# 1879615351/Go-RIO

Measured on AMD Instinct MI355X. Metric: APD-GICP GN iters/sec on 16k-pt scans + GP-preint windows/sec, higher is better.
Workload: dtype f32 search / f64 accumulate; 1 GPU; C4: 64 scan pairs 16384x16384 + 64 GP windows 1 s @ 200 Hz per GPU, k-NN covariances + 20 fixed GN iterations per pair; pairs_per_gpu=64, target_points=16384, optimizer=GN (convergence test disabled), search=pruned, parallelism=batch shard x1 (no collective)

## Files before the change

### go-rio_amd/csrc/apd_kernels.hip

```cpp
#include <hip/hip_runtime.h>
#include <math.h>
#include <stdint.h>

#include "apd_device.h"

namespace gorio {


typedef const float __attribute__((address_space(4)))* scalar_fp;
__device__ __forceinline__ scalar_fp as_scalar(const float* p) { return (scalar_fp)p; }

__device__ __forceinline__ float sqdist3(float qx, float qy, float qz, float tx, float ty, float tz) {
  float dx = qx - tx, dy = qy - ty, dz = qz - tz;
  float r = dx * dx;
  r = r + dy * dy;
  r = r + dz * dz;
  return r;
}

__device__ __forceinline__ void transform_f(const float* __restrict__ Tf, float x, float y, float z, float& qx, float& qy, float& qz) {
  float a = Tf[0] * x;
  a = a + Tf[1] * y;
  a = a + Tf[2] * z;
  qx = a + Tf[3];
// ... 111 lines not shown
      if (d[u] < bd[K - 1]) topk_insert<K>(bd, bi, d[u], j + u);
    }
  }
  if (i < n) {
    const size_t base = (size_t)split * K * n + i;
#pragma unroll
    for (int t = 0; t < K; ++t) {
      job.part_d[base + (size_t)t * n] = bd[t];
      job.part_i[base + (size_t)t * n] = bi[t];
    }
  }
}

__device__ __forceinline__ void jacobi_rot(double& app, double& aqq, double& apq, double& apr, double& aqr, double& v0p, double& v1p, double& v2p, double& v0q, double& v1q, double& v2q) {
  if (apq == 0.0) return;
  const double g = 100.0 * fabs(apq);
  if (fabs(app) + g == fabs(app) && fabs(aqq) + g == fabs(aqq)) {
    apq = 0.0;
    return;
  }
  const double theta = (aqq - app) / (2.0 * apq);
  double t = 1.0 / (fabs(theta) + sqrt(theta * theta + 1.0));
  if (theta < 0.0) t = -t;
  const double c = 1.0 / sqrt(t * t + 1.0);
  const double s = t * c;
  app = app - t * apq;
  aqq = aqq + t * apq;
  apq = 0.0;
  const double npr = c * apr - s * aqr;
  const double nqr = s * apr + c * aqr;
  apr = npr;
  aqr = nqr;
  double a, b;
  a = v0p; b = v0q; v0p = c * a - s * b; v0q = s * a + c * b;
  a = v1p; b = v1q; v1p = c * a - s * b; v1q = s * a + c * b;
  a = v2p; b = v2q; v2p = c * a - s * b; v2q = s * a + c * b;
}

struct Eig3 {
  double w0, w1, w2;
  double v00, v10, v20;
  double v01, v11, v21;
  double v02, v12, v22;
};

__device__ __forceinline__ void swap_cols(double& wa, double& wb, double& a0, double& a1, double& a2, double& b0, double& b1, double& b2) {
  double t;
  t = wa; wa = wb; wb = t;
  t = a0; a0 = b0; b0 = t;
  t = a1; a1 = b1; b1 = t;
  t = a2; a2 = b2; b2 = t;
}

__device__ __forceinline__ Eig3 sym3_eigen(double a00, double a01, double a02, double a11, double a12, double a22) {
  Eig3 e;
  e.v00 = 1; e.v10 = 0; e.v20 = 0;
  e.v01 = 0; e.v11 = 1; e.v21 = 0;
  e.v02 = 0; e.v12 = 0; e.v22 = 1;
#pragma unroll 1
  for (int sweep = 0; sweep < 12; ++sweep) {
    if (a01 == 0.0 && a02 == 0.0 && a12 == 0.0) break;
    jacobi_rot(a00, a11, a01, a02, a12, e.v00, e.v10, e.v20, e.v01, e.v11, e.v21);
    jacobi_rot(a00, a22, a02, a01, a12, e.v00, e.v10, e.v20, e.v02, e.v12, e.v22);
    jacobi_rot(a11, a22, a12, a01, a02, e.v01, e.v11, e.v21, e.v02, e.v12, e.v22);
  }
  e.w0 = a00; e.w1 = a11; e.w2 = a22;
  if (e.w0 < e.w1) swap_cols(e.w0, e.w1, e.v00, e.v10, e.v20, e.v01, e.v11, e.v21);
  if (e.w1 < e.w2) swap_cols(e.w1, e.w2, e.v01, e.v11, e.v21, e.v02, e.v12, e.v22);
  if (e.w0 < e.w1) swap_cols(e.w0, e.w1, e.v00, e.v10, e.v20, e.v01, e.v11, e.v21);
  return e;
}

__device__ __forceinline__ double geo_weight(double c00, double c01, double c02, double c11, double c12, double c22) {
  Eig3 e = sym3_eigen(c00, c01, c02, c11, c12, c22);
  const double s0 = fabs(e.w0), s1 = fabs(e.w1), s2 = fabs(e.w2);
  const double smax = fmax(s0, fmax(s1, s2)), smin = fmin(s0, fmin(s1, s2));
  return smin / smax;
}

__device__ __forceinline__ void inv_sym3(double a00, double a01, double a02, double a11, double a12, double a22, double& i00, double& i01, double& i02, double& i11, double& i12, double& i22) {
  const double c00 = a11 * a22 - a12 * a12;
  const double c01 = a02 * a12 - a01 * a22;
  const double c02 = a01 * a12 - a02 * a11;
  const double det = a00 * c00 + a01 * c01 + a02 * c02;
  const double r = 1.0 / det;
  i00 = c00 * r;
  i01 = c01 * r;
  i02 = c02 * r;
  i11 = (a00 * a22 - a02 * a02) * r;
  i12 = (a01 * a02 - a00 * a12) * r;
  i22 = (a00 * a11 - a01 * a01) * r;
}

template <int K>
__device__ __forceinline__ void covariance_from_list(const KnnJob& job, int i, const float (&bd)[K], const int (&bi)[K]) {
  const int k = job.k;
  (void)bd;
  if (job.knn_out) {
#pragma unroll
    for (int t = 0; t < K; ++t)
      if (t < k) job.knn_out[(size_t)i * k + t] = bi[t];
  }
  const float4* __restrict__ pts = job.cloud.p4;
  float px[K], py[K], pz[K];
#pragma unroll
  for (int t = 0; t < K; ++t) {
    const float4 v = pts[t < k ? bi[t] : bi[0]];
    px[t] = v.x; py[t] = v.y; pz[t] = v.z;
  }
  double mx = 0.0, my = 0.0, mz = 0.0;
#pragma unroll
  for (int t = 0; t < K; ++t)
    if (t < k) {
      mx += (double)px[t];
      my += (double)py[t];
      mz += (double)pz[t];
    }
  const double kd = (double)k;
  mx /= kd;
  my /= kd;
  mz /= kd;
  double c00 = 0, c01 = 0, c02 = 0, c11 = 0, c12 = 0, c22 = 0;
#pragma unroll
  for (int t = 0; t < K; ++t)
    if (t < k) {
      const double dx = (double)px[t] - mx, dy = (double)py[t] - my, dz = (double)pz[t] - mz;
      c00 += dx * dx;
      c01 += dx * dy;
      c02 += dx * dz;
      c11 += dy * dy;
      c12 += dy * dz;
      c22 += dz * dz;
    }
  c00 /= kd; c01 /= kd; c02 /= kd; c11 /= kd; c12 /= kd; c22 /= kd;

  double r00, r01, r02, r11, r12, r22;
  double geo = 0.0;
  bool have_geo = false;
  if (job.regularization == 0) {
    r00 = c00; r01 = c01; r02 = c02; r11 = c11; r12 = c12; r22 = c22;
  } else if (job.regularization == 4) {
    double i00, i01, i02, i11, i12, i22;
    inv_sym3(c00 + 1e-3, c01, c02, c11 + 1e-3, c12, c22 + 1e-3, i00, i01, i02, i11, i12, i22);
    const double fro = sqrt(i00 * i00 + i11 * i11 + i22 * i22 + 2.0 * (i01 * i01 + i02 * i02 + i12 * i12));
    inv_sym3(i00 / fro, i01 / fro, i02 / fro, i11 / fro, i12 / fro, i22 / fro, r00, r01, r02, r11, r12, r22);
  } else {
    Eig3 e = sym3_eigen(c00, c01, c02, c11, c12, c22);
    double s0 = fabs(e.w0), s1 = fabs(e.w1), s2 = fabs(e.w2);
    double l0, l1, l2;
    if (job.regularization == 3) {
      l0 = 1.0; l1 = 1.0; l2 = 1e-3;
    } else if (job.regularization == 1) {
      l0 = fmax(s0, 1e-3); l1 = fmax(s1, 1e-3); l2 = fmax(s2, 1e-3);
    } else {
      const double smax = fmax(s0, fmax(s1, s2));
      l0 = fmax(s0 / smax, 1e-3); l1 = fmax(s1 / smax, 1e-3); l2 = fmax(s2 / smax, 1e-3);
    }
    r00 = e.v00 * l0 * e.v00 + e.v01 * l1 * e.v01 + e.v02 * l2 * e.v02;
    r01 = e.v00 * l0 * e.v10 + e.v01 * l1 * e.v11 + e.v02 * l2 * e.v12;
    r02 = e.v00 * l0 * e.v20 + e.v01 * l1 * e.v21 + e.v02 * l2 * e.v22;
    r11 = e.v10 * l0 * e.v10 + e.v11 * l1 * e.v11 + e.v12 * l2 * e.v12;
    r12 = e.v10 * l0 * e.v20 + e.v11 * l1 * e.v21 + e.v12 * l2 * e.v22;
    r22 = e.v20 * l0 * e.v20 + e.v21 * l1 * e.v21 + e.v22 * l2 * e.v22;
    geo = fmin(l0, fmin(l1, l2)) / fmax(l0, fmax(l1, l2));
    have_geo = true;
  }
  double* o = job.cloud.cov6 + (size_t)i * 6;
  o[0] = r00; o[1] = r01; o[2] = r02; o[3] = r11; o[4] = r12; o[5] = r22;
  job.cloud.geo_w[i] = have_geo ? geo : geo_weight(r00, r01, r02, r11, r12, r22);
}

template <int K>
__global__ __launch_bounds__(256) void cov_finalize_kernel(const KnnJob* __restrict__ jobs) {
  const KnnJob job = jobs[blockIdx.z];
  const int n = job.cloud.n;
  const int i = blockIdx.x * 256 + threadIdx.x;
  if (i >= n) return;
  float bd[K];
  int bi[K];
#pragma unroll
  for (int t = 0; t < K; ++t) {
    bd[t] = INFINITY;
    bi[t] = 0x7fffffff;
  }
  for (int s = 0; s < job.splits; ++s) {
    const size_t base = (size_t)s * K * n + i;
    for (int t = 0; t < K; ++t) {
      const float d = job.part_d[base + (size_t)t * n];
      if (!(d < bd[K - 1])) break;
      topk_insert<K>(bd, bi, d, job.part_i[base + (size_t)t * n]);
    }
  }
  covariance_from_list<K>(job, i, bd, bi);
}

__global__ __launch_bounds__(256) void geo_weight_kernel(const double* __restrict__ cov6, double* __restrict__ geo_w, int n) {
  const int i = blockIdx.x * 256 + threadIdx.x;
  if (i >= n) return;
  const double* c = cov6 + (size_t)i * 6;
  geo_w[i] = geo_weight(c[0], c[1], c[2], c[3], c[4], c[5]);
}


__global__ __launch_bounds__(256) void nn_search_kernel(const PairDesc* __restrict__ descs) {
  const PairDesc& pd = descs[blockIdx.z];
  const PairState* __restrict__ st = pd.state;
  if (st->done) return;
  const int n = pd.src.n;
  if (blockIdx.x * 256 >= n) return;
  if ((int)(blockIdx.x * 256) < pd.shard_lo || (int)(blockIdx.x * 256) >= pd.shard_hi) return;
  const int split = blockIdx.y;
  if (split >= pd.nn_splits) return;
  const int j0 = split * pd.nn_chunk;
  int j1 = j0 + pd.nn_chunk;
  if (j1 > pd.tgt.n_pad) j1 = pd.tgt.n_pad;
  const int i = blockIdx.x * 256 + threadIdx.x;
  const int iq = i < n ? i : n - 1;
  float qx, qy, qz;
  transform_f(st->Tf, pd.src.x[iq], pd.src.y[iq], pd.src.z[iq], qx, qy, qz);
  const scalar_fp tx = as_scalar(pd.tgt.x);
  const scalar_fp ty = as_scalar(pd.tgt.y);
  const scalar_fp tz = as_scalar(pd.tgt.z);
  float best = INFINITY;
  int bc = 0x7fffffff;
  for (int j = j0; j < j1; j += 16) {
    float d[16];
#pragma unroll
    for (int u = 0; u < 16; ++u) d[u] = sqdist3(qx, qy, qz, tx[j + u], ty[j + u], tz[j + u]);
    const float m0 = fminf(fminf(d[0], d[1]), d[2]), m1 = fminf(fminf(d[3], d[4]), d[5]), m2 = fminf(fminf(d[6], d[7]), d[8]);
    const float m3 = fminf(fminf(d[9], d[10]), d[11]), m4 = fminf(fminf(d[12], d[13]), d[14]);
    const float m = fminf(fminf(fminf(m0, m1), m2), fminf(fminf(m3, m4), d[15]));
    const bool lt = m < best;
    best = lt ? m : best;
    bc = lt ? j : bc;
  }
  int bj = 0x7fffffff;
  if (bc != 0x7fffffff) {
#pragma unroll
    for (int u = 15; u >= 0; --u) {
      const float d = sqdist3(qx, qy, qz, pd.tgt.x[bc + u], pd.tgt.y[bc + u], pd.tgt.z[bc + u]);
      bj = d == best ? bc + u : bj;
    }
  }
  if (i < n && bj != 0x7fffffff) {
    const unsigned long long key = ((unsigned long long)__float_as_uint(best) << 32) | (unsigned int)bj;
    atomicMin(pd.best_key + i, key);
  }
}


struct PointTerms {
  double e0, e1, e2;
  double a0, a1, a2;
  double o00, o01, o02, o11, o12, o22;
};

__device__ __forceinline__ double residual_terms(const double* __restrict__ T, float ax, float ay, float az, float bx, float by, float bz, PointTerms& p) {
#pragma clang fp contract(fast)
  const double x = (double)ax, y = (double)ay, z = (double)az;
  p.a0 = T[0] * x + T[1] * y + T[2] * z + T[3];
  p.a1 = T[4] * x + T[5] * y + T[6] * z + T[7];
  p.a2 = T[8] * x + T[9] * y + T[10] * z + T[11];
  p.e0 = (double)bx - p.a0;
  p.e1 = (double)by - p.a1;
  p.e2 = (double)bz - p.a2;
  const double m0 = p.o00 * p.e0 + p.o01 * p.e1 + p.o02 * p.e2;
  const double m1 = p.o01 * p.e0 + p.o11 * p.e1 + p.o12 * p.e2;
  const double m2 = p.o02 * p.e0 + p.o12 * p.e1 + p.o22 * p.e2;
  return p.e0 * m0 + p.e1 * m1 + p.e2 * m2;
}

__device__ void gn_step_tail(const PairDesc& pd, const ApdConsts& cst);
__device__ double vgicp_error_part(const PairDesc& pd, const VoxPair& vp, const double* __restrict__ T);
template <bool VGICP>
__device__ double ndtc_error_part(const PairDesc& pd, const NdtcPair& np, const double* __restrict__ T);

__device__ __forceinline__ float sumsq2_f(float a, float b) {
  float r = a * a;
  r = r + b * b;
  return r;
}

template <int METHOD>
__global__ __launch_bounds__(256) __attribute__((amdgpu_waves_per_eu(6, 6))) void linearize_kernel(const PairDesc* __restrict__ descs, ApdConsts cst, int fuse) {
  const GridPos gp = xcd_grid_pos();
  const PairDesc& pd = descs[gp.z];
  PairState* __restrict__ st = pd.state;
  const __attribute__((address_space(4))) PairState* sst = (const __attribute__((address_space(4))) PairState*)pd.state;
  if (sst->done) return;
  const int n = pd.src.n;
  if (gp.x * 256 >= (unsigned int)n) return;
  const int i = gp.x * 256 + threadIdx.x;

  double acc[28];
#pragma unroll
  for (int t = 0; t < 28; ++t) acc[t] = 0.0;

  if (i < n) {
    typedef const __attribute__((address_space(1))) unsigned long long* g_u64p;
    typedef const __attribute__((address_space(1))) double* g_f64p;
    typedef const __attribute__((address_space(1))) float* g_f32p;
    const unsigned long long key = ((g_u64p)pd.best_key)[i];
    const float ax = ((g_f32p)pd.src.x)[i], ay = ((g_f32p)pd.src.y)[i], az = ((g_f32p)pd.src.z)[i];
    const float src_label = ((g_f32p)pd.src.label)[i];
    const double src_geo_w = ((g_f64p)pd.src.geo_w)[i];
    double cA[6];
#pragma unroll
    for (int t = 0; t < 6; ++t) cA[t] = ((g_f64p)pd.src.cov6)[(size_t)i * 6 + t];
    pd.best_key[i] = ~0ull;
    const float d = __uint_as_float((unsigned int)(key >> 32));
    int j = (int)(unsigned int)(key & 0xffffffffu);
    const bool found = key != ~0ull;
    pd.sqd[i] = found ? d : INFINITY;
    if (!found || !((double)d < cst.thr2)) j = -1;
    pd.corr[i] = j;
    const int jj = j >= 0 ? j : 0;
    double cB[6];
#pragma unroll
    for (int t = 0; t < 6; ++t) cB[t] = ((g_f64p)pd.tgt.cov6)[(size_t)jj * 6 + t];
    float4 tb;
    {
      typedef float v4f_lin __attribute__((ext_vector_type(4)));
      const v4f_lin t4 = ((const __attribute__((address_space(1))) v4f_lin*)pd.tgt.p4)[jj];
      tb = make_float4(t4.x, t4.y, t4.z, t4.w);
    }
    double* om = pd.omega6 + (size_t)i * 6;
    if (j >= 0) {
#pragma clang fp contract(fast)
      double T[12];
      float Tf[12];
#pragma unroll
      for (int t = 0; t < 12; ++t) {
        T[t] = sst->x0[t];
        Tf[t] = sst->Tf[t];
      }
      double r00 = 0.0, r01 = 0.0, r02 = 0.0, r11 = 0.0, r12 = 0.0, r22 = 0.0;
      if constexpr (METHOD == kMethodApd) {
      float qx, qy, qz;
      transform_f(Tf, ax, ay, az, qx, qy, qz);
      const double px = (double)qx, py = (double)qy, pz = (double)qz;
      const double pxy2 = px * px + py * py;
      const double dist = sqrt(pxy2 + pz * pz);
      const double s_x = dist * cst.dist_var / 400;
      const double s_y = dist * cst.sin_az;
      const double s_z = dist * cst.sin_el;
      const float rxy = (float)sqrt((double)sumsq2_f(qx, qy));
      double ce, se, ca, sa;
      {
        const double rd = (double)rxy;
        const double el = atan2(rd, pz), az = atan2(py, px);
        const double del = (double)(float)el - el, daz = (double)(float)az - az;
        const double h2 = rd * rd + pz * pz;
        const double ih = h2 > 0.0 ? rsqrt_newton(h2) : 0.0, ir = pxy2 > 0.0 ? rsqrt_newton(pxy2) : 0.0;
        const double se0 = rd * ih, ce0 = h2 > 0.0 ? pz * ih : 1.0;
        const double sa0 = py * ir, ca0 = pxy2 > 0.0 ? px * ir : 1.0;
        const double sde = del - del * del * del * (1.0 / 6.0), cde = 1.0 - 0.5 * del * del;
        const double sda = daz - daz * daz * daz * (1.0 / 6.0), cda = 1.0 - 0.5 * daz * daz;
        se = se0 * cde + ce0 * sde;
        ce = ce0 * cde - se0 * sde;
        sa = sa0 * cda + ca0 * sda;
        ca = ca0 * cda - sa0 * sda;
      }
      const double A00 = ca * ce * s_x, A01 = -sa * s_y, A02 = ca * se * s_z;
      const double A10 = sa * ce * s_x, A11 = ca * s_y, A12 = sa * se * s_z;
      const double A20 = -se * s_x, A22 = ce * s_z;
      r00 = A00 * A00 + A01 * A01 + A02 * A02;
      r01 = A00 * A10 + A01 * A11 + A02 * A12;
      r02 = A00 * A20 + A02 * A22;
      r11 = A10 * A10 + A11 * A11 + A12 * A12;
      r12 = A10 * A20 + A12 * A22;
      r22 = A20 * A20 + A22 * A22;
      }
      double a00 = cA[0], a01 = cA[1], a02 = cA[2], a11 = cA[3], a12 = cA[4], a22 = cA[5];
      if constexpr (METHOD == kMethodApd) {
        a00 = cA[0] + r00; a01 = cA[1] + r01; a02 = cA[2] + r02; a11 = cA[3] + r11; a12 = cA[4] + r12; a22 = cA[5] + r22;
      }
      const double R00 = T[0], R01 = T[1], R02 = T[2], R10 = T[4], R11 = T[5], R12 = T[6], R20 = T[8], R21 = T[9], R22 = T[10];
      const double M00 = R00 * a00 + R01 * a01 + R02 * a02, M01 = R00 * a01 + R01 * a11 + R02 * a12, M02 = R00 * a02 + R01 * a12 + R02 * a22;
      const double M10 = R10 * a00 + R11 * a01 + R12 * a02, M11 = R10 * a01 + R11 * a11 + R12 * a12, M12 = R10 * a02 + R11 * a12 + R12 * a22;
      const double M20 = R20 * a00 + R21 * a01 + R22 * a02, M21 = R20 * a01 + R21 * a11 + R22 * a12, M22 = R20 * a02 + R21 * a12 + R22 * a22;
      if constexpr (METHOD == kMethodApd) {
        cB[0] += r00; cB[1] += r01; cB[2] += r02; cB[3] += r11; cB[4] += r12; cB[5] += r22;
      }
      const double q00 = cB[0] + (M00 * R00 + M01 * R01 + M02 * R02);
      const double q01 = cB[1] + (M00 * R10 + M01 * R11 + M02 * R12);
      const double q02 = cB[2] + (M00 * R20 + M01 * R21 + M02 * R22);
      const double q11 = cB[3] + (M10 * R10 + M11 * R11 + M12 * R12);
      const double q12 = cB[4] + (M10 * R20 + M11 * R21 + M12 * R22);
      const double q22 = cB[5] + (M20 * R20 + M21 * R21 + M22 * R22);
      PointTerms p;
      inv_sym3(q00, q01, q02, q11, q12, q22, p.o00, p.o01, p.o02, p.o11, p.o12, p.o22);
      if (pd.write_omega) {
        om[0] = p.o00; om[1] = p.o01; om[2] = p.o02; om[3] = p.o11; om[4] = p.o12; om[5] = p.o22;
      }

      const double quad = residual_terms(T, ax, ay, az, tb.x, tb.y, tb.z, p);
      if constexpr (METHOD == kMethodApd) {
        const double w = 1.0 + src_geo_w + ((tb.w == src_label) ? 1.0 / (double)(pd.cl_points > 0 ? pd.cl_points : n) : 0.0);
        acc[27] = w * quad;
      } else {
        acc[27] = quad;
      }

      const double G00 = p.a2 * p.o01 - p.a1 * p.o02, G01 = p.a2 * p.o11 - p.a1 * p.o12, G02 = p.a2 * p.o12 - p.a1 * p.o22;
      const double G10 = -p.a2 * p.o00 + p.a0 * p.o02, G11 = -p.a2 * p.o01 + p.a0 * p.o12, G12 = -p.a2 * p.o02 + p.a0 * p.o22;
      const double G20 = p.a1 * p.o00 - p.a0 * p.o01, G21 = p.a1 * p.o01 - p.a0 * p.o11, G22 = p.a1 * p.o02 - p.a0 * p.o12;
      const double Hrr00 = G01 * p.a2 - G02 * p.a1, Hrr01 = -G00 * p.a2 + G02 * p.a0, Hrr02 = G00 * p.a1 - G01 * p.a0;
      const double Hrr11 = -G10 * p.a2 + G12 * p.a0, Hrr12 = G10 * p.a1 - G11 * p.a0;
      const double Hrr22 = G20 * p.a1 - G21 * p.a0;
      acc[0] = Hrr00; acc[1] = Hrr01; acc[2] = Hrr02; acc[3] = -G00; acc[4] = -G01; acc[5] = -G02;
      acc[6] = Hrr11; acc[7] = Hrr12; acc[8] = -G10; acc[9] = -G11; acc[10] = -G12;
      acc[11] = Hrr22; acc[12] = -G20; acc[13] = -G21; acc[14] = -G22;
      acc[15] = p.o00; acc[16] = p.o01; acc[17] = p.o02;
      acc[18] = p.o11; acc[19] = p.o12;
      acc[20] = p.o22;
      const double oe0 = p.o00 * p.e0 + p.o01 * p.e1 + p.o02 * p.e2;
      const double oe1 = p.o01 * p.e0 + p.o11 * p.e1 + p.o12 * p.e2;
      const double oe2 = p.o02 * p.e0 + p.o12 * p.e1 + p.o22 * p.e2;
      acc[21] = G00 * p.e0 + G01 * p.e1 + G02 * p.e2;
      acc[22] = G10 * p.e0 + G11 * p.e1 + G12 * p.e2;
      acc[23] = G20 * p.e0 + G21 * p.e1 + G22 * p.e2;
      acc[24] = -oe0; acc[25] = -oe1; acc[26] = -oe2;
    } else {
      if (pd.write_omega) {
        om[0] = 0; om[1] = 0; om[2] = 0; om[3] = 0; om[4] = 0; om[5] = 0;
      }
    }
  }

  __shared__ double red[4][28];
  const int lane = threadIdx.x & 63, wv = threadIdx.x >> 6;
  {
    double ws[7];
    wave_sum28(acc, ws);
    if ((lane & 15) == 0) {
#pragma unroll
      for (int k = 0; k < 7; ++k) red[wv][7 * (lane >> 4) + k] = ws[k];
    }
  }
  __syncthreads();
  if (threadIdx.x < 28) {
    const double s = (red[0][threadIdx.x] + red[1][threadIdx.x]) + (red[2][threadIdx.x] + red[3][threadIdx.x]);
    if (!fuse) {
      pd.partials[(size_t)gp.x * 28 + threadIdx.x] = s;
    } else {
      __hip_atomic_store(pd.partials + (size_t)gp.x * 28 + threadIdx.x, s, __ATOMIC_RELAXED, __HIP_MEMORY_SCOPE_AGENT);
    }
  }
  if (!fuse) return;
  __shared__ int s_last;
  asm volatile("s_waitcnt vmcnt(0) lgkmcnt(0)" ::: "memory");
  if (threadIdx.x == 0) s_last = __hip_atomic_fetch_add(&st->arrive, 1u, __ATOMIC_RELAXED, __HIP_MEMORY_SCOPE_AGENT) == (unsigned int)pd.nblk - 1u;
  __syncthreads();
  if (!s_last) return;
  if (threadIdx.x == 0) __hip_atomic_store(&st->arrive, 0u, __ATOMIC_RELAXED, __HIP_MEMORY_SCOPE_AGENT);
  gn_step_tail(pd, cst);
}


__device__ void ldlt6_solve(const double* __restrict__ A_in, const double* __restrict__ rhs, double* __restrict__ x, double* __restrict__ ws) {
  double* A = ws;
  double* y = ws + 36;
  double* col = ws + 42;
  int* perm = reinterpret_cast<int*>(ws + 48);
  for (int i = 0; i < 36; ++i) A[i] = A_in[i];
  for (int i = 0; i < 6; ++i) perm[i] = i;
  for (int k = 0; k < 6; ++k) {
    int piv = k;
    double best = fabs(A[k * 6 + k]);
    for (int i = k + 1; i < 6; ++i)
      if (fabs(A[i * 6 + i]) > best) {
        best = fabs(A[i * 6 + i]);
        piv = i;
      }
    if (piv != k) {
      for (int c = 0; c < 6; ++c) {
        double t = A[k * 6 + c];
        A[k * 6 + c] = A[piv * 6 + c];
        A[piv * 6 + c] = t;
      }
      for (int r = 0; r < 6; ++r) {
        double t = A[r * 6 + k];
        A[r * 6 + k] = A[r * 6 + piv];
        A[r * 6 + piv] = t;
      }
      int t = perm[k];
      perm[k] = perm[piv];
      perm[piv] = t;
    }
    const double d = A[k * 6 + k];
    if (d == 0.0) continue;
    for (int i = k + 1; i < 6; ++i) col[i] = A[i * 6 + k];
    for (int i = k + 1; i < 6; ++i) {
      const double l = col[i] / d;
      for (int j = k + 1; j <= i; ++j) A[i * 6 + j] -= l * col[j];
      A[i * 6 + k] = l;
    }
    for (int i = k + 1; i < 6; ++i)
      for (int j = i + 1; j < 6; ++j) A[i * 6 + j] = A[j * 6 + i];
  }
  for (int i = 0; i < 6; ++i) y[i] = rhs[perm[i]];
  for (int i = 0; i < 6; ++i)
    for (int j = 0; j < i; ++j) y[i] -= A[i * 6 + j] * y[j];
  for (int i = 0; i < 6; ++i) y[i] = (A[i * 6 + i] != 0.0) ? y[i] / A[i * 6 + i] : 0.0;
  for (int i = 5; i >= 0; --i)
    for (int j = i + 1; j < 6; ++j) y[i] -= A[j * 6 + i] * y[j];
  for (int i = 0; i < 6; ++i) x[perm[i]] = y[i];
}

__device__ void delta_from_d(const double* __restrict__ d, double* __restrict__ delta) {
  const double theta_sq = d[0] * d[0] + d[1] * d[1] + d[2] * d[2];
  double imag, real;
  if (theta_sq < 1e-10) {
    const double theta_quad = theta_sq * theta_sq;
    imag = 0.5 - 1.0 / 48.0 * theta_sq + 1.0 / 3840.0 * theta_quad;
    real = 1.0 - 1.0 / 8.0 * theta_sq + 1.0 / 384.0 * theta_quad;
  } else {
    const double theta = sqrt(theta_sq);
    const double half = 0.5 * theta;
    imag = sin(half) / theta;
    real = cos(half);
  }
  const double w = real, x = imag * d[0], y = imag * d[1], z = imag * d[2];
  const double tx = 2.0 * x, ty = 2.0 * y, tz = 2.0 * z;
  const double twx = tx * w, twy = ty * w, twz = tz * w, txx = tx * x, txy = ty * x, txz = tz * x, tyy = ty * y, tyz = tz * y, tzz = tz * z;
  delta[0] = 1.0 - (tyy + tzz); delta[1] = txy - twz; delta[2] = txz + twy; delta[3] = d[3];
  delta[4] = txy + twz; delta[5] = 1.0 - (txx + tzz); delta[6] = tyz - twx; delta[7] = d[4];
  delta[8] = txz - twy; delta[9] = tyz + twx; delta[10] = 1.0 - (txx + tyy); delta[11] = d[5];
  delta[12] = 0; delta[13] = 0; delta[14] = 0; delta[15] = 1;
}

__device__ void isom_mul(const double* __restrict__ A, const double* __restrict__ B, double* __restrict__ C) {
  double t[16];
#pragma unroll
  for (int r = 0; r < 3; ++r) {
#pragma unroll
    for (int c = 0; c < 3; ++c) t[r * 4 + c] = A[r * 4 + 0] * B[c] + A[r * 4 + 1] * B[4 + c] + A[r * 4 + 2] * B[8 + c];
    t[r * 4 + 3] = A[r * 4 + 0] * B[3] + A[r * 4 + 1] * B[7] + A[r * 4 + 2] * B[11] + A[r * 4 + 3];
  }
  t[12] = 0; t[13] = 0; t[14] = 0; t[15] = 1;
#pragma unroll
  for (int i = 0; i < 16; ++i) C[i] = t[i];
}

__device__ bool is_converged(const double* __restrict__ delta, double inv_rot_eps, double inv_trans_eps) {
  double rmax = 0.0, tmax = 0.0;
#pragma unroll
  for (int r = 0; r < 3; ++r) {
#pragma unroll
    for (int c = 0; c < 3; ++c) {
      const double v = inv_rot_eps * fabs(delta[r * 4 + c] - (r == c ? 1.0 : 0.0));
      rmax = v > rmax ? v : rmax;
    }
    const double v = inv_trans_eps * fabs(delta[r * 4 + 3]);
    tmax = v > tmax ? v : tmax;
  }
  return fmax(rmax, tmax) < 1.0;
}

template <int METHOD, typename AUX>
__device__ double block_error(const PairDesc& pd, const AUX* __restrict__ vp, const double* __restrict__ T, const ApdConsts& cst, double* __restrict__ sred) {
  const int n = pd.src.n;
  double sum = 0.0;
  if constexpr (METHOD == kMethodVgicp) {
    sum = vgicp_error_part(pd, *vp, T);
  } else if constexpr (METHOD == kMethodNdtCuda) {
    sum = ndtc_error_part<false>(pd, *vp, T);
  } else if constexpr (METHOD == kMethodVgicpCuda) {
    sum = ndtc_error_part<true>(pd, *vp, T);
  } else {
    for (int i = threadIdx.x; i < n; i += blockDim.x) {
      const int j = pd.corr[i];
      if (j < 0) continue;
      const double* om = pd.omega6 + (size_t)i * 6;
      PointTerms p;
      p.o00 = om[0]; p.o01 = om[1]; p.o02 = om[2]; p.o11 = om[3]; p.o12 = om[4]; p.o22 = om[5];
      const float4 tb = pd.tgt.p4[j];
      const double quad = residual_terms(T, pd.src.x[i], pd.src.y[i], pd.src.z[i], tb.x, tb.y, tb.z, p);
      if constexpr (METHOD == kMethodApd) {
        const double w = 1.0 + pd.src.geo_w[i] + ((tb.w == pd.src.label[i]) ? 1.0 / (double)(pd.cl_points > 0 ? pd.cl_points : n) : 0.0);
        sum += w * quad;
      } else {
        sum += quad;
      }
    }
  }
  sum = wave_sum(sum);
  const int lane = threadIdx.x & 63, wv = threadIdx.x >> 6;
  __syncthreads();
  if (lane == 0) sred[wv] = sum;
  __syncthreads();
  double tot = 0.0;
  const int nw = blockDim.x >> 6;
  for (int w = 0; w < nw; ++w) tot += sred[w];
  return tot;
}

template <int METHOD, typename AUX>
__device__ void lm_solve_body(const PairDesc& pd, const AUX* __restrict__ vp, const ApdConsts& cst, int mode) {
  PairState* __restrict__ st = pd.state;
  __shared__ double sH[36], sb[6], sxi[16], sdelta[16], sd[6], sws[56], sHl[36], snb[6];
  __shared__ double sy0, sred[16];
  __shared__ int sflag;
  if (mode == 2) {
    const double yi = block_error<METHOD>(pd, vp, st->xi, cst, sred);
    if (threadIdx.x == 0) st->yi = yi;
    return;
  }
  if (st->done) return;

  if (threadIdx.x < 28) {
    double s = 0.0;
    for (int bk0 = 0; bk0 < pd.nblk; bk0 += 16) {
      double v[16];
#pragma unroll
      for (int u = 0; u < 16; ++u) v[u] = (bk0 + u < pd.nblk) ? pd.partials[(size_t)(bk0 + u) * 28 + threadIdx.x] : 0.0;
#pragma unroll
      for (int u = 0; u < 16; ++u) s += v[u];
    }
    const int t = threadIdx.x;
    if (t < 21) {
      int r = 0, c = t;
      int rowlen = 6;
      while (c >= rowlen) {
        c -= rowlen;
        ++r;
        --rowlen;
      }
      c += r;
      sH[r * 6 + c] = s;
      sH[c * 6 + r] = s;
    } else if (t < 27) {
      sb[t - 21] = s;
    } else {
      sy0 = s;
    }
  }
  __syncthreads();
  if (threadIdx.x == 0) {
    for (int a = 0; a < 36; ++a) st->H[a] = sH[a];
    for (int a = 0; a < 6; ++a) st->b[a] = sb[a];
    st->y0 = sy0;
    st->n_linearize += 1;
  }
  if (mode == 1) return;

  const double inv_re = 1.0 / cst.rot_eps, inv_te = 1.0 / cst.trans_eps;
  int ok = 0;
  if (cst.optimizer == 0) {
    if (threadIdx.x == 0) {
      for (int a = 0; a < 6; ++a) snb[a] = -sb[a];
      ldlt6_solve(sH, snb, sd, sws);
      delta_from_d(sd, sdelta);
      isom_mul(sdelta, st->x0, sxi);
      for (int a = 0; a < 16; ++a) st->x0[a] = sxi[a];
      for (int a = 0; a < 36; ++a) st->Hfin[a] = sH[a];
    }
    ok = 1;
  } else {
    double lambda = st->lambda;
    if (lambda < 0.0) {
      double mx = 0.0;
      for (int a = 0; a < 6; ++a) mx = fmax(mx, fabs(sH[a * 6 + a]));
      lambda = cst.lm_init_lambda_factor * mx;
    }
    double nu = 2.0;
    for (int trial = 0; trial < cst.lm_max_iterations; ++trial) {
      if (threadIdx.x == 0) {
        for (int a = 0; a < 36; ++a) sHl[a] = sH[a];
        for (int a = 0; a < 6; ++a) {
          sHl[a * 6 + a] += lambda;
          snb[a] = -sb[a];
        }
        ldlt6_solve(sHl, snb, sd, sws);
        delta_from_d(sd, sdelta);
        isom_mul(sdelta, st->x0, sxi);
      }
      __syncthreads();
      const double yi = block_error<METHOD>(pd, vp, sxi, cst, sred);
      if (threadIdx.x == 0) {
        st->n_error += 1;
        double den = 0.0;
        for (int a = 0; a < 6; ++a) den += sd[a] * (lambda * sd[a] - sb[a]);
        const double rho = (sy0 - yi) / den;
        if (rho < 0) {
          sflag = is_converged(sdelta, inv_re, inv_te) ? 2 : 0;
        } else {
          sflag = 1;
          for (int a = 0; a < 16; ++a) st->x0[a] = sxi[a];
          const double f = 1 - pow(2 * rho - 1, 3);
          st->lambda = lambda * fmax(1.0 / 3.0, f);
          for (int a = 0; a < 36; ++a) st->Hfin[a] = sH[a];
        }
      }
      __syncthreads();
      const int flag = sflag;
      if (flag == 1) {
        ok = 1;
        break;
      }
      if (flag == 2) {
        ok = 1;
        if (threadIdx.x == 0) st->lambda = lambda;
        break;
      }
      lambda = nu * lambda;
      nu = 2 * nu;
      if (threadIdx.x == 0) st->lambda = lambda;
    }
  }
  __syncthreads();
  if (threadIdx.x == 0) {
    const int it = st->iter;
    st->nr_iterations = it;
    int done = 0, conv = 0;
    if (!ok) {
      done = 1;
      st->lm_failed = 1;
    } else {
      conv = is_converged(sdelta, inv_re, inv_te) ? 1 : 0;
      if (conv) done = 1;
    }
    st->iter = it + 1;
    if (it + 1 >= cst.max_iterations) done = 1;
    st->converged = conv;
    for (int a = 0; a < 12; ++a) st->Tf[a] = (float)st->x0[a];
    __threadfence();
// ... 295 lines not shown
```

### go-rio_amd/csrc/ugpm_api.hip

```cpp
#include <hip/hip_runtime.h>

#include <algorithm>
#include <cstdlib>
#include <chrono>
#include <cstdio>
#include <cstring>
#include <limits>
#include <memory>
#include <string>
#include <atomic>
#include <vector>

#include "../../include/gorio_ugpm.h"
#include "dev_buffer.h"
#include "ugpm_kernels.hip"
#include "ugpm_lpm_out.hip"
#include "ugpm_chunks.h"
#include "ugpm_windows.h"

using namespace gorio;
using namespace gorio::windows;

namespace {

#ifndef GORIO_EVAL_SPLIT
#define GORIO_EVAL_SPLIT 12
#endif
constexpr int kEvalSplit = GORIO_EVAL_SPLIT;

thread_local std::string g_err;
thread_local double g_stage_s[8] = {0, 0, 0, 0, 0, 0, 0, 0};
thread_local int g_stage_n[8] = {0, 0, 0, 0, 0, 0, 0, 0};
std::atomic<int> g_speculative_rot{1};
std::atomic<int> g_debug_path{0};

int ufail(int code, const std::string& msg) {
  g_err = msg;
  return code;
}

#define UHIP(expr)                                                                                              \
  do {                                                                                                          \
    hipError_t e_ = (expr);                                                                                     \
    if (e_ != hipSuccess) return ufail(GORIO_UGPM_ERR_NO_DEVICE, std::string(#expr) + ": " + hipGetErrorString(e_)); \
  } while (0)

struct StreamPair {
  hipStream_t s = nullptr, s2 = nullptr;
  hipEvent_t ev_jac = nullptr, ev_corr = nullptr;
};

int make_stream_pair(StreamPair& p) {
  int lo = 0, hi = 0;
  if (!(hipDeviceGetStreamPriorityRange(&lo, &hi) == hipSuccess && hipStreamCreateWithPriority(&p.s, hipStreamNonBlocking, hi) == hipSuccess))
    UHIP(hipStreamCreateWithFlags(&p.s, hipStreamNonBlocking));
  UHIP(hipStreamCreateWithFlags(&p.s2, hipStreamNonBlocking));
  UHIP(hipEventCreateWithFlags(&p.ev_jac, hipEventDisableTiming));
  UHIP(hipEventCreateWithFlags(&p.ev_corr, hipEventDisableTiming));
  return 0;
}

void destroy_stream_pair(StreamPair& p) {
  if (p.s) hipStreamDestroy(p.s);
  if (p.s2) hipStreamDestroy(p.s2);
  if (p.ev_jac) hipEventDestroy(p.ev_jac);
  if (p.ev_corr) hipEventDestroy(p.ev_corr);
  p = StreamPair();
}

struct Ctx {
  int device = -1;
  StreamPair main;
  hipEvent_t ev_up = nullptr;
  struct Group : StreamPair { hipEvent_t ev_done = nullptr, ev_tab = nullptr; };
  std::vector<Group> groups;
  DevBuf<double> ws;
  DevBuf<UgpmWin> d_wins;
  DevBuf<int> d_ints;
  DevBuf<double> d_diag;
  size_t wins_cap = 0;
  int lm_budget[2] = {0, 0};
  PinnedBuf pin_in;
  PinnedBuf pin_out;
  DevBuf<double> lpm_ws;
  DevBuf<int> lpm_ints;
  DevBuf<ug::LpmOutWin> d_lpm_wins;
  struct StageEvents { hipEvent_t a, b; int stage; };
  std::vector<StageEvents> ev;

  void drop_stage_events() {
    for (auto& e : ev) { hipEventDestroy(e.a); hipEventDestroy(e.b); }
    ev.clear();
  }
  void reset() {
    if (device >= 0) hipSetDevice(device);
    for (size_t g = 1; g < groups.size(); ++g) destroy_stream_pair(groups[g]);
    for (Group& g : groups) { hipEventDestroy(g.ev_done); hipEventDestroy(g.ev_tab); }
    groups.clear();
    destroy_stream_pair(main);
    if (ev_up) hipEventDestroy(ev_up);
    ev_up = nullptr;
    drop_stage_events();
    ws.reset(); d_wins.reset(); d_ints.reset(); d_diag.reset(); pin_in.reset(); pin_out.reset(); lpm_ws.reset(); lpm_ints.reset(); d_lpm_wins.reset();
    wins_cap = 0;
    lm_budget[0] = lm_budget[1] = 0;
    device = -1;
  }
  ~Ctx() { reset(); }
};
thread_local Ctx g_ctx;

struct Stage {
  Ctx& c;
  hipStream_t stream;
  size_t slot = 0;
  bool on = false;
  Stage(Ctx& c_, int s, hipStream_t st = nullptr) : c(c_), stream(st ? st : c_.main.s) {
    hipEvent_t a = nullptr, b = nullptr;
    if (hipEventCreate(&a) != hipSuccess || hipEventCreate(&b) != hipSuccess) return;
    slot = c.ev.size();
    c.ev.push_back({a, b, s});
    hipEventRecord(a, stream);
    on = true;
  }
  ~Stage() {
    if (on) hipEventRecord(c.ev[slot].b, stream);
  }
};
struct StageEventsGuard {
  Ctx& c;
  ~StageEventsGuard() { c.drop_stage_events(); }
};

struct Run : Ctx::Group {
  int g0 = 0, nw = 0;
  const UgpmWin* wins = nullptr;
  bool active = true;
};

struct Batch {
  const gorio_ugpm_window* windows;
  int nw;
  std::vector<HostWin> hw;
  std::vector<UgpmWin> dw;
  std::vector<int> ints, flags, lpm_ints_h;
  std::vector<double> lpm_in;
  std::vector<ug::LpmOutWin> lw;
  std::vector<size_t> out_offs;
  std::vector<Run> runs;
  size_t total_doubles = 0, total_in = 0, total_out = 0;
  double* out_region = nullptr;
  int max_S = 0, max_G = 2, max_V = 2, max_infer = 0, n_lpm = 0;
  bool rerun = false;
  bool looks = false;
  bool enqueued_blind[2] = {false, false};
  std::vector<int> final_status;
  int first_error = 0;
  std::string first_error_msg;
  void note_error(int i, int code, const std::string& m) {
    if (first_error) return;
    first_error = code;
    first_error_msg = "window " + std::to_string(i) + ": " + m;
  }
};

int ensure_context(Ctx& c, int device) {
  int ndev = 0;
  if (hipGetDeviceCount(&ndev) != hipSuccess || ndev <= 0) return ufail(GORIO_UGPM_ERR_NO_DEVICE, "no usable HIP device (no CPU fallback exists)");
  if (device < 0 || device >= ndev) return ufail(GORIO_UGPM_ERR_INVALID, "bad device ordinal");
  if (c.device != device) c.reset();
  UHIP(hipSetDevice(device));
  if (c.device == device) return 0;
  if (int rc = make_stream_pair(c.main)) return rc;
  UHIP(hipFuncSetAttribute(reinterpret_cast<const void*>(&ug::corr_diag_kernel), hipFuncAttributeMaxDynamicSharedMemorySize, 140 * 1024));
  UHIP(hipFuncSetAttribute(reinterpret_cast<const void*>(&ug::infer_kernel), hipFuncAttributeMaxDynamicSharedMemorySize, 17 * (6 * 160 + 16) * 8) );
  const void* fns[] = {reinterpret_cast<const void*>(&ug::ata_kernel<4, 16, kAtaTilesCorr>), reinterpret_cast<const void*>(&ug::ata_kernel<8, 16, kAtaTilesCorr>),
                       reinterpret_cast<const void*>(&ug::ata_kernel<16, 8, kAtaTilesCorr>), reinterpret_cast<const void*>(&ug::ata_kernel<4, 16, kAtaTilesLm>),
                       reinterpret_cast<const void*>(&ug::ata_kernel<8, 16, kAtaTilesLm>)};
  for (const void* f : fns) UHIP(hipFuncSetAttribute(f, hipFuncAttributeMaxDynamicSharedMemorySize, 144 * 1024));
  c.device = device;
  return 0;
}

void plan_windows(Batch& b) {
  b.hw.resize(b.nw);
  int total_infer = 0;
  for (int i = 0; i < b.nw; ++i) {
    const gorio_ugpm_window& w = b.windows[i];
    HostWin& h = b.hw[i];
    total_infer += std::max(0, w.n_infer);
    b.max_infer = std::max(b.max_infer, w.n_infer);
    std::string err;
    if (plan_window(w, h, err) != 0) {
      b.note_error(i, h.status, err);
    } else if (h.is_lpm) {
      b.n_lpm++;
    } else {
      b.max_S = std::max(b.max_S, h.S);
      b.total_in += input_slot(w, h);
      b.total_doubles += h.ws_doubles;
    }
  }
  for (const HostWin& h : b.hw) {
    b.max_G = std::max(b.max_G, h.is_lpm ? 2 : h.G);
    b.max_V = std::max(b.max_V, h.is_lpm ? 2 : h.V);
  }
  b.total_out = (size_t)total_infer * 83;
  b.total_doubles += b.total_in + b.total_out + 64;
}

int reserve_workspace(Ctx& c, const Batch& b) {
  const size_t nw = b.nw;
  UHIP(c.ws.reserve(b.total_doubles));
  UHIP(reserve_group(c.wins_cap, nw, nw, c.d_wins, nw, c.d_ints, kWinInts * nw, c.d_diag, 4 * nw));
  UHIP(c.pin_in.reserve(sizeof(double) * b.total_in, sizeof(double) * (b.total_in + b.total_in / 4 + 64)));
  const size_t down = sizeof(double) * (b.total_out + 4 * nw) + sizeof(int) * kWinInts * nw;
  UHIP(c.pin_out.reserve(down, down + down / 4 + 64));
  return 0;
}

int stage_and_upload(Ctx& c, Batch& b) {
  b.dw.resize(b.nw);
  b.ints.assign(kWinInts * (size_t)b.nw, 0);
  b.out_offs.assign(b.nw, 0);
  double* const in_region = c.ws.get();
  b.out_region = in_region + b.total_in;
  double* base = b.out_region + (b.total_out + 31) / 32 * 32;
  double* const stage_in = static_cast<double*>(c.pin_in.get());
  size_t in_off = 0, out_off = 0;
  for (int i = 0; i < b.nw; ++i) {
    const gorio_ugpm_window& w = b.windows[i];
    const HostWin& h = b.hw[i];
    UgpmWin& u = b.dw[i];
    std::memset(&u, 0, sizeof(u));
    u.lmi = c.d_ints + kWinInts * (size_t)i;
    u.status = c.d_ints + kWinInts * (size_t)i + 16;
    b.ints[kWinInts * (size_t)i + 16] = h.status;
    u.n_infer = std::max(0, w.n_infer);
    b.out_offs[i] = out_off;
    u.out = b.out_region + out_off;
    out_off += (size_t)u.n_infer * 83;
    if (h.status != 0) continue;
    if (h.is_lpm) {
      b.ints[kWinInts * (size_t)i + 16] = 1;
      u.n_infer = 0;
      continue;
    }
    carve(w, h, u, base, in_region + in_off, u.out);
    u.G = h.G; u.V = h.V; u.S = h.S;
    u.correlate = w.correlate ? 1 : 0; u.overlap = w.overlap;
    u.state_freq = h.state_freq;
    copy_noise_and_priors(w, u);
    base += h.ws_doubles;
    double* s = stage_in + in_off;
    const size_t padded = input_slot(w, h);
    for (size_t k = padded - 4; k < padded; ++k) s[k] = 0.0;
    s = stage_samples(s, w, h.g0, h.G, h.v0, h.V);
    std::copy(h.state_t.begin(), h.state_t.end(), s);
    in_off += padded;
  }
  if (b.total_in) UHIP(hipMemcpyAsync(in_region, stage_in, sizeof(double) * b.total_in, hipMemcpyHostToDevice, c.main.s));
  UHIP(hipMemcpyAsync(c.d_wins, b.dw.data(), sizeof(UgpmWin) * b.nw, hipMemcpyHostToDevice, c.main.s));
  UHIP(hipMemcpyAsync(c.d_ints, b.ints.data(), sizeof(int) * b.ints.size(), hipMemcpyHostToDevice, c.main.s));
  UHIP(hipMemsetAsync(c.d_diag, 0, sizeof(double) * 4 * b.nw, c.main.s));
  return 0;
}

int run_lpm_windows(Ctx& c, Batch& b) {
  if (b.n_lpm == 0) return 0;
  std::vector<LpmHost> lh(b.n_lpm);
  std::vector<int> widx;
  size_t dbl = 0, in_dbl = 0, nint = 0;
  int max_T = 2;
  for (int i = 0; i < b.nw; ++i) {
    if (!b.hw[i].is_lpm || b.hw[i].status != 0) continue;
    LpmHost& L = lh[widx.size()];
    build_lpm_timeline(b.windows[i], L);
    widx.push_back(i);
    max_T = std::max(max_T, (int)L.tl.size());
    ug::LpmOutWin dummy;
    const LpmSize sz = carve_lpm(b.windows[i], L.tl.size(), dummy, nullptr, nullptr, nullptr);
    in_dbl += sz.in;
    dbl += sz.scratch + 8;
    nint += sz.ints;
  }
  UHIP(c.lpm_ws.reserve(in_dbl + dbl));
  UHIP(c.lpm_ints.reserve(nint));
  UHIP(c.d_lpm_wins.reserve(b.n_lpm));
  b.lw.resize(widx.size());
  b.lpm_in.assign(in_dbl, 0.0);
  b.lpm_ints_h.assign(nint, 0);
  LpmSize at;
  for (size_t k = 0; k < widx.size(); ++k) {
    const int i = widx[k];
    const gorio_ugpm_window& w = b.windows[i];
    const LpmHost& L = lh[k];
    ug::LpmOutWin& u = b.lw[k];
    std::memset(&u, 0, sizeof(u));
    const LpmSize sz = carve_lpm(w, L.tl.size(), u, c.lpm_ws.get() + at.in, c.lpm_ws.get() + in_dbl + at.scratch, c.lpm_ints.get() + at.ints);
    std::copy(L.tl.begin(), L.tl.end(), stage_samples(b.lpm_in.data() + at.in, w, 0, w.n_gyr, 0, w.n_vel));
    stage_lpm_tables(b.lpm_ints_h.data() + at.ints, L);
    at.in += sz.in; at.scratch += sz.scratch; at.ints += sz.ints;
    u.G = w.n_gyr; u.V = w.n_vel; u.T = (int)L.tl.size(); u.n_infer = w.n_infer;
    u.start_index = L.start_index; u.dt_index = L.dt_index;
    copy_noise_and_priors(w, u);
    u.out = b.dw[i].out;
    u.status = c.d_ints + kWinInts * (size_t)i + 17;
  }
  UHIP(hipMemcpyAsync(c.lpm_ws, b.lpm_in.data(), sizeof(double) * in_dbl, hipMemcpyHostToDevice, c.main.s));
  UHIP(hipMemcpyAsync(c.lpm_ints, b.lpm_ints_h.data(), sizeof(int) * nint, hipMemcpyHostToDevice, c.main.s));
  UHIP(hipMemcpyAsync(c.d_lpm_wins, b.lw.data(), sizeof(ug::LpmOutWin) * b.lw.size(), hipMemcpyHostToDevice, c.main.s));
  const int nl = (int)b.lw.size();
  if (nl > 0) {
    Stage st(c, 0);
    ug::lpm_out_steps_kernel<<<dim3((max_T + 255) / 256, 5, nl), 256, 0, c.main.s>>>(c.d_lpm_wins);
    ug::lpm_out_scan_kernel<<<dim3(5, nl), 64, 0, c.main.s>>>(c.d_lpm_wins);
    ug::lpm_out_finish_kernel<<<nl, 256, 0, c.main.s>>>(c.d_lpm_wins);
    UHIP(hipGetLastError());
  }
  return 0;
}

int open_groups(Ctx& c, Batch& b) {
  int n_groups = 1;
  if (const char* e = std::getenv("GORIO_UGPM_GROUPS")) n_groups = std::atoi(e);
  n_groups = std::max(1, std::min(std::min(n_groups, 8), b.nw));
  while ((int)c.groups.size() < n_groups) {
    Ctx::Group g;
    if (c.groups.empty()) static_cast<StreamPair&>(g) = c.main;
    else if (int rc = make_stream_pair(g)) return rc;
    UHIP(hipEventCreateWithFlags(&g.ev_done, hipEventDisableTiming));
    UHIP(hipEventCreateWithFlags(&g.ev_tab, hipEventDisableTiming));
    c.groups.push_back(g);
  }
  if (!c.ev_up) UHIP(hipEventCreateWithFlags(&c.ev_up, hipEventDisableTiming));
  UHIP(hipEventRecord(c.ev_up, c.main.s));
  b.runs.resize(n_groups);
  for (int g = 0; g < n_groups; ++g) {
    Run& r = b.runs[g];
    static_cast<Ctx::Group&>(r) = c.groups[g];
    r.g0 = (int)((long)b.nw * g / n_groups);
    r.nw = (int)((long)b.nw * (g + 1) / n_groups) - r.g0;
    r.wins = c.d_wins + r.g0;
    if (g > 0) UHIP(hipStreamWaitEvent(r.s, c.ev_up, 0));
  }
  return 0;
}

void launch_ata(Ctx& c, int max_S, const Run& r, int which, int decide = 0) {
  hipStream_t sq = which == 2 ? r.s2 : r.s;
  Stage st_ata(c, which == 2 ? 6 : 5, sq);
  const int n = (which == 2 ? 6 : 3) * max_S;
  const int tpg = which == 2 ? kAtaTilesCorr : kAtaTilesLm;
  const int dense = (g_debug_path.load() & 1) ? 1 : 0;
  const int ng = ata_cut(n, which == 2 && !dense ? 3 * max_S : n, tpg).groups();
  const int npad = ((n + 15) / 32) * 32 + 16;
  const int grid = ((r.nw + 7) / 8) * ng * 8;
  auto lds = [&](int kc) { return sizeof(double) * 2 * kc * (npad + 1); };
  if (which == 2) {
    if (npad <= 256) ug::ata_kernel<4, 16, kAtaTilesCorr><<<grid, 512, lds(16), sq>>>(r.wins, which, r.nw, ng, decide, dense);
    else if (npad <= 512) ug::ata_kernel<8, 16, kAtaTilesCorr><<<grid, 512, lds(16), sq>>>(r.wins, which, r.nw, ng, decide, dense);
    else ug::ata_kernel<16, 8, kAtaTilesCorr><<<grid, 512, lds(8), sq>>>(r.wins, which, r.nw, ng, decide, dense);
  } else {
    if (npad <= 256) ug::ata_kernel<4, 16, kAtaTilesLm><<<grid, 512, lds(16), sq>>>(r.wins, which, r.nw, ng, decide, dense);
    else ug::ata_kernel<8, 16, kAtaTilesLm><<<grid, 512, lds(16), sq>>>(r.wins, which, r.nw, ng, decide, dense);
  }
}

int enqueue_tables_and_correlation(Ctx& c, Batch& b) {
  const int max_S = b.max_S;
  for (const Run& r : b.runs) {
    {
      Stage st(c, 0, r.s);
      ug::lpm_rot_kernel<<<dim3(r.nw, 5), 320, 0, r.s>>>(r.wins);
      ug::lpm_init_kernel<<<r.nw, 320, 0, r.s>>>(r.wins);
    }
    {
      Stage st(c, 1, r.s);
      ug::gram_kernel<<<dim3(6, r.nw), 256, 0, r.s>>>(r.wins);
      ug::cross_kernel<<<dim3(12, r.nw, (std::max(b.max_G, b.max_V) + ug::kCrossRows - 1) / ug::kCrossRows), 256, sizeof(double) * ug::kCrossRows * (((max_S + 31) / 32) * 32 + 4), r.s>>>(r.wins);
    }
    UHIP(hipEventRecord(r.ev_tab, r.s));
    UHIP(hipStreamWaitEvent(r.s2, r.ev_tab, 0));
    {
      Stage st(c, 2, r.s2);
      ug::corr_jac_kernel<<<dim3(ug::kCorrJacParts, r.nw), 256, 0, r.s2>>>(r.wins);
      UHIP(hipEventRecord(r.ev_jac, r.s2));
      launch_ata(c, max_S, r, 2);
      ug::corr_factor_kernel<<<r.nw, 512, 0, r.s2>>>(r.wins);
      ug::corr_diag_kernel<<<dim3((6 * max_S + 15) / 16, r.nw), 256, sizeof(double) * 17 * (6 * max_S + 16), r.s2>>>(r.wins);
    }
    UHIP(hipEventRecord(r.ev_corr, r.s2));
  }
  return 0;
}

int run_fit(Ctx& c, Batch& b, int problem) {
  const int max_S = b.max_S;
  std::vector<int>& flags = b.flags;
  const bool lmtrace = std::getenv("GORIO_UGPM_LMTRACE") != nullptr;
  const bool speculative = g_speculative_rot.load() != 0;
  std::vector<std::unique_ptr<Stage>> st_lm;
  for (Run& r : b.runs) {
    st_lm.emplace_back(new Stage(c, 3, r.s));
    if (problem == 0) ug::rot_eval_kernel<<<dim3(r.nw, kEvalSplit), 256, 0, r.s>>>(r.wins, 2);
    else ug::vel_eval_kernel<<<dim3(r.nw, kEvalSplit), 256, 0, r.s>>>(r.wins, 2);
    launch_ata(c, max_S, r, problem);
    r.active = true;
  }
  for (int it = 0; it <= 51; ++it) {
    bool any = false;
    for (Run& r : b.runs) {
      if (!r.active) continue;
      any = true;
      ug::lm_step_kernel<<<dim3(r.nw, problem == 1 ? kVelBlocks : 1), 512, 0, r.s>>>(r.wins);
      if (problem == 0 && speculative) {
        ug::rot_eval_kernel<<<dim3(r.nw, kEvalSplit), 256, 0, r.s>>>(r.wins, 3);
        launch_ata(c, max_S, r, problem, 1);
        continue;
      }
      if (problem == 0) ug::rot_eval_kernel<<<dim3(r.nw, kEvalSplit), 256, 0, r.s>>>(r.wins, 0);
      else ug::vel_eval_kernel<<<dim3(r.nw, kEvalSplit), 256, 0, r.s>>>(r.wins, 0);
      if (problem == 0) {
        ug::rot_eval_kernel<<<dim3(r.nw, kEvalSplit), 256, 0, r.s>>>(r.wins, 1);
        launch_ata(c, max_S, r, problem);
      } else {
        ug::lm_relinearize_linear_kernel<<<dim3(r.nw, (3 * max_S + 63) / 64), 256, 0, r.s>>>(r.wins);
      }
    }
    if (!any) break;
    if (lmtrace) {
      double lc[16];
      int li[16];
      UHIP(hipStreamSynchronize(b.runs[0].s));
      UHIP(hipMemcpy(lc, b.dw[0].lmc, sizeof(lc), hipMemcpyDeviceToHost));
      UHIP(hipMemcpy(li, b.dw[0].lmi, sizeof(li), hipMemcpyDeviceToHost));
      std::fprintf(stderr, "[ugpm lm] problem %d it %d: iter %d done %d term %d succ %d cost %.17g cost_new %.17g radius %.6g mcc %.17g step_norm2 %.6g x_norm %.17g initial %.17g\n", problem, it,
                   li[0], li[1], li[5], li[6], lc[0], lc[1], lc[2], lc[8], lc[11], lc[4], lc[7]);
    }
    const int budget = c.lm_budget[problem];
    if (budget > 0 && !b.looks) {
      b.enqueued_blind[problem] = true;
      if (it + 1 >= budget) break;
      continue;
    }
    const bool look = budget > 0 ? (it + 1 >= budget && ((it + 1 - budget) & 1) == 0) : (it >= 3 && (it & 1) == 1);
    if (look) {
      for (Run& r : b.runs)
        if (r.active) UHIP(hipMemcpyAsync(flags.data() + kWinInts * (size_t)r.g0, c.d_ints + kWinInts * (size_t)r.g0, sizeof(int) * kWinInts * (size_t)r.nw, hipMemcpyDeviceToHost, r.s));
      for (Run& r : b.runs) {
        if (!r.active) continue;
        UHIP(hipStreamSynchronize(r.s));
        bool all = true;
        for (int i = r.g0; i < r.g0 + r.nw; ++i) all = all && (flags[kWinInts * (size_t)i + 1] || flags[kWinInts * (size_t)i + 16] != 0);
        if (all) r.active = false;
      }
      bool every = true;
      for (Run& r : b.runs) every = every && !r.active;
      if (every) {
        int need = 1;
        for (int i = 0; i < b.nw; ++i) {
          const int* f = flags.data() + kWinInts * (size_t)i;
          if (f[16] != 0) continue;
          need = std::max(need, f[0] + (f[5] >= 3 ? 1 : 0));
        }
        need = std::min(need, it + 1);
        c.lm_budget[problem] = b.rerun ? std::max(c.lm_budget[problem], need) : need;
      }
    }
  }
  for (size_t g = 0; g < b.runs.size(); ++g) {
    const Run& r = b.runs[g];
    if (problem == 0) {
      UHIP(hipStreamWaitEvent(r.s, r.ev_jac, 0));
      ug::lm_turn_kernel<<<r.nw, 256, 0, r.s>>>(r.wins, c.d_diag + 4 * (size_t)r.g0);
    }
    st_lm[g].reset();
  }
  return 0;
}

int enqueue_finish_and_infer(Ctx& c, Batch& b) {
  for (const Run& r : b.runs) {
    UHIP(hipStreamWaitEvent(r.s, r.ev_corr, 0));
    {
      Stage st(c, 4, r.s);
      ug::finish_kernel<<<r.nw, 256, 0, r.s>>>(r.wins, c.d_diag + 4 * (size_t)r.g0);
      ug::infer_kernel<<<dim3(std::max(1, b.max_infer), r.nw), 256, sizeof(double) * 17 * (6 * b.max_S + 16), r.s>>>(r.wins);
    }
    UHIP(hipEventRecord(r.ev_done, r.s));
  }
  for (size_t g = 1; g < b.runs.size(); ++g) UHIP(hipStreamWaitEvent(c.main.s, b.runs[g].ev_done, 0));
  UHIP(hipGetLastError());
  return 0;
}

int collect(Ctx& c, Batch& b, gorio_ugpm_meas* out, gorio_ugpm_diag* diag, std::vector<int>& unfinished) {
  double* const rec = static_cast<double*>(c.pin_out.get());
  double* const dg = rec + b.total_out;
  int* const fin = reinterpret_cast<int*>(dg + 4 * (size_t)b.nw);
  UHIP(hipMemcpyAsync(fin, c.d_ints, sizeof(int) * kWinInts * (size_t)b.nw, hipMemcpyDeviceToHost, c.main.s));
  UHIP(hipMemcpyAsync(dg, c.d_diag, sizeof(double) * 4 * (size_t)b.nw, hipMemcpyDeviceToHost, c.main.s));
  if (b.total_out) UHIP(hipMemcpyAsync(rec, b.out_region, sizeof(double) * b.total_out, hipMemcpyDeviceToHost, c.main.s));
  UHIP(hipStreamSynchronize(c.main.s));
  if (b.total_out) std::memcpy(out, rec, sizeof(double) * b.total_out);
  for (const Ctx::StageEvents& e : c.ev) {
    float ms = 0.f;
    if (hipEventSynchronize(e.b) == hipSuccess && hipEventElapsedTime(&ms, e.a, e.b) == hipSuccess) {
      g_stage_s[e.stage] += ms * 1e-3;
      g_stage_n[e.stage] += 1;
    }
  }
  c.drop_stage_events();
  if (b.enqueued_blind[0] || b.enqueued_blind[1]) {
    FitOutcome o = fit_outcome(fin, b.hw);
    for (int p = 0; p < 2; ++p)
      if (b.enqueued_blind[p] && o.need[p] > 0) c.lm_budget[p] = o.need[p];
    unfinished.swap(o.rerun);
  }
  b.final_status.assign(b.nw, 0);
  for (int i = 0; i < b.nw; ++i) {
    const HostWin& h = b.hw[i];
    const int st = h.status != 0 ? h.status : fin[kWinInts * (size_t)i + (h.is_lpm ? 17 : 16)];
    b.final_status[i] = st;
    if (diag) {
      gorio_ugpm_diag& d = diag[i];
      d.nb_state = h.S; d.nb_gyr = h.G; d.nb_vel = h.V;
      d.iters_rot = (int)dg[4 * (size_t)i + 0]; d.cost_rot = dg[4 * (size_t)i + 1];
      d.iters_vel = (int)dg[4 * (size_t)i + 2]; d.cost_vel = dg[4 * (size_t)i + 3];
      d.status = st; d.state_freq = h.state_freq;
    }
  }
  return 0;
}

int preint_batch_flat(const gorio_ugpm_window* windows, int n_windows, gorio_ugpm_meas* out, gorio_ugpm_diag* diag, int device, bool rerun);

int rerun_unfinished(Batch& b, const std::vector<int>& unfinished, gorio_ugpm_meas* out, gorio_ugpm_diag* diag, int device) {
  std::vector<gorio_ugpm_window> sub;
  size_t n_out = 0;
  for (int i : unfinished) {
    sub.push_back(b.windows[i]);
    n_out += (size_t)b.windows[i].n_infer;
  }
  std::vector<gorio_ugpm_meas> sub_out(n_out);
  std::vector<gorio_ugpm_diag> sub_diag(sub.size());
  const int rc = preint_batch_flat(sub.data(), (int)sub.size(), sub_out.data(), sub_diag.data(), device, true);
  bool per_window = false;
  for (const gorio_ugpm_diag& d : sub_diag) per_window = per_window || d.status != 0;
  if (rc != 0 && !per_window) return rc;
  size_t at = 0;
  for (size_t k = 0; k < unfinished.size(); ++k) {
    const int i = unfinished[k];
    const size_t cnt = (size_t)b.windows[i].n_infer;
    std::memcpy(reinterpret_cast<double*>(out) + b.out_offs[i], sub_out.data() + at, sizeof(gorio_ugpm_meas) * cnt);
    at += cnt;
    b.final_status[i] = sub_diag[k].status;
    if (diag) diag[i] = sub_diag[k];
  }
  return 0;
}

void report(Batch& b, gorio_ugpm_meas* out) {
  for (int i = 0; i < b.nw; ++i) {
    const HostWin& h = b.hw[i];
    const int st = b.final_status[i];
    if (h.status != 0 || (h.is_lpm && st != 0)) {
      double* o = reinterpret_cast<double*>(out) + b.out_offs[i];
      std::fill(o, o + (size_t)std::max(0, b.windows[i].n_infer) * 83, std::numeric_limits<double>::quiet_NaN());
    }
    if (st != 0 && h.status == 0)
      b.note_error(i, st, st == GORIO_UGPM_ERR_NUMERIC ? "Cholesky factorisation met a non-positive pivot" : "LPM Partial: the start_time is not in the data domain");
  }
}

int preint_batch_flat(const gorio_ugpm_window* windows, int n_windows, gorio_ugpm_meas* out, gorio_ugpm_diag* diag, int device, bool rerun) {
  if (!windows || n_windows <= 0 || !out) return ufail(GORIO_UGPM_ERR_INVALID, "gorio_ugpm_preint_batch: bad arguments");
  Ctx& c = g_ctx;
  if (int rc = ensure_context(c, device)) return rc;
  if (!rerun)
    for (int i = 0; i < 8; ++i) { g_stage_s[i] = 0; g_stage_n[i] = 0; }
  std::vector<int> unfinished;
  Batch b{windows, n_windows};
  b.rerun = rerun;
  b.looks = rerun || (g_debug_path.load() & 2) != 0;
  {
    StageEventsGuard guard{c};
    auto tnow = [] { return std::chrono::duration<double>(std::chrono::steady_clock::now().time_since_epoch()).count(); };
    const double tt0 = tnow();
    plan_windows(b);
    if (int rc = reserve_workspace(c, b)) return rc;
    if (int rc = stage_and_upload(c, b)) return rc;
    const double tt1 = tnow();
    if (int rc = run_lpm_windows(c, b)) return rc;
    if (b.max_S > 0) {
      b.flags.resize(kWinInts * (size_t)b.nw);
      if (int rc = open_groups(c, b)) return rc;
      if (int rc = enqueue_tables_and_correlation(c, b)) return rc;
      for (int problem = 0; problem < 2; ++problem)
        if (int rc = run_fit(c, b, problem)) return rc;
      if (int rc = enqueue_finish_and_infer(c, b)) return rc;
    }
    const double tt3 = tnow();
    if (int rc = collect(c, b, out, diag, unfinished)) return rc;
    if (std::getenv("GORIO_UGPM_TRACE")) std::fprintf(stderr, "[ugpm trace] prep %.3f ms, kernels+polls %.3f ms, results %.3f ms, unfinished %d\n", (tt1 - tt0) * 1e3, (tt3 - tt1) * 1e3, (tnow() - tt3) * 1e3, (int)unfinished.size());
  }
  if (!unfinished.empty())
    if (int rc = rerun_unfinished(b, unfinished, out, diag, device)) return rc;
  report(b, out);
  if (b.first_error) return ufail(b.first_error, b.first_error_msg);
  return GORIO_UGPM_OK;
}

}

extern "C" {

void gorio_ugpm_default_window(gorio_ugpm_window* w) {
  if (!w) return;
  std::memset(w, 0, sizeof(*w));
  w->type = GORIO_UGPM_TYPE_UGPM;
  w->min_freq = 500;
  w->quantum = -1;
  w->state_freq = 50.0;
  w->correlate = 1;
  w->overlap = 8;
  w->vel_bias_std = 0.3;
  w->gyr_bias_std = 0.03;
}

const char* gorio_ugpm_last_error(void) { return g_err.c_str(); }

void gorio_ugpm_debug_set_schedule(int speculative_rot) { g_speculative_rot.store(speculative_rot ? 1 : 0); }

void gorio_ugpm_debug_set_path(int flags) { g_debug_path.store(flags); }

int gorio_ugpm_get_stage_times(double seconds[8], int counts[8]) {
  for (int i = 0; i < 8; ++i) {
    if (seconds) seconds[i] = g_stage_s[i];
    if (counts) counts[i] = g_stage_n[i];
  }
  return 0;
}

int gorio_ugpm_preint_batch(const gorio_ugpm_window* windows, int n_windows, gorio_ugpm_meas* out, gorio_ugpm_diag* diag, int device) {
  if (!windows || n_windows <= 0 || !out) return ufail(GORIO_UGPM_ERR_INVALID, "gorio_ugpm_preint_batch: bad arguments");
  bool any_chunked = false;
  for (int i = 0; i < n_windows; ++i) any_chunked = any_chunked || windows[i].quantum >= 0;
  if (!any_chunked) return preint_batch_flat(windows, n_windows, out, diag, device, false);
  struct Req { int first = 0, count = 0, status = 0; chunks::Plan plan; size_t out0 = 0; };
  std::vector<Req> reqs(n_windows);
  std::vector<gorio_ugpm_window> flat;
  std::vector<size_t> flat_out0;
  int first_error = 0;
  std::string first_error_msg;
  size_t n_flat_out = 0, out_off = 0;
  for (int i = 0; i < n_windows; ++i) {
    const gorio_ugpm_window& w = windows[i];
    Req& r = reqs[i];
    r.out0 = out_off;
    out_off += (size_t)std::max(0, w.n_infer);
    r.first = (int)flat.size();
    if (w.quantum < 0) {
      r.count = 1;
      flat.push_back(w);
      flat_out0.push_back(n_flat_out);
      n_flat_out += (size_t)std::max(0, w.n_infer);
      continue;
    }
    std::string err;
    if (!w.gyr_t || !w.gyr || !w.vel_t || !w.vel || !w.infer_t || w.n_infer <= 0) {
      r.status = GORIO_UGPM_ERR_INVALID;
      err = "null pointers or no inference time";
    } else {
      r.status = chunks::plan_chunks(w, r.plan, err);
    }
    if (r.status != 0) {
      if (!first_error) {
        first_error = r.status;
        first_error_msg = "window " + std::to_string(i) + ": " + err;
      }
      continue;
    }
    for (chunks::Chunk& c : r.plan.chunks) {
      gorio_ugpm_window cw = w;
      cw.gyr_t = w.gyr_t + c.g0; cw.gyr = w.gyr + 3 * (size_t)c.g0; cw.n_gyr = c.ng;
      cw.vel_t = w.vel_t + c.v0; cw.vel = w.vel + 3 * (size_t)c.v0; cw.n_vel = c.nv;
      cw.start_t = c.start_t;
      cw.infer_t = c.infer_t.data(); cw.n_infer = (int)c.infer_t.size();
      cw.group_sizes = c.group_sizes.data(); cw.n_groups = (int)c.group_sizes.size();
      cw.quantum = -1;
      cw.vel_bias_std = 0.0; cw.gyr_bias_std = 0.0;
      flat.push_back(cw);
      flat_out0.push_back(n_flat_out);
      n_flat_out += c.infer_t.size();
    }
    r.count = (int)r.plan.chunks.size();
  }
  const gorio_ugpm_meas nan_meas = [] {
    gorio_ugpm_meas m;
    double* p = reinterpret_cast<double*>(&m);
    for (size_t k = 0; k < sizeof(m) / sizeof(double); ++k) p[k] = std::numeric_limits<double>::quiet_NaN();
    return m;
  }();
  std::vector<gorio_ugpm_meas> flat_out(std::max<size_t>(1, n_flat_out), nan_meas);
  std::vector<gorio_ugpm_diag> flat_diag(std::max<size_t>(1, flat.size()));
  int rc = 0;
  if (!flat.empty()) {
    rc = preint_batch_flat(flat.data(), (int)flat.size(), flat_out.data(), flat_diag.data(), device, false);
    bool per_window = false;
    for (const gorio_ugpm_diag& d : flat_diag) per_window = per_window || d.status != 0;
    if (rc != 0 && !per_window) return rc;
  }
  const std::string flat_msg = rc != 0 ? g_err : std::string();
  for (int i = 0; i < n_windows; ++i) {
    const gorio_ugpm_window& w = windows[i];
    Req& r = reqs[i];
    gorio_ugpm_meas* o = out + r.out0;
    gorio_ugpm_diag d{};
    if (r.status == 0 && w.quantum < 0) {
      for (int k = 0; k < w.n_infer; ++k) o[k] = flat_out[flat_out0[r.first] + k];
      d = flat_diag[r.first];
      r.status = d.status;
    } else if (r.status == 0) {
      std::vector<const gorio_ugpm_meas*> recs;
      for (int q = 0; q < r.count; ++q) {
        const gorio_ugpm_diag& cd = flat_diag[r.first + q];
        if (cd.status != 0 && r.status == 0) r.status = cd.status;
        recs.push_back(flat_out.data() + flat_out0[r.first + q]);
        d.nb_state = cd.nb_state; d.nb_gyr = cd.nb_gyr; d.nb_vel = cd.nb_vel; d.state_freq = cd.state_freq;
        d.iters_rot += cd.iters_rot; d.iters_vel += cd.iters_vel; d.cost_rot += cd.cost_rot; d.cost_vel += cd.cost_vel;
      }
      if (r.status == 0) chunks::chain_chunks(r.plan, recs, w.vel_bias_std, w.gyr_bias_std, o);
    }
    if (r.status != 0) {
      for (int k = 0; k < std::max(0, w.n_infer); ++k) o[k] = nan_meas;
      if (!first_error) {
        first_error = r.status;
        first_error_msg = "window " + std::to_string(i) + (flat_msg.empty() ? std::string(": failed") : ": (expanded batch) " + flat_msg);
      }
    }
    d.status = r.status;
    if (diag) diag[i] = d;
  }
  if (first_error) return ufail(first_error, first_error_msg);
  return 0;
}

int gorio_ugpm_combine_preints(const gorio_ugpm_meas* prev, const gorio_ugpm_meas* cur, gorio_ugpm_meas* out) {
  if (!prev || !cur || !out) return ufail(GORIO_UGPM_ERR_INVALID, "gorio_ugpm_combine_preints: null pointer");
  *out = chunks::combine_preints(*prev, *cur);
  return 0;
}

}
```

### go-rio_amd/csrc/ugpm_device.h

```cpp
#pragma once
#include <stdint.h>

namespace gorio {

constexpr int kAtaTilesLm = 24, kAtaTilesCorr = 48;
constexpr int kWinInts = 48;
constexpr int kLmiNeed = 18;
constexpr int kStatusUnfinished = 2;
constexpr int kVelBlocks = 3;

#if defined(__HIPCC__)
#define GORIO_HD __host__ __device__
#else
#define GORIO_HD
#endif

struct AtaCut {
  int ntile, q_zero, ng_dense, ng_skip;
  GORIO_HD int groups() const { return ng_dense + ng_skip; }
  GORIO_HD bool skips(int grp) const { return grp >= ng_dense; }
  GORIO_HD int q_lo(int grp) const {
    return grp < ng_dense ? (int)((long)grp * q_zero / ng_dense) : q_zero + (int)((long)(grp - ng_dense) * (ntile - q_zero) / ng_skip);
  }
  GORIO_HD int q_hi(int grp) const { return grp + 1 == groups() ? ntile : q_lo(grp + 1); }
};
GORIO_HD inline AtaCut ata_cut(int n, int zero_col, int tpg) {
  const int T = (n + 15) / 16, tz = zero_col >= n ? T : (zero_col + 15) / 16;
  AtaCut c;
  c.ntile = T * (T + 1) / 2;
  c.q_zero = tz * (tz + 1) / 2;
  c.ng_dense = (c.q_zero + tpg - 1) / tpg;
  c.ng_skip = (c.ntile - c.q_zero + tpg - 1) / tpg;
  return c;
}

struct UgpmWin {
  const double* gyr_t;
  const double* gyr;
  const double* vel_t;
  const double* vel;
  const double* infer_t;
  double* state_t;
  int G, V, S, n_infer;
  int correlate, overlap;
  double start_t, state_freq, gyr_var, vel_var;
  double gyr_bias[3], vel_bias[3];
  double vel_bias_std, gyr_bias_std;
  double* Rq;
  double* Rstart;
  double* velr;
  double* dp;
  double* r0;
  double* r1;
  double* s_dr;
  double* s_vel;
  double* hyper;
  double* d_r_dt_local;
  double* d_r_dt_local_shift;
  double* delta_r_time;
  double* delta_r_bw;
  double* d_r_bw_local_shift;
  double* Kinv;
  double* KKinv;
  double* KintKinv;
  double* var;
  double* wgp;
  double* sstd;
  double* KsKinv;
  double* KsIntKinv;
  double* KgyrIntKinv;
  double* KvelKinv;
  double* Jrot;
  double* Jvel;
  double* res;
  double* res_new;
  double* JtJ;
  double* lhs;
  double* lmv;
  double* sample_tmp;
  double* sample_tmp_c;
  double* Jc;
  double* Ac;
  double* Linv;
  double* dsc;
  double* alpha;
  double* state_r;
  double* d_state_bw;
  double* d_d_r_dt;
  double* d_vel_bv;
  double* d_vel_bw;
  double* d_vel_dt;
  double* out;
  double* lmc;
  int* lmi;
  int* status;
};

}
```

### go-rio_amd/csrc/ugpm_kernels.hip

```cpp
#include <hip/hip_runtime.h>
#include <math.h>

#include "ugpm_device.h"

namespace gorio {
namespace ug {

__device__ __forceinline__ UgpmWin load_win(const UgpmWin* __restrict__ wins, int i) {
  UgpmWin w;
  __builtin_memcpy(&w, (const __attribute__((address_space(4))) void*)(wins + i), sizeof(UgpmWin));
  return w;
}


#ifndef GORIO_UGPM_XCD
#define GORIO_UGPM_XCD 1
#endif
struct WinPart {
  int win, part, z;
};
__device__ __forceinline__ WinPart xcd_win_part() {
  WinPart r{(int)blockIdx.y, (int)blockIdx.x, (int)blockIdx.z};
#if GORIO_UGPM_XCD
  if (gridDim.y >= 16u && (gridDim.y & 7u) == 0u) {
// ... 311 lines not shown
    if ((top1 - top2) > (1.0 / 500.0)) {
      const int nb = (int)floor((top1 - first) * 500.0);
      if (nb > 0) { nfake = nb; fake_first = first; fake_q = (top1 - first) / ((double)nb); }
    }
  }
  const int T = 2 * S + 3 + V + nfake;
  if (T > kLpmMaxT || (size_t)T * 9 > rseq_cap) return false;
  auto count_in = [&](int l, double v, bool upper) -> int {
    switch (l) {
      case 0: return upper ? upper_bound_f(S, v, w.state_t, 0.0) : lower_bound_f(S, v, w.state_t, 0.0);
      case 1: return upper ? upper_bound_f(S, v, w.state_t, -kDt) : lower_bound_f(S, v, w.state_t, -kDt);
      case 2: return upper ? (w.start_t <= v ? 1 : 0) : (w.start_t < v ? 1 : 0);
      case 3: { const double a0 = lpm_start, a1 = lpm_start + kDt; return upper ? ((a0 <= v) + (a1 <= v)) : ((a0 < v) + (a1 < v)); }
      case 4: return upper ? upper_bound_f(V, v, w.vel_t, tshift) : lower_bound_f(V, v, w.vel_t, tshift);
      default: {
        int lo = 0, hi = nfake;
        while (lo < hi) {
          const int mid = (lo + hi) >> 1;
          const double c = fake_first + mid * fake_q;
          if (upper ? (c <= v) : (c < v)) lo = mid + 1; else hi = mid;
        }
        return lo;
      }
    }
  };
  const int prio[6] = {1, 2, 3, 0, 4, 5};
  const int nl[6] = {S, S, 1, 2, V, nfake};
  for (int e = tid; e < T; e += nthr) {
    int l = 0, i = e;
    while (i >= nl[l]) { i -= nl[l]; ++l; }
    double v;
    switch (l) {
      case 0: v = w.state_t[i]; break;
      case 1: v = w.state_t[i] + kDt; break;
      case 2: v = w.start_t; break;
      case 3: v = lpm_start + (i ? kDt : 0.0); break;
      case 4: v = w.vel_t[i] - tshift; break;
      default: v = fake_first + i * fake_q; break;
    }
    int rank = i;
    for (int b = 0; b < 6; ++b)
      if (b != l && nl[b] > 0) rank += count_in(b, v, prio[b] < prio[l]);
    L.tl[rank] = v;
    L.kind[rank] = (unsigned short)l;
    L.kidx[rank] = (unsigned short)i;
    if (l == 3 && i == 0) L.start_rank = rank;
  }
  __syncthreads();
  auto gt = [&](int i) -> double { return w.gyr_t[i] - tshift; };
  auto gd = [&](int a, int i) -> double {
    double d = w.gyr[a * G + i];
    if (variant == 0) d -= w.gyr_bias[a];
    if (variant - 2 == a) d += kBw;
    return d;
  };
  const double gt0 = gt(0);
  auto step_rot = [&](int i) -> M3 {
    const double t = L.tl[i];
    int p = 0;
    if (t > gt0) {
      p = lower_bound_f(G, t, w.gyr_t, tshift) - 1;
      if (p > G - 2) p = G - 2;
      if (p < 0) p = 0;
    }
    const double t0 = gt(p), t1 = gt(p + 1);
    double wv[3];
    for (int a = 0; a < 3; ++a) {
      const double d0 = gd(a, p), d1 = gd(a, p + 1);
      const double al = (d1 - d0) / (t1 - t0);
      const double be = d0 - (al * t0);
      wv[a] = al * t + be;
    }
    const double dt = L.tl[i + 1] - t;
    return expMap(v3(wv[0] * dt, wv[1] * dt, wv[2] * dt));
  };
  const int nch = nthr < 256 ? nthr : 256;
  const int ch = (T + nch - 1) / nch;
  if (tid < nch) {
    M3 acc = eye3();
    const int i0 = tid * ch, i1 = min(T, i0 + ch);
    for (int i = i0; i < i1; ++i) {
      storeM(Rseq + (size_t)i * 9, acc);
      if (i < T - 1) acc = mmul(acc, step_rot(i));
    }
    storeM(&L.tot[0][tid][0], acc);
  }
  __syncthreads();
  int cur = 0;
  for (int off = 1; off < nch; off <<= 1) {
    if (tid < nch) {
      M3 m = loadM(&L.tot[cur][tid][0]);
      if (tid >= off) m = mmul(loadM(&L.tot[cur][tid - off][0]), m);
      storeM(&L.tot[cur ^ 1][tid][0], m);
    }
    __syncthreads();
    cur ^= 1;
  }
  if (tid < nch) {
    const M3 pre = tid > 0 ? loadM(&L.tot[cur][tid - 1][0]) : eye3();
    const int i0 = tid * ch, i1 = min(T, i0 + ch);
    for (int i = i0; i < i1; ++i) {
      const M3 Pi = mmul(pre, loadM(Rseq + (size_t)i * 9));
      storeM(Rseq + (size_t)i * 9, Pi);
      if (i == L.start_rank) storeM(L.ps, mtr(Pi));
    }
  }
  __syncthreads();
  const M3 PsT = loadM(L.ps);
  double* Rq = w.Rq + (size_t)variant * 2 * S * 9;
  for (int i = tid; i < T; i += nthr) {
    const int l = L.kind[i], idx = L.kidx[i];
    if (l == 5 || l == 3) continue;
    if (l == 4 && variant != 0) continue;
    const M3 Pi = loadM(Rseq + (size_t)i * 9);
    const M3 R = i >= L.start_rank ? mmul(PsT, Pi) : Pi;
    if (l == 0) storeM(Rq + (size_t)idx * 9, R);
    else if (l == 1) storeM(Rq + (size_t)(S + idx) * 9, R);
    else if (l == 2) storeM(w.Rstart + variant * 9, R);
    else {
      const V3 vr = mvec(R, v3(w.vel[idx] - w.vel_bias[0], w.vel[V + idx] - w.vel_bias[1], w.vel[2 * V + idx] - w.vel_bias[2]));
      w.velr[idx] = vr.x;
      w.velr[V + idx] = vr.y;
      w.velr[2 * V + idx] = vr.z;
    }
  }
  __syncthreads();
  return true;
}

__device__ void lpm_position(const UgpmWin& w, int axis) {
  const int S = w.S, V = w.V;
  const double start = w.state_t[0];
  const double* vt = w.vel_t;
  const double* vd = w.velr + (size_t)axis * V;
  int data_ptr = 0;
  while (vt[data_ptr + 1] < start) {
    data_ptr++;
    if (data_ptr == V - 1) {
      *w.status = -3;
      return;
    }
  }
  int ptr = data_ptr;
  double alpha = (vd[ptr + 1] - vd[ptr]) / (vt[ptr + 1] - vt[ptr]);
  double beta = vd[ptr] - alpha * vt[ptr];
  double t_0 = start, t_1 = vt[ptr + 1];
  double d_0 = alpha * vt[ptr] + beta, d_1 = vd[ptr + 1];
  double backup = 0.0;
  int p0 = 0, p1 = 0, p2 = 0;
  for (int step = 0; step < 2 * S + 1; ++step) {
    int bl = -1;
    double t = 0.0;
    if (p0 < S) { bl = 0; t = w.state_t[p0]; }
    if (p1 < S && (bl < 0 || w.state_t[p1] + kDt < t)) { bl = 1; t = w.state_t[p1] + kDt; }
    if (p2 < 1 && (bl < 0 || w.start_t < t)) { bl = 2; t = w.start_t; }
    int idx = 0;
    if (bl == 0) idx = p0++;
    else if (bl == 1) idx = p1++;
    else p2++;
    if (t > vt[0]) {
      while (true) {
        if ((t >= vt[ptr]) && (t <= vt[ptr + 1])) break;
        if (ptr < (V - 2)) {
          backup = backup + ((t_1 - t_0) * (d_0 + d_1) / 2.0);
          ptr++;
          t_0 = vt[ptr];
          t_1 = vt[ptr + 1];
          d_0 = vd[ptr];
          d_1 = vd[ptr + 1];
          alpha = (d_1 - d_0) / (t_1 - t_0);
          beta = d_0 - alpha * t_0;
        } else {
          break;
        }
      }
    }
    const double temp_d_1 = alpha * t + beta;
    const double temp_d_p = backup + ((t - t_0) * (d_0 + temp_d_1) / 2.0);
    if (bl < 2) w.dp[((size_t)bl * S + idx) * 3 + axis] = temp_d_p;
  }
}

__device__ void unwrap_variant(const UgpmWin& w, int variant) {
  const int S = w.S;
  const M3 sRt = mtr(loadM(w.Rstart + variant * 9));
  const double* Rq = w.Rq + (size_t)variant * 2 * S * 9;
  double* r0 = w.r0 + (size_t)variant * S * 3;
  double* r1 = w.r1 + (size_t)variant * S * 3;
  for (int pass = 0; pass < 2; ++pass) {
    int rev[2] = {0, 0};
    V3 prev[2] = {v3(0, 0, 0), v3(0, 0, 0)};
    const int from = pass == 0 ? w.overlap : w.overlap - 1, to = pass == 0 ? S : -1, stp = pass == 0 ? 1 : -1;
    for (int i = from; i != to; i += stp) {
      for (int j = 0; j < 2; ++j) {
        const V3 tr = logMap(mmul(sRt, loadM(Rq + ((size_t)j * S + i) * 9)));
        int id = 0;
        double best = 1.7976931348623157e308;
        V3 bc = tr;
        for (int q = 0; q < 3; ++q) {
          const V3 c = addN2Pi(tr, rev[j] + q - 1);
          const double d = vnorm(prev[j] - c);
          if (d < best) {
            best = d;
            id = q;
            bc = c;
          }
        }
        prev[j] = bc;
        rev[j] += (id - 1);
      }
      store3(r0 + (size_t)i * 3, prev[0]);
      store3(r1 + (size_t)i * 3, prev[1]);
    }
  }
}

__global__ __launch_bounds__(320) void lpm_rot_kernel(const UgpmWin* __restrict__ wins) {
  const UgpmWin w = load_win(wins, blockIdx.x);
  if (*w.status != 0) return;
  const int var = blockIdx.y, lane = threadIdx.x & 63;
  __shared__ LpmLds lds;
  {
    const size_t cap = ((size_t)(3 * w.S + 3 * w.G) * 3 * w.S) / 5;
    double* Rseq = w.Jrot + (size_t)var * cap;
    if (!lpm_rotation_parallel(w, var, lds, Rseq, cap)) {
      if (threadIdx.x == 0) lpm_rotation(w, var);
    }
  }
  __syncthreads();
  if (var == 0 && threadIdx.x < 3) lpm_position(w, threadIdx.x);
  if (threadIdx.x == 64) unwrap_variant(w, var);
  (void)lane;
}

__device__ void lm_begin_block(const UgpmWin& w, int problem);

__global__ __launch_bounds__(320) void lpm_init_kernel(const UgpmWin* __restrict__ wins) {
  const UgpmWin w = load_win(wins, blockIdx.x);
  if (*w.status != 0) return;
  const int S = w.S;
  const M3 sRt0 = mtr(loadM(w.Rstart));
  for (int i = threadIdx.x; i < S; i += blockDim.x) {
    const V3 a0 = load3(w.r0 + (size_t)i * 3), a1 = load3(w.r1 + (size_t)i * 3);
    const V3 d = (1.0 / kDt) * (a1 - a0);
    w.s_dr[i] = d.x; w.s_dr[S + i] = d.y; w.s_dr[2 * S + i] = d.z;
    const V3 vel = mvec(sRt0, (1.0 / kDt) * (load3(w.dp + ((size_t)S + i) * 3) - load3(w.dp + (size_t)i * 3)));
    w.s_vel[i] = vel.x; w.s_vel[S + i] = vel.y; w.s_vel[2 * S + i] = vel.z;
    store3(w.d_r_dt_local + (size_t)i * 3, mvec(Jr(a0), d));
    {
      const V3 b0 = load3(w.r0 + ((size_t)S + i) * 3), b1 = load3(w.r1 + ((size_t)S + i) * 3);
      const M3 J = Jr(b0);
      store3(w.d_r_dt_local_shift + (size_t)i * 3, mvec(J, (1.0 / kDt) * (b1 - b0)));
      store3(w.delta_r_time + (size_t)i * 3, mvec(J, b0 - a0));
    }
    for (int ax = 0; ax < 3; ++ax) {
      const V3 b0 = load3(w.r0 + ((size_t)(2 + ax) * S + i) * 3), b1 = load3(w.r1 + ((size_t)(2 + ax) * S + i) * 3);
      const M3 J = Jr(b0);
      store3(w.d_r_bw_local_shift + ((size_t)ax * S + i) * 3, mvec(J, (1.0 / kDt) * (b1 - b0)));
      store3(w.delta_r_bw + ((size_t)ax * S + i) * 3, mvec(J, b0 - a0));
    }
  }
  __syncthreads();
  if (threadIdx.x < 6) {
    const int c = threadIdx.x;
    double* s = (c < 3 ? w.s_dr + (size_t)c * S : w.s_vel + (size_t)(c - 3) * S);
    double m = 0.0;
    for (int i = 0; i < S; ++i) m += s[i];
    m /= (double)S;
    double var = 0.0;
    for (int i = 0; i < S; ++i) var += (s[i] - m) * (s[i] - m);
    var /= (double)S;
    const double noise = c < 3 ? w.gyr_var : w.vel_var;
    w.hyper[c * 4 + 0] = (3.0 / w.state_freq) * (3.0 / w.state_freq);
    w.hyper[c * 4 + 1] = fmax(var, noise);
    w.hyper[c * 4 + 2] = noise;
    w.hyper[c * 4 + 3] = m;
    for (int i = 0; i < S; ++i) s[i] -= m;
  }
  __syncthreads();
  lm_begin_block(w, 0);
}


constexpr int kCholNB = 16;
constexpr int kCholMaxN = 6 * 160;
#ifdef GORIO_CHOL_TIMING
__device__ long long g_chol_t[12];
#define CHOL_T(k)                                                         \
  do {                                                                    \
    if (blockIdx.x == 0 && threadIdx.x == 0) {                            \
      const long long now_ = (long long)__builtin_readcyclecounter();     \
      g_chol_t[k] += now_ - chol_t_last_;                                 \
      chol_t_last_ = now_;                                                \
    }                                                                     \
  } while (0)
#define CHOL_T_INIT long long chol_t_last_ = (long long)__builtin_readcyclecounter()
#define CHOL_T_VMWAIT asm volatile("s_waitcnt vmcnt(0)" ::: "memory")
#else
#define CHOL_T(k) do { } while (0)
#define CHOL_T_INIT do { } while (0)
#define CHOL_T_VMWAIT do { } while (0)
#endif
typedef double f64x4 __attribute__((ext_vector_type(4)));
struct CholLds {
  double D[2][kCholNB][kCholNB + 1];
  double Dinv[2][kCholNB];
  double Dt[kCholNB][kCholNB + 1];
  double dinv_n[384];
  unsigned short tile[328];
  double P[kCholMaxN > 384 ? 384 : kCholMaxN][kCholNB + 1];
};

__device__ __forceinline__ double readlane_f64(double v, int lane) {
  const int lo = __builtin_amdgcn_readlane(__double2loint(v), lane);
  const int hi = __builtin_amdgcn_readlane(__double2hiint(v), lane);
  return __hiloint2double(hi, lo);
}

__device__ __forceinline__ double rsqrt_newton(double a) {
  double y = __builtin_amdgcn_rsq(a);
  const double h = 0.5 * a;
#pragma unroll
  for (int it = 0; it < 2; ++it) {
    const double e = __builtin_fma(-h * y, y, 0.5);
    y = __builtin_fma(y, e, y);
  }
  return y;
}

__device__ __forceinline__ bool block_cholesky(double* __restrict__ A, int n, int lda, CholLds& L, int* __restrict__ sflag, double* __restrict__ rhs = nullptr) {
  constexpr int NB = kCholNB;
  const int tid = threadIdx.x, lane = tid & 63, wave = tid >> 6, nwave = (int)(blockDim.x >> 6);
  if (tid == 0) *sflag = 0;
  for (int q = tid; q < 325; q += blockDim.x) {
    int tr = (int)((sqrtf(8.0f * (float)q + 1.0f) - 1.0f) * 0.5f);
    while (tr * (tr + 1) / 2 > q) --tr;
    while ((tr + 1) * (tr + 2) / 2 <= q) ++tr;
    L.tile[q] = (unsigned short)((tr << 8) | (q - tr * (tr + 1) / 2));
  }
  __syncthreads();
  CHOL_T_INIT;
  const bool la = n - min(NB, n) + (rhs != nullptr ? 1 : 0) <= 384 && nwave >= 2;
  int cur = 0;
  auto factor_block = [&](double (&a)[NB], int kbd, int nbd, int buf) {
    const int r = lane;
    bool ok = true;
    double yinv = 1.0;
#pragma unroll
    for (int j = 0; j < NB; ++j) {
      const double ajj = readlane_f64(a[j], j);
      if (!(ajj > 0.0)) ok = false;
      const double y = rsqrt_newton(ajj);
      const double lrj = a[j] * y;
      if (r == j) yinv = y;
      a[j] = lrj;
#pragma unroll
      for (int c = j + 1; c < NB; ++c) {
        const double lcj = readlane_f64(lrj, c);
        a[c] = __builtin_fma(-lrj, lcj, a[c]);
      }
    }
    if (r < NB) {
#pragma unroll
      for (int c = 0; c < NB; ++c)
        if (c <= r) {
          L.D[buf][r][c] = a[c];
          if (r < nbd) A[(size_t)(kbd + r) * lda + kbd + c] = a[c];
        }
      L.Dinv[buf][r] = yinv;
      if (rhs != nullptr && r < nbd) L.dinv_n[kbd + r] = yinv;
    }
    if (!ok && lane == 0) *sflag = 1;
  };
  for (int kb = 0; kb < n; kb += NB) {
    const int nb = min(NB, n - kb);
    const int m = n - kb - nb;
    const int me = m + (rhs != nullptr ? 1 : 0);
    auto panel_row = [&](int i) -> double* { return (rhs != nullptr && i == m) ? rhs + kb : A + (size_t)(kb + nb + i) * lda + kb; };
    double x[NB];
    const bool own = tid < min(me, 384);
    auto load_row = [&](const double* arow) {
#pragma unroll
      for (int c = 0; c < NB; ++c) x[c] = c < nb ? arow[c] : 0.0;
    };
    if (!la || kb == 0) {
      if (wave != 0 && own) load_row(panel_row(tid));
      if (wave == 0) {
        const int r = lane;
        double a[NB];
#pragma unroll
        for (int c = 0; c < NB; ++c) a[c] = (r < nb && c <= r) ? A[(size_t)(kb + r) * lda + kb + c] : ((r == c) ? 1.0 : 0.0);
        factor_block(a, kb, nb, cur);
        if (own) load_row(panel_row(tid));
      }
      CHOL_T(0);
      __syncthreads();
      CHOL_T(1);
    } else if (own) {
      load_row(panel_row(tid));
    }
    if (*sflag) return false;
    if (me <= 0) break;
    for (int p0 = 0; p0 < me; p0 += 384) {
      const int mp = min(384, me - p0);
      for (int i = tid; i < mp; i += blockDim.x) {
        double* arow = panel_row(p0 + i);
        if (!(p0 == 0 && i == tid)) load_row(arow);
        asm volatile("" ::: "memory");
#pragma unroll
        for (int c = 0; c < NB; ++c) {
          double v = x[c];
#pragma unroll
          for (int q = 0; q < c; ++q) v = __builtin_fma(-x[q], L.D[cur][c][q], v);
          v *= L.Dinv[cur][c];
          x[c] = v;
          L.P[i][c] = v;
        }
#pragma unroll
        for (int c = 0; c < NB; ++c)
          if (c < nb) arow[c] = x[c];
      }
      for (int i = mp + tid; i < (((rhs != nullptr ? m : mp) + 15) & ~15); i += blockDim.x) {
#pragma unroll
        for (int c = 0; c < NB; ++c) L.P[i][c] = 0.0;
      }
      CHOL_T(2);
      __syncthreads();
      CHOL_T(3);
      if (p0 == 0) {
        const int mt = rhs != nullptr ? m : mp;
        const int T = (mt + 15) / 16;
        const int ntile = T * (T + 1) / 2;
        const int lr = lane & 15, lk = lane >> 4;
        const int wave_u = __builtin_amdgcn_readfirstlane(wave);
        const int vofs = lk * lda + lr, rstep = 4 * lda;
        const double* Pl = &L.P[0][0] + (lr * (NB + 1) + lk);
        double* Abase = A + (size_t)(kb + nb) * lda + kb + nb;
        constexpr int TU = 4;
        const bool ahead = la && m > 0;
        const int q_first = ahead ? 1 : 0;
        const int w_first = ahead ? 1 : 0, w_cnt = nwave - w_first;
        if (ahead && wave_u == 0) {
          double val[4];
#pragma unroll
          for (int rg = 0; rg < 4; ++rg) val[rg] = (lk + 4 * rg < mt && lr < mt) ? Abase[vofs + rg * rstep] : 0.0;
          f64x4 acc = f64x4{0.0, 0.0, 0.0, 0.0};
#pragma unroll
          for (int k0 = 0; k0 < NB; k0 += 4) acc = __builtin_amdgcn_mfma_f64_16x16x4f64(Pl[k0], Pl[k0], acc, 0, 0, 0);
#pragma unroll
          for (int rg = 0; rg < 4; ++rg) L.Dt[lk + 4 * rg][lr] = val[rg] - acc[rg];
          __builtin_amdgcn_fence(__ATOMIC_RELEASE, "wavefront");
          __builtin_amdgcn_wave_barrier();
          __builtin_amdgcn_fence(__ATOMIC_ACQUIRE, "wavefront");
          const int nbn = min(NB, m), r = lane;
          double a[NB];
#pragma unroll
          for (int c = 0; c < NB; ++c) a[c] = (r < nbn && c <= r) ? L.Dt[r][c] : ((r == c) ? 1.0 : 0.0);
          factor_block(a, kb + nb, nbn, cur ^ 1);
        }
        if (wave_u >= w_first) {
          for (int q0 = q_first + (wave_u - w_first) * TU; q0 < ntile; q0 += w_cnt * TU) {
            int trv[TU], tcv[TU];
            double cv[TU][4];
#pragma unroll
            for (int u = 0; u < TU; ++u) {
              const int t = __builtin_amdgcn_readfirstlane((int)L.tile[min(q0 + u, ntile - 1)]);
              trv[u] = t >> 8;
              tcv[u] = t & 255;
              const double* tb = Abase + (size_t)(trv[u] * 16) * lda + tcv[u] * 16;
              if (q0 + u < ntile) {
                if (trv[u] * 16 + 16 <= mt) {
#pragma unroll
                  for (int rg = 0; rg < 4; ++rg) cv[u][rg] = tb[vofs + rg * rstep];
                } else {
#pragma unroll
                  for (int rg = 0; rg < 4; ++rg)
                    cv[u][rg] = (trv[u] * 16 + lk + 4 * rg < mt && tcv[u] * 16 + lr < mt) ? tb[vofs + rg * rstep] : 0.0;
                }
              }
            }
#pragma unroll
            for (int u = 0; u < TU; ++u) {
              if (q0 + u >= ntile) break;
              const double* pa = Pl + trv[u] * 16 * (NB + 1);
              const double* pb = Pl + tcv[u] * 16 * (NB + 1);
              f64x4 acc = f64x4{0.0, 0.0, 0.0, 0.0};
#pragma unroll
              for (int k0 = 0; k0 < NB; k0 += 4) acc = __builtin_amdgcn_mfma_f64_16x16x4f64(pa[k0], pb[k0], acc, 0, 0, 0);
              double* tb = Abase + (size_t)(trv[u] * 16) * lda + tcv[u] * 16;
              if (trv[u] * 16 + 16 <= mt) {
#pragma unroll
                for (int rg = 0; rg < 4; ++rg) tb[vofs + rg * rstep] = cv[u][rg] - acc[rg];
              } else {
#pragma unroll
                for (int rg = 0; rg < 4; ++rg)
                  if (trv[u] * 16 + lk + 4 * rg < mt && tcv[u] * 16 + lr < mt) tb[vofs + rg * rstep] = cv[u][rg] - acc[rg];
              }
            }
          }
          if (rhs != nullptr) {
            for (int k = tid - w_first * 64; k < m; k += w_cnt * 64) {
              double acc = 0.0;
#pragma unroll
              for (int c = 0; c < NB; ++c) acc = __builtin_fma(L.P[m][c], L.P[k][c], acc);
              rhs[kb + nb + k] -= acc;
            }
          }
        }
      }
      if (p0 != 0 || me > 384) {
        for (long q = tid; q < (long)mp * m; q += blockDim.x) {
          const int i = p0 + (int)(q / m), k = (int)(q % m);
          if (k > i || (p0 == 0 && k < mp)) continue;
          double sacc = 0.0;
          for (int c = 0; c < nb; ++c) sacc += A[(size_t)(kb + nb + i) * lda + kb + c] * A[(size_t)(kb + nb + k) * lda + kb + c];
          A[(size_t)(kb + nb + i) * lda + kb + nb + k] -= sacc;
        }
      }
      CHOL_T(4);
      __syncthreads();
      CHOL_T(5);
    }
    if (la) cur ^= 1;
  }
  __syncthreads();
  return true;
}

template <int NC>
__device__ __forceinline__ void wave_forward(const double* __restrict__ L, int n, int lda, double* __restrict__ X, int ldx, int row0) {
  const int lane = threadIdx.x & 63;
  for (int i = row0; i < n; ++i) {
    const double* Lr = L + (size_t)i * lda;
    double acc[NC];
#pragma unroll
    for (int c = 0; c < NC; ++c) acc[c] = 0.0;
    for (int k = row0 + lane; k < i; k += 64) {
      const double l = Lr[k];
#pragma unroll
      for (int c = 0; c < NC; ++c) acc[c] += l * X[(size_t)k * ldx + c];
    }
#pragma unroll
    for (int c = 0; c < NC; ++c) {
#pragma unroll
      for (int off = 32; off > 0; off >>= 1) acc[c] += __shfl_down(acc[c], off, 64);
    }
    if (lane == 0) {
      const double d = Lr[i];
#pragma unroll
      for (int c = 0; c < NC; ++c) X[(size_t)i * ldx + c] = (X[(size_t)i * ldx + c] - acc[c]) / d;
    }
    __builtin_amdgcn_fence(__ATOMIC_RELEASE, "wavefront");
    __builtin_amdgcn_wave_barrier();
    __builtin_amdgcn_fence(__ATOMIC_ACQUIRE, "wavefront");
  }
}

__device__ __forceinline__ void wave_backward(const double* __restrict__ L, int n, int lda, double* __restrict__ x) {
  const int lane = threadIdx.x & 63;
  for (int i = n - 1; i >= 0; --i) {
    double acc = 0.0;
    for (int k = i + 1 + lane; k < n; k += 64) acc += L[(size_t)k * lda + i] * x[k];
#pragma unroll
    for (int off = 32; off > 0; off >>= 1) acc += __shfl_down(acc, off, 64);
    if (lane == 0) x[i] = (x[i] - acc) / L[(size_t)i * lda + i];
    __builtin_amdgcn_fence(__ATOMIC_RELEASE, "wavefront");
    __builtin_amdgcn_wave_barrier();
    __builtin_amdgcn_fence(__ATOMIC_ACQUIRE, "wavefront");
  }
}

__device__ __forceinline__ void block_backward(const double* __restrict__ Lm, int n, int lda, double* __restrict__ x, CholLds& C) {
  constexpr int NB = kCholNB;
  const int tid = threadIdx.x, lane = tid & 63;
  double cur[NB], nxt[NB];
  const int kb_last = ((n - 1) / NB) * NB;
  auto fetch = [&](int kb, double* dst) {
    const int nb = min(NB, n - kb);
#pragma unroll
    for (int c = 0; c < NB; ++c) dst[c] = (c < nb && tid <= kb + c) ? Lm[(size_t)(kb + c) * lda + tid] : 0.0;
  };
  fetch(kb_last, cur);
  double xv = tid < n ? x[tid] : 0.0;
  int buf = 0;
  const int r = lane & 15;
  for (int kb = kb_last; kb >= 0; kb -= NB) {
    const int nb = min(NB, n - kb);
    if (kb >= NB) fetch(kb - NB, nxt);
    double (*Db)[NB + 1] = &C.P[buf * (NB + 1)];
    if (tid >= kb && tid < kb + nb) {
#pragma unroll
      for (int c = 0; c < NB; ++c) Db[c][tid - kb] = cur[c];
      Db[NB][tid - kb] = xv;
    }
    __syncthreads();
    double v = r < nb ? Db[NB][r] : 0.0;
    const double dinv = r < nb ? C.dinv_n[kb + r] : 1.0;
    double dcol[NB];
#pragma unroll
    for (int j = 0; j < NB; ++j) dcol[j] = (j > r && j < nb) ? Db[j][r] : 0.0;
#pragma unroll
    for (int j = NB - 1; j >= 0; --j) {
      const double xj = readlane_f64(v, j) * readlane_f64(dinv, j);
      if (r == j) v = xj;
      v = __builtin_fma(-dcol[j], xj, v);
    }
    if (tid < nb) x[kb + tid] = v;
    if (tid < kb) {
#pragma unroll
      for (int c = 0; c < NB; ++c) xv = __builtin_fma(-cur[c], readlane_f64(v, c), xv);
    }
#pragma unroll
    for (int c = 0; c < NB; ++c) cur[c] = nxt[c];
    buf ^= 1;
  }
  __syncthreads();
}

__device__ __forceinline__ double block_sum(double v, double* sred) {
#pragma unroll
  for (int off = 32; off > 0; off >>= 1) v += __shfl_down(v, off, 64);
  __syncthreads();
  if ((threadIdx.x & 63) == 0) sred[threadIdx.x >> 6] = v;
  __syncthreads();
  double t = 0.0;
  for (int q = 0; q < (int)(blockDim.x >> 6); ++q) t += sred[q];
  return t;
}
__device__ __forceinline__ double block_max(double v, double* sred) {
#pragma unroll
  for (int off = 32; off > 0; off >>= 1) v = fmax(v, __shfl_down(v, off, 64));
  __syncthreads();
  if ((threadIdx.x & 63) == 0) sred[threadIdx.x >> 6] = v;
  __syncthreads();
  double t = sred[0];
  for (int q = 1; q < (int)(blockDim.x >> 6); ++q) t = fmax(t, sred[q]);
  return t;
}

struct Solve16Lds {
  double Pt[4][16][17];
  double Dl[16][17];
};
__device__ __forceinline__ void blocked_lower_solve16(const double* __restrict__ Lm, int n, int jb, double* __restrict__ Xc, Solve16Lds& sh) {
  const int nblk = (n + 15) / 16;
  const int tid = threadIdx.x, lane = tid & 63, wave = tid >> 6;
  const int lr = lane & 15, lk = lane >> 4;
  constexpr int KMAX = 16;
  double la[KMAX][4];
  auto fetch = [&](int i) {
#pragma unroll
    for (int t = 0; t < KMAX; ++t) {
      const int k = jb + wave + 4 * t;
#pragma unroll
      for (int q = 0; q < 4; ++q) {
        const int row = i * 16 + lr, col = k * 16 + q * 4 + lk;
        la[t][q] = (k < i && row < n) ? Lm[(size_t)row * n + col] : 0.0;
      }
    }
  };
  for (int i = jb; i < nblk; ++i) {
    const int nb = min(16, n - i * 16);
    {
      const int r = tid >> 4, c = tid & 15;
      const int row = i * 16 + r, col = i * 16 + c;
      sh.Dl[r][c] = (c <= r && row < n) ? Lm[(size_t)row * n + col] : ((r == c) ? 1.0 : 0.0);
    }
    f64x4 acc = f64x4{0.0, 0.0, 0.0, 0.0};
    if (i > jb) {
#pragma unroll
      for (int t = 0; t < KMAX; ++t) {
        const int k = jb + wave + 4 * t;
        if (k < i) {
          const double* xk = Xc + (size_t)(k - jb) * 16 * 17;
#pragma unroll
          for (int q = 0; q < 4; ++q) acc = __builtin_amdgcn_mfma_f64_16x16x4f64(la[t][q], xk[(q * 4 + lk) * 17 + lr], acc, 0, 0, 0);
        }
      }
    }
#pragma unroll
    for (int rg = 0; rg < 4; ++rg) sh.Pt[wave][lk + 4 * rg][lr] = acc[rg];
    if (i + 1 < nblk) fetch(i + 1);
    __syncthreads();
    if (wave == 0 && lane < 16) {
      const int c = lane;
      double x[16];
      double* xi = Xc + (size_t)(i - jb) * 16 * 17;
      const double dinv = 1.0 / sh.Dl[c][c];
#pragma unroll
      for (int r = 0; r < 16; ++r) {
        const double bsum = ((sh.Pt[0][r][c] + sh.Pt[1][r][c]) + sh.Pt[2][r][c]) + sh.Pt[3][r][c];
        double v = xi[r * 17 + c] - bsum;
#pragma unroll
        for (int q = 0; q < 16; ++q)
          if (q < r) v = __builtin_fma(-sh.Dl[r][q], x[q], v);
        v = v * readlane_f64(dinv, r);
        x[r] = (r < nb) ? v : 0.0;
      }
#pragma unroll
      for (int r = 0; r < 16; ++r) xi[r * 17 + c] = x[r];
    }
    __syncthreads();
  }
}


__device__ __forceinline__ void small_gemm_tn_sym(const double* __restrict__ B, double* __restrict__ C, int S) {
  const int lane = threadIdx.x & 63, wave = threadIdx.x >> 6, nwave = (int)(blockDim.x >> 6);
  const int lr = lane & 15, lk = lane >> 4;
  const int T = (S + 15) / 16;
  for (int q = wave; q < T * (T + 1) / 2; q += nwave) {
    int tr = (int)((sqrtf(8.0f * (float)q + 1.0f) - 1.0f) * 0.5f);
    while (tr * (tr + 1) / 2 > q) --tr;
    while ((tr + 1) * (tr + 2) / 2 <= q) ++tr;
    const int tc = q - tr * (tr + 1) / 2;
    const int i = tr * 16 + lr, j = tc * 16 + lr;
    f64x4 acc = f64x4{0.0, 0.0, 0.0, 0.0};
#pragma unroll 4
    for (int k0 = tr * 16; k0 < S; k0 += 4) {
      const int k = k0 + lk;
      const double av = (k < S && i < S) ? B[(size_t)k * S + i] : 0.0;
      const double bv = (k < S && j < S) ? B[(size_t)k * S + j] : 0.0;
      acc = __builtin_amdgcn_mfma_f64_16x16x4f64(av, bv, acc, 0, 0, 0);
    }
#pragma unroll
    for (int rg = 0; rg < 4; ++rg) {
      const int r = tr * 16 + lk + 4 * rg, c = tc * 16 + lr;
      if (r < S && c < S) {
        C[(size_t)r * S + c] = acc[rg];
        C[(size_t)c * S + r] = acc[rg];
      }
    }
  }
}
__device__ __forceinline__ void small_gemm_nn(const double* __restrict__ A, const double* __restrict__ B, double* __restrict__ C, int S) {
  const int lane = threadIdx.x & 63, wave = threadIdx.x >> 6, nwave = (int)(blockDim.x >> 6);
  const int lr = lane & 15, lk = lane >> 4;
  const int T = (S + 15) / 16;
  for (int q = wave; q < T * T; q += nwave) {
    const int ti = q / T, tj = q - ti * T;
    const int i = ti * 16 + lr, j = tj * 16 + lr;
    f64x4 acc = f64x4{0.0, 0.0, 0.0, 0.0};
#pragma unroll 4
    for (int k0 = 0; k0 < S; k0 += 4) {
      const int k = k0 + lk;
      const double av = (k < S && i < S) ? A[(size_t)i * S + k] : 0.0;
      const double bv = (k < S && j < S) ? B[(size_t)k * S + j] : 0.0;
      acc = __builtin_amdgcn_mfma_f64_16x16x4f64(av, bv, acc, 0, 0, 0);
    }
#pragma unroll
    for (int rg = 0; rg < 4; ++rg) {
      const int r = ti * 16 + lk + 4 * rg, c = tj * 16 + lr;
      if (r < S && c < S) C[(size_t)r * S + c] = acc[rg];
    }
  }
}

__global__ __launch_bounds__(256) __attribute__((amdgpu_waves_per_eu(2, 2))) void gram_kernel(const UgpmWin* __restrict__ wins) {
  const WinPart wp = xcd_win_part();
  const UgpmWin w = load_win(wins, wp.win);
  if (*w.status != 0) return;
  const int c = wp.part, S = w.S;
  const double l2 = w.hyper[c * 4 + 0], sf2 = w.hyper[c * 4 + 1], sz2 = w.hyper[c * 4 + 2];
  double* A = w.Kinv + (size_t)c * S * S;
  double* B = w.KKinv + (size_t)c * S * S;
  double* Kc = w.JtJ + (size_t)c * S * S;
  const double* st = w.state_t;
  __shared__ int sflag;
  __shared__ CholLds chol;
  __shared__ Solve16Lds sh;
  const int wave = threadIdx.x >> 6, lane = threadIdx.x & 63, nwave = (int)(blockDim.x >> 6);
  for (int i = wave; i < S; i += nwave)
    for (int j = lane; j < S; j += 64) {
      const double k = se_k(st[i], st[j], l2, sf2);
      Kc[(size_t)i * S + j] = k;
      A[(size_t)i * S + j] = k + (i == j ? sz2 : 0.0);
    }
  __syncthreads();
  if (!block_cholesky(A, S, S, chol, &sflag)) {
    if (threadIdx.x == 0) *w.status = -6;
    return;
  }
  {
    double* Xc = &chol.P[0][0];
    const int nblk = (S + 15) / 16;
    for (int jb = 0; jb < nblk; ++jb) {
      const int rows = (nblk - jb) * 16;
      for (int q = threadIdx.x; q < rows * 16; q += blockDim.x) Xc[(size_t)(q >> 4) * 17 + (q & 15)] = (q >> 4) == (q & 15) ? 1.0 : 0.0;
      blocked_lower_solve16(A, S, jb, Xc, sh);
      for (int i = wave; i < S; i += nwave) {
        if (lane < 16 && jb * 16 + lane < S) B[(size_t)i * S + jb * 16 + lane] = i >= jb * 16 ? Xc[(size_t)(i - jb * 16) * 17 + lane] : 0.0;
      }
      __syncthreads();
    }
  }
  __threadfence_block();
  __syncthreads();
  small_gemm_tn_sym(B, A, S);
  __syncthreads();
  small_gemm_nn(Kc, A, B, S);
  __syncthreads();
  for (int j = wave; j < S; j += nwave) {
    double s = 0.0;
    for (int k = lane; k < S; k += 64) s += B[(size_t)j * S + k] * Kc[(size_t)j * S + k];
#pragma unroll
    for (int off = 32; off > 0; off >>= 1) s += __shfl_down(s, off, 64);
    if (lane == 0) {
      double v = -s + sf2 + sz2;
      if (v <= 0) v = sz2;
      w.var[c * S + j] = v;
      w.sstd[c * S + j] = sqrt(v);
      double wt = sqrt(1.0 / (1000.0 * v));
      if (isnan(wt)) wt = 1.0;
      w.wgp[c * S + j] = wt;
    }
  }
  if (c < 3) {
    double* Cq = w.KintKinv + (size_t)c * S * S;
    double* Ki = w.lhs + (size_t)c * S * S;
    for (int i = wave; i < S; i += nwave)
      for (int j = lane; j < S; j += 64) Ki[(size_t)i * S + j] = se_kint(w.start_t, st[i], st[j], l2, sf2);
    __syncthreads();
    small_gemm_nn(Ki, A, Cq, S);
  }
}

constexpr int kCrossRows = 32;
__global__ __launch_bounds__(256) void cross_kernel(const UgpmWin* __restrict__ wins) {
  const WinPart wp = xcd_win_part();
  const UgpmWin w = load_win(wins, wp.win);
  if (*w.status != 0) return;
  const int tab = wp.part, S = w.S;
  const int c = tab % 3, kind = tab / 3;
  const int ch = kind == 3 ? 3 + c : c;
  const int N = kind < 2 ? w.G : w.V;
  const double* tt = kind < 2 ? w.gyr_t : w.vel_t;
  double* out = (kind == 0 ? w.KsKinv : kind == 1 ? w.KsIntKinv : kind == 2 ? w.KgyrIntKinv : w.KvelKinv) + (size_t)c * N * S;
  const double* Ki = w.Kinv + (size_t)ch * S * S;
  const double l2 = w.hyper[ch * 4 + 0], sf2 = w.hyper[ch * 4 + 1];
  const bool integral = (kind == 1 || kind == 2);
  const int LDK = ((S + 31) / 32) * 32 + 4;
  extern __shared__ double ks_dyn[];
  double* ks = ks_dyn;
  const int row0 = wp.z * kCrossRows;
  if (row0 >= N) return;
  const int wave = threadIdx.x >> 6, lane = threadIdx.x & 63;
  for (int r = wave; r < kCrossRows; r += 4) {
    const int n = row0 + r;
    for (int k = lane; k < LDK; k += 64) {
      double v = 0.0;
      if (n < N && k < S) v = integral ? se_kint(w.start_t, tt[n], w.state_t[k], l2, sf2) : se_k(tt[n], w.state_t[k], l2, sf2);
      ks[(size_t)r * LDK + k] = v;
    }
  }
  __syncthreads();
  const int lr = lane & 15, lk = lane >> 4;
  const int TJ = (S + 15) / 16;
  for (int q = wave; q < 2 * TJ; q += 4) {
    const int ti = q / TJ, tj = q - ti * TJ;
    const int j = tj * 16 + lr;
    f64x4 acc = f64x4{0.0, 0.0, 0.0, 0.0};
#pragma unroll 4
    for (int k0 = 0; k0 < S; k0 += 4) {
      const int k = k0 + lk;
      const double av = ks[(size_t)(ti * 16 + lr) * LDK + k];
      const double bv = (k < S && j < S) ? Ki[(size_t)k * S + j] : 0.0;
      acc = __builtin_amdgcn_mfma_f64_16x16x4f64(av, bv, acc, 0, 0, 0);
    }
#pragma unroll
    for (int rg = 0; rg < 4; ++rg) {
      const int n = row0 + ti * 16 + lk + 4 * rg;
      if (n < N && j < S) out[(size_t)n * S + j] = acc[rg];
    }
  }
}


__device__ void jacobian_res(V3 r, V3 dr, double D[3][6]) {
  const double n2 = r.x * r.x + r.y * r.y + r.z * r.z;
  const double n = sqrt(n2);
  if (n > kExpTol) {
    const double s = sin(n), c = cos(n);
    const double A = (1.0 - c) / n2, B = (n - s) / (n2 * n);
    const double dA = (n * s - 2.0 * (1.0 - c)) / (n2 * n);
    const double dB = ((1.0 - c) * n - 3.0 * (n - s)) / (n2 * n2);
    const V3 rxd = cross(r, dr), rxrxd = cross(r, rxd);
    const double rk[3] = {r.x, r.y, r.z};
    for (int k = 0; k < 3; ++k) {
      const V3 e = v3(k == 0, k == 1, k == 2);
      const double dn = rk[k] / n;
      const V3 exd = cross(e, dr);
      const V3 t = (-dA * dn) * rxd + (-A) * exd + (dB * dn) * rxrxd + B * (cross(e, rxd) + cross(r, exd));
      D[0][k] = t.x; D[1][k] = t.y; D[2][k] = t.z;
    }
    const M3 J = Jr(r);
    for (int i = 0; i < 3; ++i)
      for (int k = 0; k < 3; ++k) D[i][3 + k] = J.m[i * 3 + k];
  } else {
    const M3 S = skew(dr);
    for (int i = 0; i < 3; ++i)
      for (int k = 0; k < 3; ++k) {
        D[i][k] = 0.5 * S.m[i * 3 + k];
        D[i][3 + k] = (i == k) ? 1.0 : 0.0;
      }
  }
}

__device__ __forceinline__ double row_dot(const double* __restrict__ row, const double* __restrict__ s, int S) {
  double t = 0.0;
  for (int j = 0; j < S; ++j) t += row[j] * s[j];
  return t;
}

__device__ __forceinline__ void wave_row_dots6(const double* __restrict__ a, size_t a_stride, const double* __restrict__ va,
                                               const double* __restrict__ b, size_t b_stride, const double* __restrict__ vb, int S, double (&out)[6]) {
  double t[6] = {0.0, 0.0, 0.0, 0.0, 0.0, 0.0};
  for (int j = threadIdx.x & 63; j < S; j += 64) {
    double ra[3], rb[3], xa[3], xb[3];
#pragma unroll
    for (int c = 0; c < 3; ++c) {
      ra[c] = a[c * a_stride + j];
      rb[c] = b[c * b_stride + j];
      xa[c] = va[(size_t)c * S + j];
      xb[c] = vb[(size_t)c * S + j];
    }
#pragma unroll
    for (int c = 0; c < 3; ++c) {
      t[c] += ra[c] * xa[c];
      t[3 + c] += rb[c] * xb[c];
    }
  }
#pragma unroll
  for (int off = 32; off > 0; off >>= 1)
#pragma unroll
    for (int q = 0; q < 6; ++q) t[q] += __shfl_xor(t[q], off, 64);
#pragma unroll
  for (int q = 0; q < 6; ++q) out[q] = t[q];
}

__device__ __forceinline__ void wave_row_dots3(const double* __restrict__ a, size_t a_stride, const double* __restrict__ va, int S, double (&out)[3]) {
  double t[3] = {0.0, 0.0, 0.0};
  for (int j = threadIdx.x & 63; j < S; j += 64) {
    double ra[3], xa[3];
#pragma unroll
    for (int c = 0; c < 3; ++c) {
      ra[c] = a[c * a_stride + j];
      xa[c] = va[(size_t)c * S + j];
    }
#pragma unroll
    for (int c = 0; c < 3; ++c) t[c] += ra[c] * xa[c];
  }
#pragma unroll
  for (int off = 32; off > 0; off >>= 1)
#pragma unroll
    for (int q = 0; q < 3; ++q) t[q] += __shfl_xor(t[q], off, 64);
#pragma unroll
  for (int q = 0; q < 3; ++q) out[q] = t[q];
}

__device__ __forceinline__ void lm_step_bookkeeping(const UgpmWin& w) {
  w.lmi[3] = 0;
  w.lmi[8] = 0;
  w.lmi[0] += 1;
}

__device__ int lm_decide_block(const UgpmWin& w, int m, int n, bool commit, double* sred ) {
  const int nblk = w.lmi[7] == 1 ? kVelBlocks : 1;
  bool step_ok = true;
  double mcc = 0.0, sn2 = 0.0;
  for (int q = 0; q < nblk; ++q) {
    step_ok = step_ok && w.lmi[9 + q] != 0;
    mcc += w.lmc[8 + q];
    sn2 += w.lmc[11 + q];
  }
  if (!(mcc > 0.0)) step_ok = false;
  const double sn = sqrt(sn2);
  if (!step_ok) {
    if (commit && threadIdx.x == 0) {
      w.lmc[2] = w.lmc[2] / w.lmc[3];
      w.lmc[3] *= 2.0;
      w.lmi[2] = 1;
    }
    return 0;
  }
  double c = 0.0;
  const int nacc = min((int)blockDim.x, 256);
  if ((int)threadIdx.x < nacc)
    for (int k = threadIdx.x; k < m; k += nacc) c += w.res_new[k] * w.res_new[k];
  const double cost_new = 0.5 * block_sum(c, sred);
  const double cost = w.lmc[0];
  const double cost_change = cost - cost_new;
  int verdict;
  double rho = 0.0;
  if (sn <= 1e-8 * (w.lmc[4] + 1e-8)) verdict = -2;
  else if (fabs(cost_change) <= 1e-10 * cost) verdict = -1;
  else {
    rho = cost_change / mcc;
    verdict = rho > 1e-3 ? 1 : 0;
  }
  __syncthreads();
  if (commit) {
    if (threadIdx.x == 0) {
      w.lmc[1] = cost_new;
      if (verdict < 0) {
        w.lmi[1] = 1;
        w.lmi[5] = verdict == -2 ? 2 : 1;
      } else if (verdict == 1) {
        w.lmi[6] += 1;
        w.lmi[3] = 1;
        w.lmc[2] = fmin(1e16, w.lmc[2] / fmax(1.0 / 3.0, 1.0 - pow(2.0 * rho - 1.0, 3)));
        w.lmc[3] = 2.0;
        w.lmi[2] = 0;
      } else {
        w.lmc[2] = w.lmc[2] / w.lmc[3];
        w.lmc[3] *= 2.0;
        w.lmi[2] = 1;
      }
    }
    if (verdict == 1)
      for (int j = threadIdx.x; j < n; j += blockDim.x) w.lmv[5 * (size_t)n + j] = w.lmv[6 * (size_t)n + j];
  }
  return verdict < 0 ? -1 : verdict;
}

__device__ void gpnorm_rows(const UgpmWin& w, int ch, const double* __restrict__ s, double* __restrict__ res, double* __restrict__ J, int ldj, int col0, bool writeJ) {
  const int S = w.S;
  const double* KK = w.KKinv + (size_t)ch * S * S;
  const double* wt = w.wgp + (size_t)ch * S;
  if ((int)blockIdx.y != ch % (int)gridDim.y) return;
  for (int i = threadIdx.x; i < S; i += blockDim.x) res[i] = (row_dot(KK + (size_t)i * S, s, S) - s[i]) * wt[i];
  if (writeJ)
    for (int q = threadIdx.x; q < S * S; q += blockDim.x) {
      const int i = q / S, j = q % S;
      J[(size_t)i * ldj + col0 + j] = (KK[(size_t)j * S + i] - (i == j ? 1.0 : 0.0)) * wt[i];
    }
}

__global__ __launch_bounds__(256) void rot_eval_kernel(const UgpmWin* __restrict__ wins, int mode) {
  const UgpmWin w = load_win(wins, blockIdx.x);
  if (*w.status != 0 || w.lmi[1]) return;
  const int S = w.S, G = w.G, n = 3 * S;
  __shared__ double sred[8];
  if ((mode == 0 || mode == 3) && blockIdx.y == 0 && threadIdx.x == 0) lm_step_bookkeeping(w);
  if (mode == 1) {
    if (lm_decide_block(w, 3 * S + 3 * G, n, blockIdx.y == 0, sred) != 1) return;
  }
  const double* x = mode == 2 ? w.lmv + 5 * (size_t)n : w.lmv + 6 * (size_t)n;
  double* res = (mode == 0 || mode == 3) ? w.res_new : w.res;
  double* J = w.Jrot;
  const int i_lo = (int)(((long)G * blockIdx.y) / gridDim.y), i_hi = (int)(((long)G * (blockIdx.y + 1)) / gridDim.y);
  if (mode == 2) {
    for (int c = 0; c < 3; ++c)
      if ((int)blockIdx.y == c % (int)gridDim.y)
        for (size_t q = threadIdx.x; q < (size_t)S * n; q += blockDim.x) J[(size_t)c * S * n + q] = 0.0;
  }
  __syncthreads();
  for (int c = 0; c < 3; ++c) gpnorm_rows(w, c, x + (size_t)c * S, res + (size_t)c * S, J + (size_t)c * S * n, n, c * S, mode == 2);
  __shared__ double sdot[256][6];
  for (int ib = i_lo; ib < i_hi; ib += 256) {
    const int cnt = min(256, i_hi - ib);
    for (int q = (int)(threadIdx.x >> 6); q < cnt; q += (int)(blockDim.x >> 6)) {
      const int i = ib + q;
      double d[6];
      wave_row_dots6(w.KsKinv + (size_t)i * S, (size_t)G * S, x, w.KsIntKinv + (size_t)i * S, (size_t)G * S, x, S, d);
      if ((threadIdx.x & 63) == 0) {
#pragma unroll
        for (int q2 = 0; q2 < 6; ++q2) sdot[q][q2] = d[q2];
      }
    }
    __syncthreads();
    for (int q = threadIdx.x; q < cnt; q += blockDim.x) {
      const int i = ib + q;
      const double drv[3] = {sdot[q][0], sdot[q][1], sdot[q][2]}, rot[3] = {sdot[q][3], sdot[q][4], sdot[q][5]};
      const double dtm = w.gyr_t[i] - w.start_t;
      const V3 rv = v3(rot[0] + dtm * w.hyper[3], rot[1] + dtm * w.hyper[7], rot[2] + dtm * w.hyper[11]);
      const V3 dv = v3(drv[0] + w.hyper[3], drv[1] + w.hyper[7], drv[2] + w.hyper[11]);
      const V3 t = mvec(Jr(rv), dv);
      double* r = res + 3 * S + 3 * i;
      r[0] = t.x - (w.gyr[i] - w.gyr_bias[0]);
      r[1] = t.y - (w.gyr[G + i] - w.gyr_bias[1]);
      r[2] = t.z - (w.gyr[2 * G + i] - w.gyr_bias[2]);
      if (mode != 0) {
        double D[3][6];
        jacobian_res(rv, dv, D);
        double* st = w.sample_tmp + (size_t)i * 24;
        for (int a = 0; a < 3; ++a)
          for (int k = 0; k < 6; ++k) st[a * 6 + k] = D[a][k];
      }
    }
    __syncthreads();
  }
  if (mode == 0) return;
// ... 110 lines not shown
  const double wgt = sqrt(1.0 / w.vel_var);
  __shared__ double sdot[256][6];
  {
    const int nmine = (G - part + kCorrJacParts - 1) / kCorrJacParts;
    for (int qb = 0; qb < nmine; qb += 256) {
      const int cnt = min(256, nmine - qb);
      for (int q = wave; q < cnt; q += 4) {
        const int i = part + kCorrJacParts * (qb + q);
        double d[6];
        wave_row_dots6(w.KsKinv + (size_t)i * S, (size_t)G * S, w.s_dr, w.KsIntKinv + (size_t)i * S, (size_t)G * S, w.s_dr, S, d);
        if (lane == 0) {
#pragma unroll
          for (int q2 = 0; q2 < 6; ++q2) sdot[q][q2] = d[q2];
        }
      }
      __syncthreads();
      for (int q = threadIdx.x; q < cnt; q += blockDim.x) {
        const int i = part + kCorrJacParts * (qb + q);
        const double dtm = w.gyr_t[i] - w.start_t;
        double D[3][6];
        jacobian_res(v3(sdot[q][3] + dtm * w.hyper[3], sdot[q][4] + dtm * w.hyper[7], sdot[q][5] + dtm * w.hyper[11]),
                     v3(sdot[q][0] + w.hyper[3], sdot[q][1] + w.hyper[7], sdot[q][2] + w.hyper[11]), D);
        double* st = w.sample_tmp_c + (size_t)i * 24;
        for (int a = 0; a < 3; ++a)
          for (int k = 0; k < 6; ++k) st[a * 6 + k] = D[a][k];
      }
      __syncthreads();
    }
  }
  __syncthreads();
  {
    const int nmine = (G - part + kCorrJacParts - 1) / kCorrJacParts;
    for (int rr = wave; rr < nmine * 3; rr += 4) {
      const int i = part + kCorrJacParts * (rr / 3), a = rr % 3;
      const double* st = w.sample_tmp_c + (size_t)i * 24;
      double* row = J + (size_t)(3 * i + a) * n;
      for (int c = 0; c < 3; ++c) {
        const double f0 = st[a * 6 + c], f1 = st[a * 6 + c + 3];
        const double* k0 = w.KsIntKinv + ((size_t)c * G + i) * S;
        const double* k1 = w.KsKinv + ((size_t)c * G + i) * S;
        for (int j = lane; j < S; j += 64) row[c * S + j] = f0 * k0[j] + f1 * k1[j];
      }
    }
  }
  __syncthreads();
  {
    const int nmine = (V - part + kCorrJacParts - 1) / kCorrJacParts;
    for (int qb = 0; qb < nmine; qb += 256) {
      const int cnt = min(256, nmine - qb);
      for (int q = wave; q < cnt; q += 4) {
        const int i = part + kCorrJacParts * (qb + q);
        double d[6];
        wave_row_dots6(w.KgyrIntKinv + (size_t)i * S, (size_t)V * S, w.s_dr, w.KvelKinv + (size_t)i * S, (size_t)V * S, w.s_vel, S, d);
        if (lane == 0) {
#pragma unroll
          for (int q2 = 0; q2 < 6; ++q2) sdot[q][q2] = d[q2];
        }
      }
      __syncthreads();
      for (int q = threadIdx.x; q < cnt; q += blockDim.x) {
        const int i = part + kCorrJacParts * (qb + q);
        const double dtm = w.vel_t[i] - w.start_t;
        const V3 rv = v3(sdot[q][0] + dtm * w.hyper[3], sdot[q][1] + dtm * w.hyper[7], sdot[q][2] + dtm * w.hyper[11]);
        const M3 RT = expMap(v3(-rv.x, -rv.y, -rv.z));
        const V3 t = mvec(RT, v3(sdot[q][3] + w.hyper[15], sdot[q][4] + w.hyper[19], sdot[q][5] + w.hyper[23]));
        const M3 dres = mmul(skew(t), Jr(rv));
        double* st = w.sample_tmp_c + (size_t)i * 24;
        storeM(st, dres);
        storeM(st + 9, RT);
      }
      __syncthreads();
    }
  }
  __syncthreads();
  {
    const int nmine = (V - part + kCorrJacParts - 1) / kCorrJacParts;
    for (int rr = wave; rr < nmine * 3; rr += 4) {
      const int i = part + kCorrJacParts * (rr / 3), a = rr % 3;
      const double* st = w.sample_tmp_c + (size_t)i * 24;
      double* row = J + (size_t)(3 * G + 3 * i + a) * n;
      for (int c = 0; c < 3; ++c) {
        const double f0 = wgt * st[a * 3 + c], f1 = wgt * st[9 + a * 3 + c];
        const double* k0 = w.KgyrIntKinv + ((size_t)c * V + i) * S;
        const double* k1 = w.KvelKinv + ((size_t)c * V + i) * S;
        for (int j = lane; j < S; j += 64) {
          row[c * S + j] = f0 * k0[j];
          row[(3 + c) * S + j] = f1 * k1[j];
        }
      }
    }
  }
}


__device__ __forceinline__ int ata_npad(int n) { return ((n + 15) / 32) * 32 + 16; }

template <int CMAX, int KC, int TPG>
__global__ __launch_bounds__(512) void ata_kernel(const UgpmWin* __restrict__ wins, int which, int n_windows, int groups_max, int decide, int dense) {
  const int L = blockIdx.x;
  const int xcd = L & 7, slot = L >> 3;
#ifdef GORIO_ATA_NO_XCD
  const int win = (slot * 8 + xcd) / groups_max, grp = (slot * 8 + xcd) % groups_max;
#else
  const bool long_first = which == 2 && !dense;
  const int nrow = (n_windows + 7) / 8;
  const int win = (long_first ? slot % nrow : slot / groups_max) * 8 + xcd, grp = long_first ? slot / nrow : slot % groups_max;
#endif
  if (win >= n_windows) return;
  const UgpmWin w = load_win(wins, win);
  if (*w.status != 0) return;
  int m, n;
  const double* A;
  double* C;
  const double* r = nullptr;
  double* g = nullptr;
  int zrows = 0, zcol = 0;
  if (which == 2) {
    if (!w.correlate) return;
    m = 3 * w.G + 3 * w.V; n = 6 * w.S; A = w.Jc; C = w.Ac;
    zrows = 3 * w.G; zcol = 3 * w.S;
  } else {
    if (w.lmi[1]) return;
    n = 3 * w.S;
    m = which == 0 ? 3 * w.S + 3 * w.G : 3 * w.V + 3 * w.S;
    A = which == 0 ? w.Jrot : w.Jvel;
    C = w.JtJ; r = w.res; g = w.lmv;
    if (decide) {
      __shared__ double sred[8];
      if (lm_decide_block(w, m, n, grp == 0, sred) != 1) return;
      r = w.res_new;
      if (grp == 0)
        for (int k = threadIdx.x; k < m; k += blockDim.x) w.res[k] = r[k];
    } else if (!w.lmi[3]) {
      return;
    }
  }
  const AtaCut cut = ata_cut(n, zrows > 0 && !dense ? zcol : n, TPG);
  const int ng = cut.groups();
  if (grp >= ng) return;
  const int q_lo = cut.q_lo(grp), q_hi = cut.q_hi(grp);
  const int npad = ata_npad(n);
  const int nck = (m + KC - 1) / KC;
  const int c_lo = cut.skips(grp) ? zrows / KC : 0, c_hi = nck;
  extern __shared__ double ata_lds[];
  double* rl = ata_lds + (size_t)2 * KC * npad;
  const int tid = threadIdx.x, lane = tid & 63, wave = __builtin_amdgcn_readfirstlane(tid >> 6);
  const int lr = lane & 15, lk = lane >> 4;
  constexpr int NT = TPG / 8;
  int trofs[NT], tcofs[NT], qv[NT];
#pragma unroll
  for (int t = 0; t < NT; ++t) {
    const int q = min(q_lo + wave + 8 * t, q_hi - 1);
    int tr = (int)((sqrtf(8.0f * (float)q + 1.0f) - 1.0f) * 0.5f);
    while (tr * (tr + 1) / 2 > q) --tr;
    while ((tr + 1) * (tr + 2) / 2 <= q) ++tr;
    qv[t] = __builtin_amdgcn_readfirstlane(q);
    trofs[t] = __builtin_amdgcn_readfirstlane(tr) * 16;
    tcofs[t] = __builtin_amdgcn_readfirstlane(q - tr * (tr + 1) / 2) * 16;
  }
  const int nt = max(0, min(NT, (q_hi - q_lo - wave + 7) / 8));
  f64x4 acc[NT];
#pragma unroll
  for (int t = 0; t < NT; ++t) acc[t] = f64x4{0.0, 0.0, 0.0, 0.0};
  double gacc = 0.0;
  const int gj0 = (int)((long)grp * n / ng), gj1 = (int)((long)(grp + 1) * n / ng);
  const int gcolw = ((gj1 - gj0 + 63) / 64) * 64;
  const int gparts = gcolw <= 64 ? 8 : (gcolw <= 128 ? 4 : (gcolw <= 256 ? 2 : 1));
  const int gpart = (int)threadIdx.x / gcolw, gj = gj0 + (int)threadIdx.x % gcolw;
  const bool gcol = g != nullptr && gpart < gparts && gj < gj1;
  constexpr int RMAX = KC / 8;
  double pre[RMAX][CMAX];
  double rpre = 0.0;
  auto fetch = [&](int ck) {
#pragma unroll
    for (int rr = 0; rr < RMAX; ++rr) {
      const int k = ck * KC + wave + 8 * rr;
      const int ncol = k < zrows ? zcol : n;
#pragma unroll
      for (int cc = 0; cc < CMAX; ++cc) {
        const int col = lane + 64 * cc;
        pre[rr][cc] = (k < m && col < ncol) ? A[(size_t)k * n + col] : 0.0;
      }
    }
    if (r != nullptr && tid < KC) rpre = (ck * KC + tid < m) ? r[ck * KC + tid] : 0.0;
  };
  auto stash = [&](int buf) {
    double* dst = ata_lds + (size_t)buf * KC * npad;
#pragma unroll
    for (int rr = 0; rr < RMAX; ++rr) {
      const int row = wave + 8 * rr;
#pragma unroll
      for (int cc = 0; cc < CMAX; ++cc) {
        const int col = lane + 64 * cc;
        if (col < npad) dst[row * npad + col] = pre[rr][cc];
      }
    }
    if (tid < KC) rl[buf * KC + tid] = rpre;
  };
  CHOL_T_INIT;
  if (c_lo < c_hi) {
    fetch(c_lo);
    stash(0);
  }
  __syncthreads();
  CHOL_T(0);
  for (int ck = c_lo; ck < c_hi; ++ck) {
    const int buf = (ck - c_lo) & 1;
    if (ck + 1 < c_hi) fetch(ck + 1);
    const double* src = ata_lds + (size_t)buf * KC * npad;
#pragma unroll
    for (int kk = 0; kk < KC; kk += 4) {
      const double* rowp = src + (kk + lk) * npad + lr;
      double av[NT], bv[NT];
#pragma unroll
      for (int t = 0; t < NT; ++t) {
        av[t] = rowp[trofs[t]];
        bv[t] = rowp[tcofs[t]];
      }
#pragma unroll
      for (int t = 0; t < NT; ++t) acc[t] = __builtin_amdgcn_mfma_f64_16x16x4f64(av[t], bv[t], acc[t], 0, 0, 0);
    }
    CHOL_T(1);
    if (gcol) {
      for (int kk = gpart; kk < KC; kk += gparts) gacc += src[kk * npad + gj] * rl[buf * KC + kk];
    }
    CHOL_T(2);
    if (ck + 1 < c_hi) stash(buf ^ 1);
    CHOL_T(3);
    __syncthreads();
    CHOL_T(4);
  }
  {
#pragma unroll
    for (int t = 0; t < NT; ++t) {
      if (t < nt) {
#pragma unroll
        for (int rg = 0; rg < 4; ++rg) {
          const int i = trofs[t] + lk + 4 * rg, j = tcofs[t] + lr;
          if (i < n && j < n) {
            C[(size_t)i * n + j] = acc[t][rg];
            C[(size_t)j * n + i] = acc[t][rg];
          }
        }
      }
    }
    if (g != nullptr) {
      __syncthreads();
      if (gpart < gparts) ata_lds[gpart * gcolw + (int)threadIdx.x % gcolw] = gcol ? gacc : 0.0;
      __syncthreads();
      if (tid < gj1 - gj0) {
        double v = 0.0;
        for (int q = 0; q < gparts; ++q) v += ata_lds[q * gcolw + tid];
        g[gj0 + tid] = v;
      }
    }
  }
  CHOL_T(7);
}

__global__ __launch_bounds__(256) void lm_relinearize_linear_kernel(const UgpmWin* __restrict__ wins) {
  const UgpmWin w = load_win(wins, blockIdx.x);
  if (*w.status != 0 || w.lmi[1]) return;
  const int n = 3 * w.S, m = 3 * w.V + 3 * w.S;
  const int j0 = blockIdx.y * 64;
  if (j0 >= n) return;
  __shared__ double sred[8];
  if (lm_decide_block(w, m, n, blockIdx.y == 0, sred) != 1) return;
  const double* J = w.Jvel;
  const double* rn = w.res_new;
  __shared__ double sg[4][64];
  if (blockIdx.y == 0)
    for (int k = threadIdx.x; k < m; k += blockDim.x) w.res[k] = rn[k];
  const int slice = threadIdx.x >> 6, lane = threadIdx.x & 63;
  const int j = j0 + lane;
  double acc[4] = {0.0, 0.0, 0.0, 0.0};
  if (j < n) {
    int k = slice;
    for (; k + 12 < m; k += 16) {
#pragma unroll
      for (int u = 0; u < 4; ++u) acc[u] += J[(size_t)(k + 4 * u) * n + j] * rn[k + 4 * u];
    }
    for (; k < m; k += 4) acc[0] += J[(size_t)k * n + j] * rn[k];
  }
  sg[slice][lane] = (acc[0] + acc[1]) + (acc[2] + acc[3]);
  __syncthreads();
  if (slice == 0 && j < n) w.lmv[j] = (sg[0][lane] + sg[1][lane]) + (sg[2][lane] + sg[3][lane]);
}


__device__ void lm_begin_block(const UgpmWin& w, int problem) {
  const int n = 3 * w.S;
  const double* src = problem == 0 ? w.s_dr : w.s_vel;
  for (int j = threadIdx.x; j < n; j += blockDim.x) w.lmv[5 * (size_t)n + j] = src[j];
  if (threadIdx.x == 0) {
    for (int q = 0; q < 16; ++q) w.lmi[q] = 0;
    w.lmi[3] = 1;
    w.lmi[7] = problem;
    w.lmi[8] = 1;
    w.lmc[2] = 1e4;
    w.lmc[3] = 2.0;
  }
}

__global__ __launch_bounds__(512) void lm_step_kernel(const UgpmWin* __restrict__ wins) {
  const UgpmWin w = load_win(wins, blockIdx.x);
  if (*w.status != 0 || w.lmi[1]) return;
  const int n = 3 * w.S;
  const int problem = w.lmi[7];
  const int m = problem == 0 ? 3 * w.S + 3 * w.G : 3 * w.V + 3 * w.S;
  const int nblk = (int)gridDim.y, blk = (int)blockIdx.y;
  const int j0 = (int)((long)n * blk / nblk), j1 = (int)((long)n * (blk + 1) / nblk), ns = j1 - j0;
  double* g = w.lmv;
  double* scale = w.lmv + (size_t)n;
  double* diag = w.lmv + 2 * (size_t)n;
  double* step = w.lmv + 3 * (size_t)n;
  double* delta = w.lmv + 4 * (size_t)n;
  double* x = w.lmv + 5 * (size_t)n;
  double* xn = w.lmv + 6 * (size_t)n;
  __shared__ double sred[8];
  __shared__ int sflag;
  __shared__ CholLds chol;
  if (w.lmi[3]) {
    double c = 0.0;
    for (int k = threadIdx.x; k < m; k += blockDim.x) c += w.res[k] * w.res[k];
    c = 0.5 * block_sum(c, sred);
    double gm = 0.0, xn2 = 0.0;
    for (int j = threadIdx.x; j < n; j += blockDim.x) {
      gm = fmax(gm, fabs(g[j]));
      xn2 += x[j] * x[j];
    }
    gm = block_max(gm, sred);
    xn2 = block_sum(xn2, sred);
    if (w.lmi[8])
      for (int j = j0 + (int)threadIdx.x; j < j1; j += blockDim.x) scale[j] = 1.0 / (1.0 + sqrt(w.JtJ[(size_t)j * n + j]));
    __syncthreads();
    if (threadIdx.x == 0) {
      w.lmc[0] = c;
      w.lmc[4] = sqrt(xn2);
      if (w.lmi[8]) w.lmc[7] = c;
      if (gm <= 1e-10) {
        w.lmi[1] = 1;
        w.lmi[5] = 3;
      }
    }
    if (gm <= 1e-10) return;
  }
  if (w.lmi[0] >= 50) {
    if (threadIdx.x == 0) { w.lmi[1] = 1; w.lmi[5] = 4; }
    return;
  }
  const double radius = w.lmc[2];
  if (radius < 1e-32) {
    if (threadIdx.x == 0) { w.lmi[1] = 1; w.lmi[5] = 5; }
    return;
  }
  if (!w.lmi[2])
    for (int j = j0 + (int)threadIdx.x; j < j1; j += blockDim.x) diag[j] = fmin(fmax(w.JtJ[(size_t)j * n + j] * scale[j] * scale[j], 1e-6), 1e32);
  __syncthreads();
  double* L = w.lhs + (size_t)j0 * n + j0;
  __shared__ double xs[kCholMaxN / 2];
  const bool fused = ns < 384 && ns <= (int)blockDim.x && ns <= kCholMaxN / 2;
  for (int i = threadIdx.x >> 6; i < ns; i += (int)(blockDim.x >> 6)) {
    const double si = scale[j0 + i];
    for (int j = threadIdx.x & 63; j <= i; j += 64)
      L[(size_t)i * n + j] = w.JtJ[(size_t)(j0 + i) * n + j0 + j] * si * scale[j0 + j] + (i == j ? diag[j0 + i] / radius : 0.0);
  }
  double* rhs = w.lmv + 7 * (size_t)n + j0;
  for (int j = threadIdx.x; j < ns; j += blockDim.x) {
    step[j0 + j] = g[j0 + j] * scale[j0 + j];
    if (fused) rhs[j] = g[j0 + j] * scale[j0 + j];
  }
  __syncthreads();
  bool valid = block_cholesky(L, ns, n, chol, &sflag, fused ? rhs : nullptr);
  if (valid) {
    if (fused) {
      for (int j = threadIdx.x; j < ns; j += blockDim.x) xs[j] = rhs[j];
      __syncthreads();
      block_backward(L, ns, n, xs, chol);
      for (int j = threadIdx.x; j < ns; j += blockDim.x) step[j0 + j] = xs[j];
    } else {
      double* xp = &chol.P[0][0];
      for (int j = threadIdx.x; j < ns; j += blockDim.x) xp[j] = step[j0 + j];
      __syncthreads();
      if (threadIdx.x < 64) {
        wave_forward<1>(L, ns, n, xp, 1, 0);
        wave_backward(L, ns, n, xp);
      }
      __syncthreads();
      for (int j = threadIdx.x; j < ns; j += blockDim.x) step[j0 + j] = xp[j];
    }
    __syncthreads();
    double bad = 0.0;
    for (int j = j0 + (int)threadIdx.x; j < j1; j += blockDim.x) {
      step[j] = -step[j];
      if (!isfinite(step[j])) bad = 1.0;
      delta[j] = step[j] * scale[j];
    }
    bad = block_max(bad, sred);
    valid = bad == 0.0;
  }
  double mcc = 0.0, sn2 = 0.0;
  if (valid) {
    double acc = 0.0;
    for (int i = j0 + (int)(threadIdx.x >> 6); i < j1; i += (int)(blockDim.x >> 6)) {
      const double hi = 0.5 * delta[i];
      for (int j = j0 + (int)(threadIdx.x & 63); j < j1; j += 64) acc += hi * w.JtJ[(size_t)i * n + j] * delta[j];
    }
    for (int i = j0 + (int)threadIdx.x; i < j1; i += blockDim.x) {
      acc += delta[i] * g[i];
      sn2 += delta[i] * delta[i];
      xn[i] = x[i] + delta[i];
    }
    mcc = -block_sum(acc, sred);
    sn2 = block_sum(sn2, sred);
  }
  if (threadIdx.x == 0) {
    w.lmi[9 + blk] = valid ? 1 : 0;
    w.lmc[8 + blk] = mcc;
    w.lmc[11 + blk] = sn2;
  }
}


__device__ bool lm_end_block(const UgpmWin& w, int problem, double* __restrict__ diag_out) {
  if (!w.lmi[1]) {
    __syncthreads();
    if (threadIdx.x == 0) *w.status = kStatusUnfinished;
    return false;
  }
  const int n = 3 * w.S;
  double* dst = problem == 0 ? w.s_dr : w.s_vel;
  for (int j = threadIdx.x; j < n; j += blockDim.x) dst[j] = w.lmv[5 * (size_t)n + j];
  if (threadIdx.x == 0) {
    diag_out[problem * 2 + 0] = (double)w.lmi[0];
    diag_out[problem * 2 + 1] = w.lmc[0];
    w.lmi[kLmiNeed + problem] = w.lmi[0] + (w.lmi[5] >= 3 ? 1 : 0);
  }
  return true;
}

__global__ __launch_bounds__(256) void lm_turn_kernel(const UgpmWin* __restrict__ wins, double* __restrict__ diag_out ) {
  const UgpmWin w = load_win(wins, blockIdx.x);
  if (*w.status != 0) return;
  if (!lm_end_block(w, 0, diag_out + 4 * (size_t)blockIdx.x)) return;
  __syncthreads();
  lm_begin_block(w, 1);
}


__global__ __launch_bounds__(512) void corr_factor_kernel(const UgpmWin* __restrict__ wins) {
  const UgpmWin w = load_win(wins, blockIdx.x);
  if (*w.status != 0 || !w.correlate) return;
  const int n = 6 * w.S;
  __shared__ int sflag;
  __shared__ CholLds chol;
  for (int i = threadIdx.x; i < n; i += blockDim.x) w.Ac[(size_t)i * n + i] += 0.00001;
  __syncthreads();
  if (!block_cholesky(w.Ac, n, n, chol, &sflag)) {
    if (threadIdx.x == 0) *w.status = -6;
    return;
  }
}

__global__ __launch_bounds__(256) __attribute__((amdgpu_waves_per_eu(2, 2))) void corr_diag_kernel(const UgpmWin* __restrict__ wins) {
  const WinPart wp = xcd_win_part();
  const UgpmWin w = load_win(wins, wp.win);
  if (*w.status != 0 || !w.correlate) return;
  const int n = 6 * w.S;
  const int jb = wp.part, j0 = jb * 16;
  if (j0 >= n) return;
  extern __shared__ double Xc[];
  __shared__ Solve16Lds sh;
  {
    const int rows = ((n + 15) / 16 - jb) * 16;
    for (int q = threadIdx.x; q < rows * 16; q += blockDim.x) Xc[(size_t)(q >> 4) * 17 + (q & 15)] = (q >> 4) == (q & 15) ? 1.0 : 0.0;
  }
  blocked_lower_solve16(w.Ac, n, jb, Xc, sh);
  if (threadIdx.x < 16) {
    const int c = threadIdx.x, col = j0 + c;
    const int rows = ((n + 15) / 16 - jb) * 16;
    double ssq = 0.0;
    for (int r = 0; r < rows; ++r) ssq = __builtin_fma(Xc[(size_t)r * 17 + c], Xc[(size_t)r * 17 + c], ssq);
    if (col < n) w.dsc[col] = w.sstd[col] * (1.0 / sqrt(ssq));
  }
}


__global__ __launch_bounds__(256) void finish_kernel(const UgpmWin* __restrict__ wins, double* __restrict__ diag_out ) {
  const UgpmWin w = load_win(wins, blockIdx.x);
  if (*w.status != 0) return;
  if (!lm_end_block(w, 1, diag_out + 4 * (size_t)blockIdx.x)) return;
  __syncthreads();
  const int S = w.S;
  for (int q = threadIdx.x; q < 6 * S; q += blockDim.x) {
    const int c = q / S, i = q % S;
    const double* s = c < 3 ? w.s_dr + (size_t)c * S : w.s_vel + (size_t)(c - 3) * S;
    w.alpha[q] = row_dot(w.Kinv + ((size_t)c * S + i) * S, s, S);
  }
  for (int q = threadIdx.x; q < 3 * S; q += blockDim.x) {
    const int a = q / S, i = q % S;
    w.state_r[q] = row_dot(w.KintKinv + ((size_t)a * S + i) * S, w.s_dr + (size_t)a * S, S) + (w.state_t[i] - w.start_t) * w.hyper[a * 4 + 3];
  }
  __syncthreads();
  for (int i = threadIdx.x; i < S; i += blockDim.x) {
    const V3 ri = v3(w.state_r[i], w.state_r[S + i], w.state_r[2 * S + i]);
    const M3 Ji = JrInv(ri);
    const V3 d_r = mvec(Ji, load3(w.d_r_dt_local + (size_t)i * 3));
    const V3 temp_r = ri + mvec(Ji, load3(w.delta_r_time + (size_t)i * 3));
    const V3 dd = (1.0 / kDt) * (mvec(JrInv(temp_r), load3(w.d_r_dt_local_shift + (size_t)i * 3)) - d_r);
    w.d_d_r_dt[i] = dd.x; w.d_d_r_dt[S + i] = dd.y; w.d_d_r_dt[2 * S + i] = dd.z;
    for (int ax = 0; ax < 3; ++ax) {
      const V3 trw = ri + mvec(Ji, load3(w.delta_r_bw + ((size_t)ax * S + i) * 3));
      const V3 t = (1.0 / kBw) * (mvec(JrInv(trw), load3(w.d_r_bw_local_shift + ((size_t)ax * S + i) * 3)) - d_r);
      w.d_state_bw[((size_t)0 * S + i) * 3 + ax] = t.x;
      w.d_state_bw[((size_t)1 * S + i) * 3 + ax] = t.y;
      w.d_state_bw[((size_t)2 * S + i) * 3 + ax] = t.z;
    }
  }
  __syncthreads();
  __shared__ double srd[3];
  if (threadIdx.x < 3) {
    const int c = threadIdx.x;
    double s = 0.0;
    for (int j = 0; j < S; ++j) s += se_kint(w.start_t, w.start_t + kDt, w.state_t[j], w.hyper[c * 4], w.hyper[c * 4 + 1]) * w.alpha[c * S + j];
    srd[c] = s + kDt * w.hyper[c * 4 + 3];
  }
  __syncthreads();
  const M3 dRt = mtr(expMap(v3(srd[0], srd[1], srd[2])));
  const V3 mean_vel = v3(w.hyper[15], w.hyper[19], w.hyper[23]);
  for (int i = threadIdx.x; i < S; i += blockDim.x) {
    const V3 ri = v3(w.state_r[i], w.state_r[S + i], w.state_r[2 * S + i]);
    const M3 R = expMap(ri);
    M3 drbw;
    for (int a = 0; a < 3; ++a)
      for (int c = 0; c < 3; ++c) {
        double s = 0.0;
        const double* row = w.KintKinv + ((size_t)a * S + i) * S;
        for (int j = 0; j < S; ++j) s += row[j] * w.d_state_bw[((size_t)a * S + j) * 3 + c];
        drbw.m[a * 3 + c] = s;
      }
    const V3 sv = v3(w.s_vel[i], w.s_vel[S + i], w.s_vel[2 * S + i]) + mean_vel;
    const M3 dvbw = mmul(mmul(skew(sv), Jr(v3(-ri.x, -ri.y, -ri.z))), drbw);
    const V3 dvdt = (1.0 / kDt) * (mvec(dRt, sv) - sv);
    const double dv[3] = {dvdt.x, dvdt.y, dvdt.z};
    for (int a = 0; a < 3; ++a) {
      for (int c = 0; c < 3; ++c) {
        w.d_vel_bv[((size_t)a * S + i) * 3 + c] = R.m[a * 3 + c];
        w.d_vel_bw[((size_t)a * S + i) * 3 + c] = -dvbw.m[a * 3 + c];
      }
      w.d_vel_dt[a * S + i] = dv[a];
    }
  }
}

__global__ __launch_bounds__(256) void infer_kernel(const UgpmWin* __restrict__ wins) {
  const WinPart wp = xcd_win_part();
  const UgpmWin w = load_win(wins, wp.win);
  const int qi = wp.part;
  if (qi >= w.n_infer) return;
  double* out = w.out + (size_t)qi * 83;
  if (*w.status != 0) {
    for (int k = threadIdx.x; k < 83; k += blockDim.x) out[k] = __longlong_as_double(0x7ff8000000000000LL);
    return;
  }
  const int S = w.S, n = 6 * S;
  const double t = w.infer_t[qi], dt = t - w.start_t;
  __shared__ double ksv[6][160];
  __shared__ double ksd[3][160];
  __shared__ double ksK[6][160];
  __shared__ double sval[6][8];
  __shared__ double sval2[6][4];
  __shared__ double sred[8];
  __shared__ double scov[36];
  for (int q = threadIdx.x; q < 6 * S; q += blockDim.x) {
    const int c = q / S, j = q - c * S;
    ksv[c][j] = se_kint(w.start_t, t, w.state_t[j], w.hyper[c * 4], w.hyper[c * 4 + 1]);
    if (c >= 3) ksd[c - 3][j] = se_kint_dt(w.start_t, t, w.state_t[j], w.hyper[c * 4], w.hyper[c * 4 + 1]);
  }
  __syncthreads();
  for (int q = threadIdx.x; q < 6 * S; q += blockDim.x) {
    const int c = q / S, j = q - c * S;
    const double* Kc = w.Kinv + (size_t)c * S * S + j;
    double s = 0.0;
    for (int k = 0; k < S; ++k) s += ksv[c][k] * Kc[(size_t)k * S];
    ksK[c][j] = s;
  }
  __syncthreads();
  {
    const int wv = threadIdx.x >> 6, lane = threadIdx.x & 63;
    for (int c = wv; c < 6; c += (int)(blockDim.x >> 6)) {
      double acc[9] = {0, 0, 0, 0, 0, 0, 0, 0, 0};
      for (int j = lane; j < S; j += 64) {
        const double ks = ksv[c][j], kk = ksK[c][j];
        acc[0] += ks * w.alpha[c * S + j];
        acc[1] += kk * ks;
        if (c < 3) {
          acc[2] += kk * w.d_d_r_dt[c * S + j];
          for (int q = 0; q < 3; ++q) acc[3 + q] += kk * w.d_state_bw[((size_t)c * S + j) * 3 + q];
        } else {
          acc[2] += ksd[c - 3][j] * w.alpha[c * S + j] + kk * w.d_vel_dt[(c - 3) * S + j];
          for (int q = 0; q < 3; ++q) {
            acc[3 + q] += kk * w.d_vel_bw[((size_t)(c - 3) * S + j) * 3 + q];
            acc[6 + q] += kk * w.d_vel_bv[((size_t)(c - 3) * S + j) * 3 + q];
          }
        }
      }
#pragma unroll
      for (int v = 0; v < 9; ++v)
#pragma unroll
        for (int off = 32; off > 0; off >>= 1) acc[v] += __shfl_down(acc[v], off, 64);
      if (lane == 0) {
        const double l2 = w.hyper[c * 4], sf2 = w.hyper[c * 4 + 1];
        double var = kss_int(w.start_t, t, l2, sf2) - acc[1];
        if (var <= 0) var = dt * dt * w.hyper[c * 4 + 2];
        sval[c][0] = acc[0] + dt * w.hyper[c * 4 + 3];
        sval[c][1] = var;
        sval[c][2] = acc[2];
        for (int q = 0; q < 3; ++q) {
          sval[c][3 + q] = acc[3 + q];
          sval2[c][q] = acc[6 + q];
        }
      }
    }
  }
  __syncthreads();
  if (w.correlate) {
    extern __shared__ double Xc[];
    __shared__ Solve16Lds sh;
    const int rows = ((n + 15) / 16) * 16;
    for (int q = threadIdx.x; q < rows * 16; q += blockDim.x) Xc[(size_t)(q >> 4) * 17 + (q & 15)] = 0.0;
    __syncthreads();
    for (int row = threadIdx.x; row < n; row += blockDim.x) {
      const int c = row / S;
      Xc[(size_t)row * 17 + c] = w.dsc[row] * ksK[c][row - c * S];
    }
    blocked_lower_solve16(w.Ac, n, 0, Xc, sh);
    for (int pair = 0; pair < 21; ++pair) {
      int a2 = 0, b2 = pair;
      while (b2 >= 6 - a2) { b2 -= 6 - a2; ++a2; }
      b2 += a2;
      double acc = 0.0;
      for (int k = threadIdx.x; k < rows; k += blockDim.x) acc += Xc[(size_t)k * 17 + a2] * Xc[(size_t)k * 17 + b2];
      acc = block_sum(acc, sred);
      if (threadIdx.x == 0) {
        scov[a2 * 6 + b2] = acc;
        scov[b2 * 6 + a2] = acc;
      }
    }
  } else {
    if (threadIdx.x < 36) scov[threadIdx.x] = 0.0;
    __syncthreads();
    if (threadIdx.x < 6) {
      const int a2 = threadIdx.x;
      double s2 = 0.0;
      for (int j = 0; j < S; ++j) s2 += ksK[a2][j] * w.var[a2 * S + j] * ksK[a2][j];
      scov[a2 * 6 + a2] = s2;
    }
  }
  __syncthreads();
  if (threadIdx.x == 0) {
    const V3 r = v3(sval[0][0], sval[1][0], sval[2][0]);
    const M3 jr = Jr(r);
    const M3 R = expMap(r);
    M3 d_r_dw, d_p_dw, d_p_dv;
    for (int a = 0; a < 3; ++a)
      for (int q = 0; q < 3; ++q) {
        d_r_dw.m[a * 3 + q] = sval[a][3 + q];
        d_p_dw.m[a * 3 + q] = sval[3 + a][3 + q];
        d_p_dv.m[a * 3 + q] = sval2[3 + a][q];
      }
    storeM(out, R);
    out[9] = sval[3][0]; out[10] = sval[4][0]; out[11] = sval[5][0];
    out[12] = dt;
    out[13] = 0.5 * dt * dt;
    double cov[36], td[6];
    for (int a = 0; a < 6; ++a) td[a] = sqrt(sval[a][1]) * (1.0 / sqrt(scov[a * 6 + a]));
    for (int a = 0; a < 6; ++a)
      for (int b = 0; b < 6; ++b) cov[a * 6 + b] = scov[a * 6 + b] * td[a] * td[b];
    M3 c00, c03;
    for (int a = 0; a < 3; ++a)
      for (int b = 0; b < 3; ++b) {
        c00.m[a * 3 + b] = cov[a * 6 + b];
        c03.m[a * 3 + b] = cov[a * 6 + 3 + b];
      }
    const M3 n00 = mmul(mmul(jr, c00), mtr(jr)), n03 = mmul(jr, c03);
    for (int a = 0; a < 3; ++a)
      for (int b = 0; b < 3; ++b) {
        cov[a * 6 + b] = n00.m[a * 3 + b];
        cov[a * 6 + 3 + b] = n03.m[a * 3 + b];
        cov[(3 + b) * 6 + a] = n03.m[a * 3 + b];
      }
    if (w.vel_bias_std > 0.0 || w.gyr_bias_std > 0.0) {
      double J[36];
      for (int q = 0; q < 36; ++q) J[q] = 0.0;
      const double g2 = w.gyr_bias_std * w.gyr_bias_std, v2 = w.vel_bias_std * w.vel_bias_std;
      const double bc[6] = {g2, g2, g2, v2, v2, v2};
      for (int a = 0; a < 3; ++a) {
        J[a * 6 + a] = 1.0;
        for (int b = 0; b < 3; ++b) {
          J[(3 + a) * 6 + b] = d_p_dw.m[a * 3 + b];
          J[(3 + a) * 6 + 3 + b] = d_p_dv.m[a * 3 + b];
        }
      }
      for (int a = 0; a < 6; ++a)
        for (int b = 0; b < 6; ++b) {
          double s = 0.0;
          for (int k = 0; k < 6; ++k) s += J[a * 6 + k] * bc[k] * J[b * 6 + k];
          cov[a * 6 + b] += s;
        }
    }
    for (int q = 0; q < 36; ++q) out[14 + q] = cov[q];
    storeM(out + 50, mmul(jr, d_r_dw));
    store3(out + 59, mvec(jr, v3(sval[0][2], sval[1][2], sval[2][2])));
    storeM(out + 62, d_p_dw);
    storeM(out + 71, d_p_dv);
    out[80] = sval[3][2]; out[81] = sval[4][2]; out[82] = sval[5][2];
  }
}

}
}
```

### go-rio_amd/csrc/ugpm_windows.h

```cpp
#pragma once

#include <algorithm>
#include <cmath>
#include <string>
#include <vector>

#include "../../include/gorio_ugpm.h"
#include "ugpm_device.h"

namespace gorio {
namespace windows {

struct HostWin {
  int g0 = 0, G = 0, v0 = 0, V = 0, S = 0;
  double state_freq = 0;
  std::vector<double> state_t;
  int status = 0;
  size_t ws_doubles = 0;
  bool is_lpm = false;
};

inline void slice(const double* t, int n, double from, double to, int& i0, int& cnt) {
  i0 = 0;
  cnt = 0;
  if (from >= to || n <= 0) return;
  for (int i = 0; i < n; ++i) {
    if (!(t[i] > from)) continue;
    if (!(t[i] < to)) break;
    if (cnt++ == 0) i0 = i;
  }
}

inline size_t input_doubles(const gorio_ugpm_window& w, const HostWin& h) { return (size_t)h.G * 4 + (size_t)h.V * 4 + (size_t)w.n_infer + (size_t)h.S; }
inline size_t input_slot(const gorio_ugpm_window& w, const HostWin& h) { return (input_doubles(w, h) + 3) / 4 * 4; }

template <typename T>
T* take_at(T* base, size_t& off, size_t cnt) {
  T* r = base ? base + off : nullptr;
  off += cnt;
  return r;
}

inline size_t carve(const gorio_ugpm_window& w, const HostWin& h, UgpmWin& u, double* base, double* in, double* outp) {
  size_t used = 0, used_in = 0;
  auto take = [&](size_t cnt) { return take_at(base, used, cnt); };
  auto take_in = [&](size_t cnt) { return take_at(in, used_in, cnt); };
  const size_t S = h.S, G = h.G, V = h.V, n = 3 * S, mrot = 3 * S + 3 * G, mvel = 3 * V + 3 * S, mc = 3 * G + 3 * V, nc = 6 * S;
  u.gyr_t = take_in(G); u.gyr = take_in(3 * G); u.vel_t = take_in(V); u.vel = take_in(3 * V); u.infer_t = take_in(w.n_infer); u.state_t = take_in(S);
  u.Rq = take(5 * 2 * S * 9); u.Rstart = take(5 * 9); u.velr = take(3 * V); u.dp = take(2 * S * 3); u.r0 = take(5 * S * 3); u.r1 = take(5 * S * 3);
  u.s_dr = take(3 * S); u.s_vel = take(3 * S); u.hyper = take(24);
  u.d_r_dt_local = take(S * 3); u.d_r_dt_local_shift = take(S * 3); u.delta_r_time = take(S * 3); u.delta_r_bw = take(3 * S * 3); u.d_r_bw_local_shift = take(3 * S * 3);
  u.Kinv = take(6 * S * S); u.KKinv = take(6 * S * S); u.KintKinv = take(3 * S * S); u.var = take(6 * S); u.wgp = take(6 * S); u.sstd = take(6 * S);
  u.KsKinv = take(3 * G * S); u.KsIntKinv = take(3 * G * S); u.KgyrIntKinv = take(3 * V * S); u.KvelKinv = take(3 * V * S);
  u.Jrot = take(mrot * n); u.Jvel = take(mvel * n); u.res = take(std::max(mrot, mvel)); u.res_new = take(std::max(mrot, mvel));
  u.JtJ = take(n * n); u.lhs = take(n * n); u.lmv = take(8 * n); u.sample_tmp = take(std::max(G, V) * 24); u.sample_tmp_c = take(std::max(G, V) * 24);
  if (w.correlate) { u.Jc = take(mc * nc); u.Ac = take(nc * nc); }
  u.dsc = take(nc);
  u.alpha = take(6 * S); u.state_r = take(3 * S); u.d_state_bw = take(3 * S * 3); u.d_d_r_dt = take(3 * S); u.d_vel_bv = take(3 * S * 3); u.d_vel_bw = take(3 * S * 3);
  u.d_vel_dt = take(3 * S); u.out = outp; u.lmc = take(16);
  return (used + 31) / 32 * 32;
}

inline int plan_window(const gorio_ugpm_window& w, HostWin& h, std::string& err) {
  auto fail = [&](int code, const char* m) {
    err = m;
    return h.status = code;
  };
  if (!w.gyr_t || !w.gyr || !w.vel_t || !w.vel || !w.infer_t || w.n_infer <= 0) return fail(GORIO_UGPM_ERR_INVALID, "null pointers or no inference time");
  if (w.quantum >= 0) return fail(GORIO_UGPM_ERR_INVALID, "a chunked request reached the device path");
  if (w.type != GORIO_UGPM_TYPE_UGPM && w.type != GORIO_UGPM_TYPE_LPM) return fail(GORIO_UGPM_ERR_INVALID, "unknown pre-integration type");
  if (w.n_gyr < 2 || w.n_vel < 2) return fail(GORIO_UGPM_ERR_RANGE, "InterpolateLinear: this function need at least 2 data points to interpolate");
  if (w.group_sizes && w.n_groups > 0) {
    long tot = 0;
    for (int g = 0; g < w.n_groups; ++g) tot += w.group_sizes[g] < 0 ? -(1L << 40) : w.group_sizes[g];
    if (tot != w.n_infer) return fail(GORIO_UGPM_ERR_INVALID, "group_sizes do not add up to n_infer");
  }
  if (w.type == GORIO_UGPM_TYPE_LPM) {
    if (!(w.min_freq > 0.0)) return fail(GORIO_UGPM_ERR_INVALID, "min_freq must be positive");
    bool any = false;
    for (int j = 0; j < w.n_infer; ++j) any = any || (w.infer_t[j] >= w.start_t);
    if (!any) return fail(GORIO_UGPM_ERR_RANGE, "FullLPM: the start_time is not in the query domain");
    h.is_lpm = true;
    h.G = w.n_gyr;
    h.V = w.n_vel;
    return 0;
  }
  const double vel_freq = (w.n_vel - 1) / (w.vel_t[w.n_vel - 1] - w.vel_t[0]);
  const double gyr_freq = (w.n_gyr - 1) / (w.gyr_t[w.n_gyr - 1] - w.gyr_t[0]);
  const double duration = *std::max_element(w.infer_t, w.infer_t + w.n_infer) - w.start_t;
  if (!(duration > 0.0) || !std::isfinite(duration)) return fail(GORIO_UGPM_ERR_ARGUMENT, "inference time is not after start_t");
  double sf = std::max(w.state_freq, 5.0 / duration);
  sf = std::min(sf, std::min(vel_freq, gyr_freq));
  h.state_freq = sf;
  h.S = (int)(std::ceil(duration * sf) + (2 * w.overlap));
  if (h.S < 2 * w.overlap + 1 || h.S > 160) return fail(GORIO_UGPM_ERR_UNSUPPORTED, "number of GP states outside [2 overlap + 1, 160]");
  h.state_t.resize(h.S);
  const double t0 = w.start_t - (((double)w.overlap) / sf);
  for (int k = 0; k < h.S; ++k) h.state_t[k] = t0 + ((double)k) / sf;
  if (!(h.state_t[0] <= h.state_t.back())) return fail(GORIO_UGPM_ERR_ARGUMENT, "The argument of GyroVelData::Get are not consistent");
  slice(w.gyr_t, w.n_gyr, h.state_t[0], h.state_t.back(), h.g0, h.G);
  slice(w.vel_t, w.n_vel, h.state_t[0], h.state_t.back(), h.v0, h.V);
  if (h.G < 2 || h.V < 2) return fail(GORIO_UGPM_ERR_RANGE, "fewer than 2 gyro / velocity samples inside the state window");
  UgpmWin dummy;
  h.ws_doubles = carve(w, h, dummy, nullptr, nullptr, nullptr);
  return 0;
}

inline double* stage_samples(double* dst, const gorio_ugpm_window& w, int g0, size_t G, int v0, size_t V) {
  for (size_t k = 0; k < G; ++k) dst[k] = w.gyr_t[g0 + k];
  dst += G;
  for (int a = 0; a < 3; ++a)
    for (size_t k = 0; k < G; ++k) dst[a * G + k] = w.gyr[3 * (size_t)(g0 + k) + a];
  dst += 3 * G;
  for (size_t k = 0; k < V; ++k) dst[k] = w.vel_t[v0 + k];
  dst += V;
  for (int a = 0; a < 3; ++a)
    for (size_t k = 0; k < V; ++k) dst[a * V + k] = w.vel[3 * (size_t)(v0 + k) + a];
  dst += 3 * V;
  for (int k = 0; k < w.n_infer; ++k) dst[k] = w.infer_t[k];
  return dst + w.n_infer;
}

template <typename Win>
void copy_noise_and_priors(const gorio_ugpm_window& w, Win& u) {
  u.start_t = w.start_t; u.gyr_var = w.gyr_var; u.vel_var = w.vel_var;
  for (int a = 0; a < 3; ++a) { u.gyr_bias[a] = w.gyr_bias[a]; u.vel_bias[a] = w.vel_bias[a]; }
  u.vel_bias_std = w.vel_bias_std; u.gyr_bias_std = w.gyr_bias_std;
}

struct FitOutcome {
  std::vector<int> rerun;
  int need[2] = {0, 0};
};

inline FitOutcome fit_outcome(const int* ints, const std::vector<HostWin>& hw) {
  FitOutcome o;
  for (size_t i = 0; i < hw.size(); ++i) {
    if (hw[i].status != 0 || hw[i].is_lpm) continue;
    const int* f = ints + kWinInts * i;
    if (f[16] == kStatusUnfinished) o.rerun.push_back((int)i);
    if (f[16] != 0) continue;
    for (int p = 0; p < 2; ++p) o.need[p] = std::max(o.need[p], f[kLmiNeed + p]);
  }
  return o;
}

struct LpmHost {
  std::vector<double> tl;
  std::vector<int> kind, kidx, qpos, qorder, qrot;
  int start_index = 0, dt_index = 0;
};

inline void build_lpm_timeline(const gorio_ugpm_window& w, LpmHost& L) {
  struct Stamp { double t; int kind, idx; };
  std::vector<Stamp> st;
  st.reserve((size_t)w.n_infer + 2 + w.n_vel);
  for (int j = 0; j < w.n_infer; ++j) st.push_back({w.infer_t[j], 0, j});
  st.push_back({w.start_t, 1, 0});
  st.push_back({w.start_t + 0.01, 1, 1});
  for (int i = 0; i < w.n_vel; ++i) st.push_back({w.vel_t[i], 2, i});
  auto by_time = [](const Stamp& a, const Stamp& b) { return a.t < b.t; };
  std::stable_sort(st.begin(), st.end(), by_time);
  if (st.size() >= 2 && (st.back().t - st[st.size() - 2].t) > (1.0 / w.min_freq)) {
    const double first = st.front().t, last = st.back().t;
    const int nb = (int)std::floor((last - first) * w.min_freq);
    if (nb > 0) {
      const double quantum = (last - first) / ((double)nb);
      for (int i = 0; i < nb; ++i) st.push_back({first + (i * quantum), 3, i});
      std::stable_sort(st.begin(), st.end(), by_time);
    }
  }
  const size_t T = st.size();
  L.tl.resize(T); L.kind.resize(T); L.kidx.resize(T);
  L.qpos.assign(w.n_infer, 0);
  L.qorder.clear();
  for (size_t r = 0; r < T; ++r) {
    L.tl[r] = st[r].t; L.kind[r] = st[r].kind; L.kidx[r] = st[r].idx;
    if (st[r].kind == 0) { L.qpos[st[r].idx] = (int)r; L.qorder.push_back(st[r].idx); }
    if (st[r].kind == 1 && st[r].idx == 0) L.start_index = (int)r;
    if (st[r].kind == 1 && st[r].idx == 1) L.dt_index = (int)r;
  }
  L.qrot.assign(w.n_infer, 0);
  std::vector<int> group_of(w.n_infer, 0), first_of_group(1, 0);
  if (w.group_sizes && w.n_groups > 0) {
    int o = 0;
    first_of_group.clear();
    for (int g = 0; g < w.n_groups; ++g) {
      first_of_group.push_back(o);
      for (int k = 0; k < w.group_sizes[g] && o < w.n_infer; ++k) group_of[o++] = g;
    }
  }
  std::vector<int> filled(first_of_group.size(), 0);
  for (size_t r = 0; r < T; ++r)
    if (st[r].kind == 0) {
      const int g = group_of[st[r].idx];
      L.qrot[first_of_group[g] + filled[g]++] = (int)r;
    }
}

struct LpmSize {
  size_t in = 0, scratch = 0, ints = 0;
};

template <typename LpmWin>
LpmSize carve_lpm(const gorio_ugpm_window& w, size_t T, LpmWin& u, const double* in, double* scratch, const int* ints) {
  LpmSize used;
  auto take_in = [&](size_t cnt) { return take_at(in, used.in, cnt); };
  auto take = [&](size_t cnt) { return take_at(scratch, used.scratch, cnt); };
  auto take_int = [&](size_t cnt) { return take_at(ints, used.ints, cnt); };
  const size_t G = w.n_gyr, V = w.n_vel, Q = w.n_infer;
  u.gyr_t = take_in(G); u.gyr = take_in(3 * G); u.vel_t = take_in(V); u.vel = take_in(3 * V); u.infer_t = take_in(Q); u.tl = take_in(T);
  u.kind = take_int(T); u.kidx = take_int(T); u.qpos = take_int(Q); u.qorder = take_int(Q); u.qrot = take_int(Q);
  u.E = take(45 * T); u.B = take(9 * T); u.cov3 = take(9 * T); u.dRdt = take(3 * T); u.dRdbw = take(9 * T);
  u.velr = take(3 * V); u.d_bw = take(18 * V); u.d_dt = take(3 * V); u.dp_shift = take(3 * Q);
  return used;
}

inline void stage_lpm_tables(int* dst, const LpmHost& L) {
  for (const std::vector<int>* v : {&L.kind, &L.kidx, &L.qpos, &L.qorder, &L.qrot}) dst = std::copy(v->begin(), v->end(), dst);
}

}
}
```

### go-rio_amd/ugpm.py

```python
import ctypes as C

import numpy as np

from .apd import GorioError, load_library

LPM, UGPM = 0, 1
REC = 83

UGPM_SYMBOLS = ["gorio_ugpm_default_window", "gorio_ugpm_preint_batch", "gorio_ugpm_last_error", "gorio_ugpm_get_stage_times", "gorio_ugpm_debug_set_schedule",
                "gorio_ugpm_debug_set_path",                 "gorio_ugpm_combine_preints"]


class UgpmWindow(C.Structure):

    _fields_ = [
        ("gyr_t", C.c_void_p), ("gyr", C.c_void_p), ("n_gyr", C.c_int),
        ("vel_t", C.c_void_p), ("vel", C.c_void_p), ("n_vel", C.c_int),
        ("gyr_var", C.c_double), ("vel_var", C.c_double), ("start_t", C.c_double),
        ("infer_t", C.c_void_p), ("n_infer", C.c_int), ("type", C.c_int),
        ("min_freq", C.c_double), ("quantum", C.c_double), ("state_freq", C.c_double),
        ("correlate", C.c_int), ("overlap", C.c_int),
        ("gyr_bias", C.c_double * 3), ("vel_bias", C.c_double * 3),
        ("vel_bias_std", C.c_double), ("gyr_bias_std", C.c_double),
        ("group_sizes", C.c_void_p), ("n_groups", C.c_int),
    ]


class UgpmDiag(C.Structure):
    _fields_ = [("nb_state", C.c_int), ("nb_gyr", C.c_int), ("nb_vel", C.c_int), ("iters_rot", C.c_int), ("iters_vel", C.c_int), ("status", C.c_int),
                ("cost_rot", C.c_double), ("cost_vel", C.c_double), ("state_freq", C.c_double)]


def _dp(a):
    return a.__array_interface__["data"][0]


def unpack(rec):
    rec = np.asarray(rec)
    return dict(
        delta_R=rec[0:9].reshape(3, 3).copy(), delta_p=rec[9:12].copy(), dt=float(rec[12]), dt_sq_half=float(rec[13]),
        cov=rec[14:50].reshape(6, 6).copy(), d_delta_R_d_bw=rec[50:59].reshape(3, 3).copy(), d_delta_R_d_t=rec[59:62].copy(),
        d_delta_p_d_bw=rec[62:71].reshape(3, 3).copy(), d_delta_p_d_bv=rec[71:80].reshape(3, 3).copy(), d_delta_p_d_t=rec[80:83].copy())


class UgpmBatch:

    def __init__(self, windows, device=0, infer_t=None, type=UGPM, state_freq=50.0, correlate=True, overlap=8, quantum=-1.0, min_freq=500.0,
                 gyr_bias=None, vel_bias=None, vel_bias_std=0.0, gyr_bias_std=0.0, groups=None):
        lib = load_library()
        lib.gorio_ugpm_last_error.restype = C.c_char_p
        n = len(windows)
        self.n, self.device = n, int(device)
        self.arr = (UgpmWindow * n)()
        self.keep = []
        self.counts = []
        for i, w in enumerate(windows):
            lib.gorio_ugpm_default_window(C.byref(self.arr[i]))
            gt = np.ascontiguousarray(w["gyr_t"], np.float64)
            g = np.ascontiguousarray(w["gyr"], np.float64)
            vt = np.ascontiguousarray(w["vel_t"], np.float64)
            v = np.ascontiguousarray(w["vel"], np.float64)
            q = np.ascontiguousarray([w["end_t"]] if infer_t is None else infer_t[i], np.float64)
            self.keep += [gt, g, vt, v, q]
            a = self.arr[i]
            a.gyr_t, a.gyr, a.n_gyr = _dp(gt), _dp(g), len(gt)
            a.vel_t, a.vel, a.n_vel = _dp(vt), _dp(v), len(vt)
            a.gyr_var, a.vel_var, a.start_t = w["gyr_var"], w["vel_var"], w["start_t"]
            a.infer_t, a.n_infer = _dp(q), len(q)
            a.type, a.min_freq, a.state_freq = int(type), min_freq, state_freq
            a.quantum = float(quantum[i]) if np.ndim(quantum) > 0 else float(quantum)
            a.correlate, a.overlap = int(bool(correlate)), int(overlap)
            for k in range(3):
                a.gyr_bias[k] = 0.0 if gyr_bias is None else float(gyr_bias[k])
                a.vel_bias[k] = 0.0 if vel_bias is None else float(vel_bias[k])
            a.vel_bias_std, a.gyr_bias_std = vel_bias_std, gyr_bias_std
            if groups is not None and groups[i] is not None:
                gs = np.ascontiguousarray(groups[i], np.int32)
                assert int(gs.sum()) == len(q)
                self.keep.append(gs)
                a.group_sizes, a.n_groups = gs.__array_interface__["data"][0], len(gs)
            self.counts.append(len(q))
        self.out = np.zeros((sum(self.counts), REC))
        self.diag = (UgpmDiag * n)()

    def run(self):
        lib = load_library()
        rc = lib.gorio_ugpm_preint_batch(self.arr, self.n, C.c_void_p(_dp(self.out)), self.diag, self.device)
        if rc < 0:
            msg = lib.gorio_ugpm_last_error()
            raise GorioError(rc, msg.decode() if msg else "")
        return self.out

    def results(self):
        res, k = [], 0
        for cnt in self.counts:
            res.append([unpack(self.out[k + j]) for j in range(cnt)])
            k += cnt
        return res

    def diagnostics(self):
        return [dict(nb_state=d.nb_state, nb_gyr=d.nb_gyr, nb_vel=d.nb_vel, iters_rot=d.iters_rot, iters_vel=d.iters_vel, status=d.status,
                     cost_rot=d.cost_rot, cost_vel=d.cost_vel, state_freq=d.state_freq) for d in self.diag]


def ugpm_preint_batch(windows, device=0, infer_t=None, type=UGPM, state_freq=50.0, correlate=True, overlap=8, quantum=-1.0, min_freq=500.0,
                      gyr_bias=None, vel_bias=None, vel_bias_std=0.0, gyr_bias_std=0.0, return_diag=False, groups=None):
    b = UgpmBatch(windows, device=device, infer_t=infer_t, type=type, state_freq=state_freq, correlate=correlate, overlap=overlap, quantum=quantum,
                  min_freq=min_freq, gyr_bias=gyr_bias, vel_bias=vel_bias, vel_bias_std=vel_bias_std, gyr_bias_std=gyr_bias_std, groups=groups)
    b.run()
    if return_diag:
        return b.results(), b.diagnostics()
    return b.results()


def pack(m):
    return np.concatenate([np.asarray(m["delta_R"], np.float64).ravel(), np.asarray(m["delta_p"], np.float64), [m["dt"], m["dt_sq_half"]],
                           np.asarray(m["cov"], np.float64).ravel(), np.asarray(m["d_delta_R_d_bw"], np.float64).ravel(), np.asarray(m["d_delta_R_d_t"], np.float64),
                           np.asarray(m["d_delta_p_d_bw"], np.float64).ravel(), np.asarray(m["d_delta_p_d_bv"], np.float64).ravel(), np.asarray(m["d_delta_p_d_t"], np.float64)])


def ugpm_combine_preints(prev, cur):
    lib = load_library()
    a, b, out = np.ascontiguousarray(pack(prev)), np.ascontiguousarray(pack(cur)), np.zeros(REC)
    lib.gorio_ugpm_combine_preints.argtypes = [C.c_void_p, C.c_void_p, C.c_void_p]
    rc = lib.gorio_ugpm_combine_preints(C.c_void_p(_dp(a)), C.c_void_p(_dp(b)), C.c_void_p(_dp(out)))
    if rc < 0:
        raise GorioError(rc, lib.gorio_ugpm_last_error().decode())
    return unpack(out)


def ugpm_debug_set_schedule(speculative_rot=True):
    lib = load_library()
    lib.gorio_ugpm_debug_set_schedule.argtypes = [C.c_int]
    lib.gorio_ugpm_debug_set_schedule.restype = None
    lib.gorio_ugpm_debug_set_schedule(1 if speculative_rot else 0)


def ugpm_debug_set_path(dense_ata=False, draining_looks=False):
    lib = load_library()
    lib.gorio_ugpm_debug_set_path.argtypes = [C.c_int]
    lib.gorio_ugpm_debug_set_path.restype = None
    lib.gorio_ugpm_debug_set_path((1 if dense_ata else 0) | (2 if draining_looks else 0))


def ugpm_stage_times():
    lib = load_library()
    s = (C.c_double * 8)()
    c = (C.c_int * 8)()
    lib.gorio_ugpm_get_stage_times(s, c)
    return list(s), list(c)


class PreintOption:

    def __init__(self, min_freq=500.0, type=UGPM, quantum=-1.0, state_freq=50.0, correlate=True):
        self.min_freq, self.type, self.quantum, self.state_freq, self.correlate = min_freq, type, quantum, state_freq, correlate


class PreintPrior:

    def __init__(self, vel_bias=(0.0, 0.0, 0.0), gyr_bias=(0.0, 0.0, 0.0)):
        self.vel_bias, self.gyr_bias = list(vel_bias), list(gyr_bias)


class VelPreintegration:

    def __init__(self, imu_data, start_t, infer_t, opt=None, prior=None, rot_only=False, overlap=8, device=0):
        opt = opt or PreintOption()
        prior = prior or PreintPrior()
        if np.isscalar(infer_t):
            self._kind, groups = "single", [[float(infer_t)]]
        elif len(infer_t) and np.isscalar(infer_t[0]):
            self._kind, groups = "vec", [list(map(float, infer_t))]
        else:
            self._kind, groups = "vecvec", [list(map(float, g)) for g in infer_t]
        flat = [t for g in groups for t in g]
        win = dict(imu_data)
        win["start_t"] = start_t
        self._args = dict(device=device, infer_t=[flat], type=opt.type, state_freq=opt.state_freq, correlate=opt.correlate, overlap=overlap,
                          quantum=opt.quantum, min_freq=opt.min_freq, gyr_bias=prior.gyr_bias, vel_bias=prior.vel_bias,
                          groups=[[len(g) for g in groups]])
        self._win = win
        self._groups = groups
        self._prior = prior
        self._cache = {}

    def _compute(self, vel_bias_std, gyr_bias_std):
        key = (vel_bias_std, gyr_bias_std)
        if key not in self._cache:
            flat = ugpm_preint_batch([self._win], vel_bias_std=vel_bias_std, gyr_bias_std=gyr_bias_std, **self._args)[0]
            out, k = [], 0
            for g in self._groups:
                out.append(flat[k:k + len(g)])
                k += len(g)
            self._cache[key] = out
        return self._cache[key]

    def get(self, *idx, vel_bias_std=0.3, gyr_bias_std=0.03):
        pre = self._compute(vel_bias_std, gyr_bias_std)
        if len(idx) == 2:
            i, j = idx
        elif len(idx) == 1:
            if self._kind != "vec":
                raise IndexError("VelPreintegration::get: The type of query does not math the type of constructor")
            i, j = 0, idx[0]
        else:
            if self._kind != "single":
                raise IndexError("VelPreintegration::get: The type of query does not math the type of constructor")
            i, j = 0, 0
        if not (0 <= i < len(pre) and 0 <= j < len(pre[i])):
            raise IndexError("VelPreintegration::get: Trying to get precomputed preintegrated measurements (wrong index query?)")
        return pre[i][j]

    def getPrior(self):
        return self._prior
```

Baseline: 179,200 linearisations/s.

## Template GP solver kernels on LDS rows and register KMAX, select small sizes

Templates the Cholesky LDS struct, the gram, LM-step, corr_diag and infer kernels on panel-row capacity and solve-block count. The host then picks smaller instantiations when the batch's state count fits, so a 66-state window uses less shared memory and fewer registers, which can raise occupancy. Separately, the APD linearisation kernel now loads the per-point label and geometric weight only on the APD path and only for matched points. The cost is more kernel instantiations, host dispatch logic, and a debug flag that forces full capacity.

```diff
diff --git a/go-rio_amd/csrc/apd_kernels.hip b/go-rio_amd/csrc/apd_kernels.hip
--- a/go-rio_amd/csrc/apd_kernels.hip
+++ b/go-rio_amd/csrc/apd_kernels.hip
@@ -437,8 +437,6 @@
     typedef const __attribute__((address_space(1))) float* g_f32p;
     const unsigned long long key = ((g_u64p)pd.best_key)[i];
     const float ax = ((g_f32p)pd.src.x)[i], ay = ((g_f32p)pd.src.y)[i], az = ((g_f32p)pd.src.z)[i];
-    const float src_label = ((g_f32p)pd.src.label)[i];
-    const double src_geo_w = ((g_f64p)pd.src.geo_w)[i];
     double cA[6];
 #pragma unroll
     for (int t = 0; t < 6; ++t) cA[t] = ((g_f64p)pd.src.cov6)[(size_t)i * 6 + t];
@@ -459,7 +457,6 @@
       const v4f_lin t4 = ((const __attribute__((address_space(1))) v4f_lin*)pd.tgt.p4)[jj];
       tb = make_float4(t4.x, t4.y, t4.z, t4.w);
     }
-    double* om = pd.omega6 + (size_t)i * 6;
     if (j >= 0) {
 #pragma clang fp contract(fast)
       double T[12];
@@ -525,7 +522,14 @@
       const double q22 = cB[5] + (M20 * R20 + M21 * R21 + M22 * R22);
       PointTerms p;
       inv_sym3(q00, q01, q02, q11, q12, q22, p.o00, p.o01, p.o02, p.o11, p.o12, p.o22);
+      double src_geo_w = 0.0;
+      float src_label = 0.0f;
+      if constexpr (METHOD == kMethodApd) {
+        src_geo_w = ((g_f64p)pd.src.geo_w)[i];
+        src_label = ((g_f32p)pd.src.label)[i];
+      }
       if (pd.write_omega) {
+        double* om = pd.omega6 + (size_t)i * 6;
         om[0] = p.o00; om[1] = p.o01; om[2] = p.o02; om[3] = p.o11; om[4] = p.o12; om[5] = p.o22;
       }
 
@@ -558,6 +562,7 @@
       acc[24] = -oe0; acc[25] = -oe1; acc[26] = -oe2;
     } else {
       if (pd.write_omega) {
+        double* om = pd.omega6 + (size_t)i * 6;
         om[0] = 0; om[1] = 0; om[2] = 0; om[3] = 0; om[4] = 0; om[5] = 0;
       }
     }
diff --git a/go-rio_amd/csrc/ugpm_api.hip b/go-rio_amd/csrc/ugpm_api.hip
--- a/go-rio_amd/csrc/ugpm_api.hip
+++ b/go-rio_amd/csrc/ugpm_api.hip
@@ -172,8 +172,10 @@
   UHIP(hipSetDevice(device));
   if (c.device == device) return 0;
   if (int rc = make_stream_pair(c.main)) return rc;
-  UHIP(hipFuncSetAttribute(reinterpret_cast<const void*>(&ug::corr_diag_kernel), hipFuncAttributeMaxDynamicSharedMemorySize, 140 * 1024));
-  UHIP(hipFuncSetAttribute(reinterpret_cast<const void*>(&ug::infer_kernel), hipFuncAttributeMaxDynamicSharedMemorySize, 17 * (6 * 160 + 16) * 8) );
+  UHIP(hipFuncSetAttribute(reinterpret_cast<const void*>(&ug::corr_diag_kernel<kSolveKmaxSmall>), hipFuncAttributeMaxDynamicSharedMemorySize, 140 * 1024));
+  UHIP(hipFuncSetAttribute(reinterpret_cast<const void*>(&ug::corr_diag_kernel<kSolveKmaxFull>), hipFuncAttributeMaxDynamicSharedMemorySize, 140 * 1024));
+  UHIP(hipFuncSetAttribute(reinterpret_cast<const void*>(&ug::infer_kernel<kSolveKmaxSmall>), hipFuncAttributeMaxDynamicSharedMemorySize, 17 * (6 * 160 + 16) * 8));
+  UHIP(hipFuncSetAttribute(reinterpret_cast<const void*>(&ug::infer_kernel<kSolveKmaxFull>), hipFuncAttributeMaxDynamicSharedMemorySize, 17 * (6 * 160 + 16) * 8) );
   const void* fns[] = {reinterpret_cast<const void*>(&ug::ata_kernel<4, 16, kAtaTilesCorr>), reinterpret_cast<const void*>(&ug::ata_kernel<8, 16, kAtaTilesCorr>),
                        reinterpret_cast<const void*>(&ug::ata_kernel<16, 8, kAtaTilesCorr>), reinterpret_cast<const void*>(&ug::ata_kernel<4, 16, kAtaTilesLm>),
                        reinterpret_cast<const void*>(&ug::ata_kernel<8, 16, kAtaTilesLm>)};
@@ -367,8 +369,38 @@
   }
 }
 
+SolverSizes batch_sizes(const Batch& b) { return solver_sizes(b.max_S, (g_debug_path.load() & 4) != 0); }
+
+void launch_gram(const Run& r, const SolverSizes& z) {
+  const dim3 grid(6, r.nw);
+  if (z.gram_rows == kGramRowsSmall) ug::gram_kernel<kGramRowsSmall, kGramKmax><<<grid, 256, 0, r.s>>>(r.wins);
+  else if (z.gram_rows == kGramRows) ug::gram_kernel<kGramRows, kGramKmax><<<grid, 256, 0, r.s>>>(r.wins);
+  else ug::gram_kernel<kCholRowsFull, kSolveKmaxFull><<<grid, 256, 0, r.s>>>(r.wins);
+}
+
+void launch_lm_step(const Run& r, const SolverSizes& z, int problem) {
+  const dim3 grid(r.nw, problem == 1 ? kVelBlocks : 1);
+  if (z.lm_rows == kLmRowsSmall) ug::lm_step_kernel<kLmRowsSmall><<<grid, 512, 0, r.s>>>(r.wins);
+  else ug::lm_step_kernel<kCholRowsFull><<<grid, 512, 0, r.s>>>(r.wins);
+}
+
+void launch_corr_diag(const Run& r, const SolverSizes& z, int max_S) {
+  const dim3 grid((6 * max_S + 15) / 16, r.nw);
+  const size_t lds = sizeof(double) * 17 * (6 * max_S + 16);
+  if (z.solve_kmax == kSolveKmaxSmall) ug::corr_diag_kernel<kSolveKmaxSmall><<<grid, 256, lds, r.s2>>>(r.wins);
+  else ug::corr_diag_kernel<kSolveKmaxFull><<<grid, 256, lds, r.s2>>>(r.wins);
+}
+
+void launch_infer(const Run& r, const SolverSizes& z, int max_S, int max_infer) {
+  const dim3 grid(std::max(1, max_infer), r.nw);
+  const size_t lds = sizeof(double) * 17 * (6 * max_S + 16);
+  if (z.solve_kmax == kSolveKmaxSmall) ug::infer_kernel<kSolveKmaxSmall><<<grid, 256, lds, r.s>>>(r.wins);
+  else ug::infer_kernel<kSolveKmaxFull><<<grid, 256, lds, r.s>>>(r.wins);
+}
+
 int enqueue_tables_and_correlation(Ctx& c, Batch& b) {
   const int max_S = b.max_S;
+  const SolverSizes sizes = batch_sizes(b);
   for (const Run& r : b.runs) {
     {
       Stage st(c, 0, r.s);
@@ -377,7 +409,7 @@
     }
     {
       Stage st(c, 1, r.s);
-      ug::gram_kernel<<<dim3(6, r.nw), 256, 0, r.s>>>(r.wins);
+      launch_gram(r, sizes);
       ug::cross_kernel<<<dim3(12, r.nw, (std::max(b.max_G, b.max_V) + ug::kCrossRows - 1) / ug::kCrossRows), 256, sizeof(double) * ug::kCrossRows * (((max_S + 31) / 32) * 32 + 4), r.s>>>(r.wins);
     }
     UHIP(hipEventRecord(r.ev_tab, r.s));
@@ -388,7 +420,7 @@
       UHIP(hipEventRecord(r.ev_jac, r.s2));
       launch_ata(c, max_S, r, 2);
       ug::corr_factor_kernel<<<r.nw, 512, 0, r.s2>>>(r.wins);
-      ug::corr_diag_kernel<<<dim3((6 * max_S + 15) / 16, r.nw), 256, sizeof(double) * 17 * (6 * max_S + 16), r.s2>>>(r.wins);
+      launch_corr_diag(r, sizes, max_S);
     }
     UHIP(hipEventRecord(r.ev_corr, r.s2));
   }
@@ -397,6 +429,7 @@
 
 int run_fit(Ctx& c, Batch& b, int problem) {
   const int max_S = b.max_S;
+  const SolverSizes sizes = batch_sizes(b);
   std::vector<int>& flags = b.flags;
   const bool lmtrace = std::getenv("GORIO_UGPM_LMTRACE") != nullptr;
   const bool speculative = g_speculative_rot.load() != 0;
@@ -413,7 +446,7 @@
     for (Run& r : b.runs) {
       if (!r.active) continue;
       any = true;
-      ug::lm_step_kernel<<<dim3(r.nw, problem == 1 ? kVelBlocks : 1), 512, 0, r.s>>>(r.wins);
+      launch_lm_step(r, sizes, problem);
       if (problem == 0 && speculative) {
         ug::rot_eval_kernel<<<dim3(r.nw, kEvalSplit), 256, 0, r.s>>>(r.wins, 3);
         launch_ata(c, max_S, r, problem, 1);
@@ -481,12 +514,13 @@
 }
 
 int enqueue_finish_and_infer(Ctx& c, Batch& b) {
+  const SolverSizes sizes = batch_sizes(b);
   for (const Run& r : b.runs) {
     UHIP(hipStreamWaitEvent(r.s, r.ev_corr, 0));
     {
       Stage st(c, 4, r.s);
       ug::finish_kernel<<<r.nw, 256, 0, r.s>>>(r.wins, c.d_diag + 4 * (size_t)r.g0);
-      ug::infer_kernel<<<dim3(std::max(1, b.max_infer), r.nw), 256, sizeof(double) * 17 * (6 * b.max_S + 16), r.s>>>(r.wins);
+      launch_infer(r, sizes, b.max_S, b.max_infer);
     }
     UHIP(hipEventRecord(r.ev_done, r.s));
   }
diff --git a/go-rio_amd/csrc/ugpm_device.h b/go-rio_amd/csrc/ugpm_device.h
--- a/go-rio_amd/csrc/ugpm_device.h
+++ b/go-rio_amd/csrc/ugpm_device.h
@@ -7,6 +7,7 @@
 constexpr int kWinInts = 48;
 constexpr int kLmiNeed = 18;
 constexpr int kStatusUnfinished = 2;
+constexpr int kCholRowsFull = 384;
 constexpr int kVelBlocks = 3;
 
 #if defined(__HIPCC__)
diff --git a/go-rio_amd/csrc/ugpm_kernels.hip b/go-rio_amd/csrc/ugpm_kernels.hip
--- a/go-rio_amd/csrc/ugpm_kernels.hip
+++ b/go-rio_amd/csrc/ugpm_kernels.hip
@@ -637,13 +637,14 @@
 #define CHOL_T_VMWAIT do { } while (0)
 #endif
 typedef double f64x4 __attribute__((ext_vector_type(4)));
+template <int ROWS>
 struct CholLds {
   double D[2][kCholNB][kCholNB + 1];
   double Dinv[2][kCholNB];
   double Dt[kCholNB][kCholNB + 1];
-  double dinv_n[384];
+  double dinv_n[ROWS + kCholNB < kCholRowsFull ? ROWS + kCholNB : kCholRowsFull];
   unsigned short tile[328];
-  double P[kCholMaxN > 384 ? 384 : kCholMaxN][kCholNB + 1];
+  double P[ROWS][kCholNB + 1];
 };
 
 __device__ __forceinline__ double readlane_f64(double v, int lane) {
@@ -663,7 +664,8 @@
   return y;
 }
 
-__device__ __forceinline__ bool block_cholesky(double* __restrict__ A, int n, int lda, CholLds& L, int* __restrict__ sflag, double* __restrict__ rhs = nullptr) {
+template <int ROWS>
+__device__ __forceinline__ bool block_cholesky(double* __restrict__ A, int n, int lda, CholLds<ROWS>& L, int* __restrict__ sflag, double* __restrict__ rhs = nullptr) {
   constexpr int NB = kCholNB;
   const int tid = threadIdx.x, lane = tid & 63, wave = tid >> 6, nwave = (int)(blockDim.x >> 6);
   if (tid == 0) *sflag = 0;
@@ -675,7 +677,7 @@
   }
   __syncthreads();
   CHOL_T_INIT;
-  const bool la = n - min(NB, n) + (rhs != nullptr ? 1 : 0) <= 384 && nwave >= 2;
+  const bool la = n - min(NB, n) + (rhs != nullptr ? 1 : 0) <= ROWS && nwave >= 2;
   int cur = 0;
   auto factor_block = [&](double (&a)[NB], int kbd, int nbd, int buf) {
     const int r = lane;
@@ -713,7 +715,7 @@
     const int me = m + (rhs != nullptr ? 1 : 0);
     auto panel_row = [&](int i) -> double* { return (rhs != nullptr && i == m) ? rhs + kb : A + (size_t)(kb + nb + i) * lda + kb; };
     double x[NB];
-    const bool own = tid < min(me, 384);
+    const bool own = tid < min(me, ROWS);
     auto load_row = [&](const double* arow) {
 #pragma unroll
       for (int c = 0; c < NB; ++c) x[c] = c < nb ? arow[c] : 0.0;
@@ -736,8 +738,8 @@
     }
     if (*sflag) return false;
     if (me <= 0) break;
-    for (int p0 = 0; p0 < me; p0 += 384) {
-      const int mp = min(384, me - p0);
+    for (int p0 = 0; p0 < me; p0 += ROWS) {
+      const int mp = min(ROWS, me - p0);
       for (int i = tid; i < mp; i += blockDim.x) {
         double* arow = panel_row(p0 + i);
         if (!(p0 == 0 && i == tid)) load_row(arow);
@@ -843,7 +845,7 @@
           }
         }
       }
-      if (p0 != 0 || me > 384) {
+      if (p0 != 0 || me > ROWS) {
         for (long q = tid; q < (long)mp * m; q += blockDim.x) {
           const int i = p0 + (int)(q / m), k = (int)(q % m);
           if (k > i || (p0 == 0 && k < mp)) continue;
@@ -905,7 +907,9 @@
   }
 }
 
-__device__ __forceinline__ void block_backward(const double* __restrict__ Lm, int n, int lda, double* __restrict__ x, CholLds& C) {
+template <int ROWS>
+__device__ __forceinline__ void block_backward(const double* __restrict__ Lm, int n, int lda, double* __restrict__ x, CholLds<ROWS>& C) {
+  static_assert(ROWS >= 2 * (kCholNB + 1), "two staging buffers of 17 panel rows");
   constexpr int NB = kCholNB;
   const int tid = threadIdx.x, lane = tid & 63;
   double cur[NB], nxt[NB];
@@ -977,11 +981,11 @@
   double Pt[4][16][17];
   double Dl[16][17];
 };
+template <int KMAX>
 __device__ __forceinline__ void blocked_lower_solve16(const double* __restrict__ Lm, int n, int jb, double* __restrict__ Xc, Solve16Lds& sh) {
   const int nblk = (n + 15) / 16;
   const int tid = threadIdx.x, lane = tid & 63, wave = tid >> 6;
   const int lr = lane & 15, lk = lane >> 4;
-  constexpr int KMAX = 16;
   double la[KMAX][4];
   auto fetch = [&](int i) {
 #pragma unroll
@@ -1091,6 +1095,7 @@
   }
 }
 
+template <int ROWS, int KMAX>
 __global__ __launch_bounds__(256) __attribute__((amdgpu_waves_per_eu(2, 2))) void gram_kernel(const UgpmWin* __restrict__ wins) {
   const WinPart wp = xcd_win_part();
   const UgpmWin w = load_win(wins, wp.win);
@@ -1102,7 +1107,7 @@
   double* Kc = w.JtJ + (size_t)c * S * S;
   const double* st = w.state_t;
   __shared__ int sflag;
-  __shared__ CholLds chol;
+  __shared__ CholLds<ROWS> chol;
   __shared__ Solve16Lds sh;
   const int wave = threadIdx.x >> 6, lane = threadIdx.x & 63, nwave = (int)(blockDim.x >> 6);
   for (int i = wave; i < S; i += nwave)
@@ -1122,7 +1127,7 @@
     for (int jb = 0; jb < nblk; ++jb) {
       const int rows = (nblk - jb) * 16;
       for (int q = threadIdx.x; q < rows * 16; q += blockDim.x) Xc[(size_t)(q >> 4) * 17 + (q & 15)] = (q >> 4) == (q & 15) ? 1.0 : 0.0;
-      blocked_lower_solve16(A, S, jb, Xc, sh);
+      blocked_lower_solve16<KMAX>(A, S, jb, Xc, sh);
       for (int i = wave; i < S; i += nwave) {
         if (lane < 16 && jb * 16 + lane < S) B[(size_t)i * S + jb * 16 + lane] = i >= jb * 16 ? Xc[(size_t)(i - jb * 16) * 17 + lane] : 0.0;
       }
@@ -1839,6 +1844,7 @@
   }
 }
 
+template <int ROWS>
 __global__ __launch_bounds__(512) void lm_step_kernel(const UgpmWin* __restrict__ wins) {
   const UgpmWin w = load_win(wins, blockIdx.x);
   if (*w.status != 0 || w.lmi[1]) return;
@@ -1856,7 +1862,7 @@
   double* xn = w.lmv + 6 * (size_t)n;
   __shared__ double sred[8];
   __shared__ int sflag;
-  __shared__ CholLds chol;
+  __shared__ CholLds<ROWS> chol;
   if (w.lmi[3]) {
     double c = 0.0;
     for (int k = threadIdx.x; k < m; k += blockDim.x) c += w.res[k] * w.res[k];
@@ -1896,7 +1902,7 @@
   __syncthreads();
   double* L = w.lhs + (size_t)j0 * n + j0;
   __shared__ double xs[kCholMaxN / 2];
-  const bool fused = ns < 384 && ns <= (int)blockDim.x && ns <= kCholMaxN / 2;
+  const bool fused = ns < kCholRowsFull && ns <= (int)blockDim.x && ns <= kCholMaxN / 2;
   for (int i = threadIdx.x >> 6; i < ns; i += (int)(blockDim.x >> 6)) {
     const double si = scale[j0 + i];
     for (int j = threadIdx.x & 63; j <= i; j += 64)
@@ -1990,7 +1996,7 @@
   if (*w.status != 0 || !w.correlate) return;
   const int n = 6 * w.S;
   __shared__ int sflag;
-  __shared__ CholLds chol;
+  __shared__ CholLds<kCholRowsFull> chol;
   for (int i = threadIdx.x; i < n; i += blockDim.x) w.Ac[(size_t)i * n + i] += 0.00001;
   __syncthreads();
   if (!block_cholesky(w.Ac, n, n, chol, &sflag)) {
@@ -1999,6 +2005,7 @@
   }
 }
 
+template <int KMAX>
 __global__ __launch_bounds__(256) __attribute__((amdgpu_waves_per_eu(2, 2))) void corr_diag_kernel(const UgpmWin* __restrict__ wins) {
   const WinPart wp = xcd_win_part();
   const UgpmWin w = load_win(wins, wp.win);
@@ -2012,7 +2019,7 @@
     const int rows = ((n + 15) / 16 - jb) * 16;
     for (int q = threadIdx.x; q < rows * 16; q += blockDim.x) Xc[(size_t)(q >> 4) * 17 + (q & 15)] = (q >> 4) == (q & 15) ? 1.0 : 0.0;
   }
-  blocked_lower_solve16(w.Ac, n, jb, Xc, sh);
+  blocked_lower_solve16<KMAX>(w.Ac, n, jb, Xc, sh);
   if (threadIdx.x < 16) {
     const int c = threadIdx.x, col = j0 + c;
     const int rows = ((n + 15) / 16 - jb) * 16;
@@ -2090,6 +2097,7 @@
   }
 }
 
+template <int KMAX>
 __global__ __launch_bounds__(256) void infer_kernel(const UgpmWin* __restrict__ wins) {
   const WinPart wp = xcd_win_part();
   const UgpmWin w = load_win(wins, wp.win);
@@ -2171,7 +2179,7 @@
       const int c = row / S;
       Xc[(size_t)row * 17 + c] = w.dsc[row] * ksK[c][row - c * S];
     }
-    blocked_lower_solve16(w.Ac, n, 0, Xc, sh);
+    blocked_lower_solve16<KMAX>(w.Ac, n, 0, Xc, sh);
     for (int pair = 0; pair < 21; ++pair) {
       int a2 = 0, b2 = pair;
       while (b2 >= 6 - a2) { b2 -= 6 - a2; ++a2; }
diff --git a/go-rio_amd/csrc/ugpm_windows.h b/go-rio_amd/csrc/ugpm_windows.h
--- a/go-rio_amd/csrc/ugpm_windows.h
+++ b/go-rio_amd/csrc/ugpm_windows.h
@@ -10,6 +10,8 @@
 
 namespace gorio {
 namespace windows {
+
+constexpr int kMaxStates = 160;
 
 struct HostWin {
   int g0 = 0, G = 0, v0 = 0, V = 0, S = 0;
@@ -93,7 +95,7 @@
   sf = std::min(sf, std::min(vel_freq, gyr_freq));
   h.state_freq = sf;
   h.S = (int)(std::ceil(duration * sf) + (2 * w.overlap));
-  if (h.S < 2 * w.overlap + 1 || h.S > 160) return fail(GORIO_UGPM_ERR_UNSUPPORTED, "number of GP states outside [2 overlap + 1, 160]");
+  if (h.S < 2 * w.overlap + 1 || h.S > kMaxStates) return fail(GORIO_UGPM_ERR_UNSUPPORTED, "number of GP states outside [2 overlap + 1, 160]");
   h.state_t.resize(h.S);
   const double t0 = w.start_t - (((double)w.overlap) / sf);
   for (int k = 0; k < h.S; ++k) h.state_t[k] = t0 + ((double)k) / sf;
@@ -144,6 +146,41 @@
   }
   return o;
 }
+
+constexpr int kSolveKmaxFull = 16;
+constexpr int kGramRowsSmall = 96, kGramRows = 160;
+constexpr int kGramKmax = 3;
+constexpr int kLmRowsSmall = 192;
+constexpr int kSolveKmaxSmall = 8;
+
+constexpr int ceil16(int v) { return (v + 15) / 16 * 16; }
+constexpr int chol_first_panel(int n, bool rhs) { return n - (n < 16 ? n : 16) + (rhs ? 1 : 0); }
+constexpr bool chol_same_path(int rows, int n, bool rhs) { return chol_first_panel(n, rhs) <= rows; }
+constexpr int chol_rows_needed(int n, bool rhs) {
+  const int m = n - (n < 16 ? n : 16);
+  return rhs ? (ceil16(m) > m + 1 ? ceil16(m) : m + 1) : ceil16(m);
+}
+constexpr int solve16_blocks_needed(int n) { return (ceil16(n) / 16 - 1 + 3) / 4; }
+constexpr int gram_rows_needed(int S) { return chol_rows_needed(S, false) > ceil16(S) ? chol_rows_needed(S, false) : ceil16(S); }
+constexpr int lm_rows_needed(int S) { return chol_rows_needed(3 * S, true) > 34 ? chol_rows_needed(3 * S, true) : 34; }
+constexpr bool gram_fits(int rows, int S) { return gram_rows_needed(S) <= rows && chol_same_path(rows, S, false); }
+constexpr bool lm_fits(int rows, int S) { return 3 * S < kCholRowsFull && lm_rows_needed(S) <= rows && 3 * S <= rows + 16 && chol_same_path(rows, 3 * S, true) && chol_same_path(rows, S, true); }
+
+struct SolverSizes {
+  int gram_rows, gram_kmax;
+  int lm_rows;
+  int solve_kmax;
+};
+
+constexpr SolverSizes solver_sizes(int max_S, bool full) {
+  if (full) return SolverSizes{kCholRowsFull, kSolveKmaxFull, kCholRowsFull, kSolveKmaxFull};
+  return SolverSizes{gram_fits(kGramRowsSmall, max_S) ? kGramRowsSmall : kGramRows, kGramKmax, lm_fits(kLmRowsSmall, max_S) ? kLmRowsSmall : kCholRowsFull,
+                     solve16_blocks_needed(6 * max_S) <= kSolveKmaxSmall ? kSolveKmaxSmall : kSolveKmaxFull};
+}
+static_assert(gram_fits(kGramRows, kMaxStates) && solve16_blocks_needed(kMaxStates) <= kGramKmax, "gram_kernel's capacities hold the largest window");
+static_assert(solve16_blocks_needed(6 * kMaxStates) <= kSolveKmaxFull, "the full solve holds the largest correlation system");
+static_assert(solver_sizes(66, false).gram_rows == kGramRowsSmall && solver_sizes(66, false).lm_rows == kLmRowsSmall && solver_sizes(66, false).solve_kmax == kSolveKmaxSmall,
+              "the 66-state window of the scan-to-scan step runs the small instantiations");
 
 struct LpmHost {
   std::vector<double> tl;
diff --git a/go-rio_amd/ugpm.py b/go-rio_amd/ugpm.py
--- a/go-rio_amd/ugpm.py
+++ b/go-rio_amd/ugpm.py
@@ -136,11 +136,11 @@
     lib.gorio_ugpm_debug_set_schedule(1 if speculative_rot else 0)
 
 
-def ugpm_debug_set_path(dense_ata=False, draining_looks=False):
+def ugpm_debug_set_path(dense_ata=False, draining_looks=False, full_capacity=False):
     lib = load_library()
     lib.gorio_ugpm_debug_set_path.argtypes = [C.c_int]
     lib.gorio_ugpm_debug_set_path.restype = None
-    lib.gorio_ugpm_debug_set_path((1 if dense_ata else 0) | (2 if draining_looks else 0))
+    lib.gorio_ugpm_debug_set_path((1 if dense_ata else 0) | (2 if draining_looks else 0) | (4 if full_capacity else 0))
 
 
 def ugpm_stage_times():
```

Result: faster. 184,800 linearisations/s, median of 6 (+3.1%).
